# KyleHuang9/YOLO-LP

Measured on AMD Instinct MI355X. Metric: images/sec (640×640) end-to-end detect+NMS, yololps, 1/2/4/8 MI355X, higher is better.
Workload: dtype f16; 1 GPU; yololps 640x640 bs=32/GPU f16, synthetic frames resident in HBM, seeded random-init weights (sigma 0.25), conf 0.40 iou 0.45 max_det 1000; global_batch=32, parallelism=dp1: images sharded, all-gather of detections

## Files before the change

### include/lp_hip.h

```cpp
#ifndef LP_HIP_H
#define LP_HIP_H

#include <stddef.h>
#include <stdint.h>

#ifdef __cplusplus
extern "C" {
#endif

typedef enum { LP_OK = 0, LP_ERR_ARG = -1, LP_ERR_STATE = -2, LP_ERR_HIP = -3, LP_ERR_UNSUPPORTED = -4 } lp_status;
typedef enum { LP_F16 = 0, LP_BF16 = 1, LP_F32 = 2 } lp_dtype;
typedef enum { LP_ACT_NONE = 0, LP_ACT_RELU = 1, LP_ACT_SILU = 2 } lp_act;

#define LP_PRED_COLS 290
#define LP_DET_COLS 28
#define LP_MAX_SRC 4

typedef struct lp_engine lp_engine;

const char* lp_version(void);
const char* lp_last_error(void);

int lp_engine_create(lp_engine** out, int act_dtype );
void lp_engine_destroy(lp_engine* e);

int lp_engine_tensor(lp_engine* e, int channels, int stride_log2);

int lp_engine_set_lane(lp_engine* e, int lane);

int lp_engine_add_input(lp_engine* e, int dst);

typedef struct lp_conv_desc {
    int n_src;
    int src[LP_MAX_SRC];
    int dst;
    int ksize;
    int stride;
    int act;
    int res;
    float res_alpha;
    const float* weight;
    const float* bias;
    int dst2;
} lp_conv_desc;

int lp_engine_add_conv(lp_engine* e, const lp_conv_desc* d);

int lp_engine_add_deconv2x2(lp_engine* e, int src, int dst, const float* weight, const float* bias);

int lp_engine_add_pool5_chain(lp_engine* e, int src, int dst1, int dst2, int dst3);

int lp_engine_add_head_cls(lp_engine* e, int src, int level, int n_cls, const float* weight, const float* bias);

int lp_engine_add_head_box(lp_engine* e, int src, int level, int reg_bins, const float* weight, const float* bias,
                           const float* proj);

int lp_engine_finalize(lp_engine* e, int n_levels);
size_t lp_engine_weight_bytes(const lp_engine* e);
int lp_engine_upload(lp_engine* e, void* dev_weights, void* stream);

size_t lp_engine_arena_bytes(const lp_engine* e, int B, int H, int W);
int lp_engine_bind(lp_engine* e, void* dev_arena, size_t bytes, int B, int H, int W);
int lp_engine_tensor_info(const lp_engine* e, int id, size_t* offset, int* c, int* c_stored, int* h, int* w);
int lp_engine_num_anchors(const lp_engine* e);

int lp_engine_forward(lp_engine* e, const void* x, int x_dtype, float* pred, void* stream);

int lp_engine_forward_det(lp_engine* e, const void* x, int x_dtype, double conf_thres, void* workspace, size_t workspace_bytes,
                          void* stream);

int lp_engine_set_graph(lp_engine* e, int enable);

int lp_engine_set_single_lane(lp_engine* e, int enable);

int lp_engine_set_mfma16(lp_engine* e, int enable);

int lp_engine_num_ops(const lp_engine* e);
int lp_engine_op_info(const lp_engine* e, int op, int* kind, int* ksize, int* cin, int* cout, double* flops,
                      double* bytes);
int lp_engine_profile(lp_engine* e, const void* x, int x_dtype, float* pred, void* stream, float* op_ms, int reps);
int lp_engine_profile_ops(lp_engine* e, const void* x, int x_dtype, float* pred, void* stream, float* op_ms, int reps, int inner);

enum { LP_VARIANT_STREAM64 = 16, LP_VARIANT_STREAM128 = 17, LP_VARIANT_ROWS = 18,
       LP_VARIANT_PIPE_D = 32, LP_VARIANT_PIPE_B = 33, LP_VARIANT_PIPE_F = 34, LP_VARIANT_PIPE_C = 35,
       LP_VARIANT_PIPE_P = 36 ,
       LP_VARIANT_PIPE16_D = 39, LP_VARIANT_PIPE16_F = 41 ,
       LP_VARIANT_PIPE16_V0 = 42, LP_VARIANT_PIPE16_V1 = 43 ,
       LP_VARIANT_FUSED_STEM2 = 37 ,
       LP_VARIANT_FUSED_PW_S2 = 38  };
enum { LP_VARIANT_FUSED_BIFUSION = 45 };
enum { LP_VARIANT_BOX_SPARSE = 46, LP_VARIANT_BOX_DENSE = 47 };
enum { LP_VARIANT_PIPE16_S2A = 48, LP_VARIANT_PIPE16_S2B = 49 };
int lp_engine_op_carrier(const lp_engine* e, int op, int frame_direct);
int lp_engine_op_io(const lp_engine* e, int op, int* src , int* n_src, int* res, int* dst );
int lp_engine_autotune(lp_engine* e, const void* x, int x_dtype, float* pred, void* stream, int reps);
int lp_engine_op_variant(const lp_engine* e, int op, int* cfg, int* nbuf);
int lp_engine_set_op_variant(lp_engine* e, int op, int cfg, int nbuf);
int lp_engine_set_op_tile(lp_engine* e, int op, int choice);
int lp_engine_op_tile(const lp_engine* e, int op, int* choice, int* TH, int* TW);
int lp_engine_copy_tuning(lp_engine* dst, const lp_engine* src);

size_t lp_nms_workspace_bytes(int B, int N);
int lp_nms(float* pred, int B, int N, double conf_thres, double iou_thres, int max_det, float* det, int32_t* count,
           int32_t* keep, void* workspace, size_t workspace_bytes, void* stream);

int lp_nms_candidates(int B, int N, double iou_thres, int max_det, float* det, int32_t* count, int32_t* keep, void* workspace,
                      size_t workspace_bytes, void* stream);

const int32_t* lp_nms_candidate_counts(const void* workspace, int B, int N);

int lp_preprocess_letterbox(const unsigned char* img, int h0, int w0, void* out, int out_dtype, int H, int W, int rh, int rw,
                            int top, int left, void* stream);
int lp_rescale_round(float* det, int n, double ratio, double padx, double pady, int img_w, int img_h, void* stream);

#define LP_FRAMES_PER_LAUNCH 64
typedef struct lp_frame_desc {
    const unsigned char* img;
    int h0, w0, rh, rw, top, left;
} lp_frame_desc;
typedef struct lp_rescale_desc { double ratio, padx, pady; int img_w, img_h; } lp_rescale_desc;
int lp_preprocess_letterbox_batch(const lp_frame_desc* desc, int n_frames, int B, void* out, int out_dtype, int H, int W,
                                  void* stream);
int lp_rescale_round_batch(float* det, const int32_t* count, int B, int max_det, const lp_rescale_desc* desc, void* stream);

typedef struct lp_tile_desc {
    const unsigned char* img;
    int h0, w0;
    int y0, x0, th, tw;
    int rh, rw, top, left;
} lp_tile_desc;
int lp_preprocess_tiles_batch(const lp_tile_desc* desc, int n_tiles, int B, void* out, int out_dtype, int H, int W, void* stream);

#define LP_NV12_PER_LAUNCH 32
typedef struct lp_nv12_desc {
    const unsigned char* y;
    const unsigned char* uv;
    int pitch_y, pitch_uv;
    int h0, w0;
    int y0, x0, th, tw;
    int rh, rw, top, left;
    int matrix;
} lp_nv12_desc;
typedef struct lp_nv12_bgr_desc {
    const unsigned char* y;
    const unsigned char* uv;
    int pitch_y, pitch_uv;
    int h0, w0;
    int matrix;
    unsigned char* out;
} lp_nv12_bgr_desc;
int lp_preprocess_nv12_batch(const lp_nv12_desc* desc, int n, int B, void* out, int out_dtype, int H, int W, void* stream);
int lp_nv12_to_bgr_batch(const lp_nv12_bgr_desc* desc, int n, void* stream);

typedef struct lp_tile_ref { int frame, y0, x0, th, tw; } lp_tile_ref;
size_t lp_merge_tiles_workspace_bytes(int n_frames, int max_det);
int lp_merge_tiles(const float* det_t, const int32_t* count_t, const lp_tile_ref* tiles, int n_tiles, int max_det_t,
                   const int* frame_hw, int n_frames, double thres, int metric , int border, int max_det,
                   float* det, int32_t* count, int32_t* src, void* workspace, size_t workspace_bytes, void* stream);

#define LP_TRACK_MAX_TRACKS 128
#define LP_TRACK_MAX_DETS 128
#define LP_TRACK_MAX_CLS 64
typedef struct lp_track_params { double match_thres, new_thres, expand; int max_age; int ncls[8]; } lp_track_params;
size_t lp_track_state_bytes(int n_streams, int max_tracks);
size_t lp_track_dropped_offset(int max_tracks, int stream_index);
int lp_track_update(void* state, int n_streams, int max_tracks, const lp_track_params* p,
                    const float* det, const int32_t* count, int B, int max_det,
                    const int* stream_of , const unsigned char* flush ,
                    float* det_out, int32_t* tid, int32_t* ended_i, float* ended_f, int32_t* ended_count,
                    int max_ended, void* stream);
int lp_track_update_slots(void* state, int n_streams, int max_tracks, const lp_track_params* p,
                          const float* det, const int32_t* count, int B, int max_det,
                          const int* stream_of , const unsigned char* flush ,
                          float* det_out, int32_t* tid, int32_t* slot, int32_t* ended_i, float* ended_f, int32_t* ended_count,
                          int max_ended, void* stream);
typedef struct lp_track_hold_params { int min_hits, max_misses; } lp_track_hold_params;
int lp_track_update_hold(void* state, int n_streams, int max_tracks, const lp_track_params* p,
                         const float* det, const int32_t* count, int B, int max_det,
                         const int* stream_of , const unsigned char* flush ,
                         float* det_out, int32_t* tid, int32_t* slot, int32_t* ended_i, float* ended_f, int32_t* ended_count,
                         int max_ended, const lp_track_hold_params* hp, float* det_hold, int32_t* count_hold, int32_t* tid_hold,
                         void* stream);

typedef struct lp_crop_desc {
    const unsigned char* img;
    int h0, w0;
    int max_crops;
    int out_slot;
} lp_crop_desc;
int lp_plate_crops_batch(const lp_crop_desc* desc, int n_frames, const float* det, const int32_t* count, int max_det,
                         unsigned char* out, int32_t* status, int n_slots, int crop_h, int crop_w, void* stream);

int lp_crop_sharpness(const unsigned char* crops, const int32_t* status, int n_slots, int crop_h, int crop_w,
                      unsigned long long* sharp, void* stream);

size_t lp_best_shot_state_bytes(int n_streams, int max_tracks, int crop_h, int crop_w);
int lp_best_shot_update(void* state, int n_streams, int max_tracks, int crop_h, int crop_w,
                        const float* det, const int32_t* count, int B, int max_det, const int32_t* tid, const int32_t* slot,
                        const unsigned char* crops, const int32_t* status, const unsigned long long* sharp, int max_crops,
                        const int* stream_of , const int32_t* ended_i, const int32_t* ended_count, int max_ended,
                        double min_score, unsigned char* shot_crops, int32_t* shot_i, unsigned long long* shot_q, float* shot_det,
                        void* stream);

typedef struct lp_stack_params { double min_score, min_width; unsigned long long min_sharp; int search, max_frames; } lp_stack_params;
size_t lp_stack_state_bytes(int n_streams, int max_tracks, int crop_h, int crop_w);
int lp_stack_update(void* state, int n_streams, int max_tracks, int crop_h, int crop_w,
                    const float* det, const int32_t* count, int B, int max_det, const int32_t* tid, const int32_t* slot,
                    const unsigned char* crops, const int32_t* status, const unsigned long long* sharp, int max_crops,
                    const int* stream_of , const int32_t* ended_i, const int32_t* ended_count, int max_ended,
                    const lp_stack_params* p, unsigned char* stack_crops, int32_t* stack_i, void* stream);

#define LP_REDACT_MAX_CELL 64
typedef struct lp_redact_desc {
    unsigned char* p0;
    unsigned char* p1;
    int pitch0, pitch1;
    int h0, w0;
    int format;
} lp_redact_desc;
typedef struct lp_redact_params {
    int mode;
    int cell;
    double margin;
    unsigned char fill[3];
} lp_redact_params;
size_t lp_redact_workspace_bytes(const lp_redact_desc* desc, int n_frames, const lp_redact_params* p);
int lp_redact_plates_batch(const lp_redact_desc* desc, int n_frames, const float* det, const int32_t* count, int max_det,
                           const lp_redact_params* p, int32_t* status ,
                           void* workspace, size_t workspace_bytes, void* stream);

#define LP_REDACT_MAX_RADIUS 48
typedef struct lp_redact_gauss_params {
    double margin;
    int radius, radius_c;
    uint16_t taps[LP_REDACT_MAX_RADIUS + 1];
    uint16_t taps_c[LP_REDACT_MAX_RADIUS + 1];
} lp_redact_gauss_params;
size_t lp_redact_gauss_workspace_bytes(const lp_redact_desc* desc, int n_frames, const lp_redact_gauss_params* p);
int lp_redact_gauss_batch(const lp_redact_desc* desc, int n_frames, const float* det, const int32_t* count, int max_det,
                          const lp_redact_gauss_params* p, int32_t* status ,
                          void* workspace, size_t workspace_bytes, void* stream);

#define LP_JPEG_MAX_RESTART 32
#define LP_JPEG_PER_LAUNCH 32
typedef struct lp_jpeg_desc {
// ... 90 lines not shown
```

### yolo-lp_amd/csrc/lp_conv.hip

```cpp
#include "lp_internal.h"

#include <cstdlib>

namespace lp {

int conv_launch_f16(int cfg, int mode, int ksize, int stride, int nbuf, const ConvArgs& a, hipStream_t st);
int conv_launch_bf16(int cfg, int mode, int ksize, int stride, int nbuf, const ConvArgs& a, hipStream_t st);
int conv_launch_f32(int cfg, int mode, int ksize, int stride, int nbuf, const ConvArgs& a, hipStream_t st);

int conv_stream_launch_f16(int wc, const ConvArgs& a, int cb_pack, int lds, hipStream_t st);
int conv_stream_launch_bf16(int wc, const ConvArgs& a, int cb_pack, int lds, hipStream_t st);
int conv_stream_launch_f32(int wc, const ConvArgs& a, int cb_pack, int lds, hipStream_t st);

int conv_pipe_launch_f16(int pcfg, const ConvArgs& a, int ncu, hipStream_t st);
int conv_pipe_launch_bf16(int pcfg, const ConvArgs& a, int ncu, hipStream_t st);

int head_rows_launch_f16(const ConvArgs& a, int cb_pack, hipStream_t st);
int head_rows_launch_bf16(const ConvArgs& a, int cb_pack, hipStream_t st);
int head_rows_launch_f32(const ConvArgs& a, int cb_pack, hipStream_t st);
int head_box_det_launch_f16(const ConvArgs& a, int cb_pack, hipStream_t st);
int head_box_det_launch_bf16(const ConvArgs& a, int cb_pack, hipStream_t st);
int head_box_det_launch_f32(const ConvArgs& a, int cb_pack, hipStream_t st);

ConvShape conv_shape(int dtype, int cfg, int ksize, int stride) {
    const int sz = (int)dtype_size(dtype);
    ConvShape s;
    int wc = 2, wp = 2, wgc = 1, wgp = 4;
    switch (cfg) {
        case CFG_A: wgc = 2; wgp = 2; break;
        case CFG_B: break;
        case CFG_C: wc = 1; break;
        case CFG_D: wgc = 2; wgp = 4; break;
        case CFG_E: wc = 1; wgc = 2; wgp = 2; break;
        case CFG_F: wc = 1; wgc = 4; wgp = 2; break;
    }
    s.WP = wp;
    s.WGC = wgc;
    s.WGP = wgp;
    s.CB = 32 * wc * wgc;
    s.PB = 32 * wp * wgp;
    s.NT = 64 * wgc * wgp;
    s.KC = ksize == 1 ? 128 / sz : 32 / sz;
    s.HPMAX = ksize == 1 ? s.PB : (stride == 1 ? 2 * s.PB + 128 : 5 * s.PB + 128);
    return s;
}

static inline int swz_host(int row, int g, int gpr) { return gpr == 2 ? (g ^ ((row >> 3) & 1)) : (g ^ ((row >> 1) & 7)); }

int conv_pick_pitch(const ConvShape& s, int dtype, int ksize, int stride, int TH, int TW) {
    const int hw = (TW - 1) * stride + ksize, hh = (TH - 1) * stride + ksize;
    if (ksize == 1) return hw;
    (void)dtype;
    const int rowb = 32, gpr = 2, npix = TH * TW;
    static const int G0[16] = {0, 1, 2, 3, 12, 13, 14, 15, 20, 21, 22, 23, 24, 25, 26, 27};
    static const int G1[16] = {4, 5, 6, 7, 8, 9, 10, 11, 16, 17, 18, 19, 28, 29, 30, 31};
    long best_cost = -1;
    int best = hw;
    for (int pitch = hw; pitch < hw + 16; ++pitch) {
        if (hh * pitch > s.HPMAX) break;
        long cost = 0;
        for (int blk = 0; blk * 32 < s.PB; ++blk)
            for (int t = 0; t < ksize * ksize; ++t)
                for (int half = 0; half < 2; ++half)
                    for (int g = 0; g < 2; ++g) {
                        const int* lanes = g ? G1 : G0;
                        int addr[16], n = 0, slot_cnt[16] = {0};
                        for (int k = 0; k < 16; ++k) {
                            int pl = blk * 32 + lanes[k];
                            if (pl >= npix) pl = 0;
                            const int ty = pl / TW, tx = pl - ty * TW;
                            const int kx = t % ksize, hwe = (hw + 1) >> 1;
                            const int col = stride == 2 ? (kx & 1) * hwe + tx + (kx >> 1) : tx * stride + kx;
                            const int hp = (ty * stride + t / ksize) * pitch + col;
                            const int a = hp * rowb + swz_host(hp, half, gpr) * 16;
                            bool dup = false;
                            for (int m = 0; m < n; ++m) dup |= addr[m] == a;
                            if (!dup) { addr[n++] = a; ++slot_cnt[(a >> 4) & 15]; }
                        }
                        int mx = 1;
                        for (int k = 0; k < 16; ++k) mx = slot_cnt[k] > mx ? slot_cnt[k] : mx;
                        cost += mx;
                    }
        cost = cost * 64 + (pitch - hw);
        if (best_cost < 0 || cost < best_cost) { best_cost = cost; best = pitch; }
    }
    return best;
}

int conv_pick_pitch16(const ConvShape& s, int TH, int TW) {
    const int hw = TW + 2, hh = TH + 2, rowb = 32, npix = TH * TW;
    static const int GRP[4][16] = {{0, 1, 2, 3, 12, 13, 14, 15, 20, 21, 22, 23, 24, 25, 26, 27}, {4, 5, 6, 7, 8, 9, 10, 11, 16, 17, 18, 19, 28, 29, 30, 31},
                                   {32, 33, 34, 35, 44, 45, 46, 47, 52, 53, 54, 55, 56, 57, 58, 59}, {36, 37, 38, 39, 40, 41, 42, 43, 48, 49, 50, 51, 60, 61, 62, 63}};
    auto qo = [](int i) { return ((i >> 2) == 2 ? 12 : (i >> 2) == 3 ? 8 : (i & 12)) + (i & 3); };
    long best_cost = -1;
    int best = hw;
    for (int pitch = hw; pitch < hw + 16; ++pitch) {
        if (hh * pitch > s.HPMAX) break;
        long cost = 0;
        for (int blk = 0; blk * 16 < s.PB; ++blk)
            for (int st = 0; st < 9; ++st) {
                const int ta = st < 4 ? 2 * st : (st == 4 ? 8 : 2 * st - 9), tb = st == 4 ? 0 : ta + 1;
                for (int gq = 0; gq < 4; ++gq) {
                    int addr[16], n = 0, slot_cnt[16] = {0};
                    for (int k = 0; k < 16; ++k) {
                        const int l = GRP[gq][k], i = l & 15, g = l >> 4;
                        int pl = blk * 16 + qo(i);
                        if (pl >= npix) pl = 0;
                        const int ty = pl / TW, tx = pl - ty * TW, t = g < 2 ? ta : tb;
                        const int hp = (ty + t / 3) * pitch + tx + t % 3;
                        const int a = hp * rowb + swz_host(hp, g & 1, 2) * 16 + (g >> 1) * (1 << 20);
                        bool dup = false;
                        for (int m = 0; m < n; ++m) dup |= addr[m] == a;
                        if (!dup) { addr[n++] = a; ++slot_cnt[(a >> 4) & 15]; }
                    }
                    int mx = 1;
                    for (int k = 0; k < 16; ++k) mx = slot_cnt[k] > mx ? slot_cnt[k] : mx;
                    cost += mx;
                }
            }
        cost = cost * 64 + (pitch - hw);
        if (best_cost < 0 || cost < best_cost) { best_cost = cost; best = pitch; }
    }
    return best;
}

void conv_pick_tile16v(const ConvShape& s, int Ho, int Wo, int B, int nct, int choice, int* TH, int* TW, int stride) {
    struct Cand { double cost; int th, tw; };
    Cand best[4];
    int n = 0;
    const int ncu = device_cus();
    for (int th = 1; th <= Ho; ++th)
        for (int tw = 1; tw <= Wo; ++tw) {
            const int hh = (th - 1) * stride + 3, hw = (tw - 1) * stride + 3;
            if (th * tw > s.PB || hh * hw > s.HPMAX) continue;
            const long tiles = (long)B * ceil_div(Ho, th) * ceil_div(Wo, tw) * nct;
            const int nb = ceil_div(th * tw, 16), per_wave = ceil_div(nb, s.WGP);
            const double cost = (double)ceil_div((int)tiles, ncu) * (per_wave + 0.75) + 1e-4 * hh * hw + 1e-7 * tiles;
            int pos = n < 4 ? n : 4;
            for (int k = 0; k < (n < 4 ? n : 4); ++k)
                if (cost < best[k].cost) { pos = k; break; }
            if (pos >= 4) continue;
            for (int k = (n < 4 ? n : 3); k > pos; --k) best[k] = best[k - 1];
            best[pos] = {cost, th, tw};
            if (n < 4) ++n;
        }
    if (n == 0) { *TH = 1; *TW = 1; return; }
    if (choice < 0) choice = 0;
    if (choice >= n) choice = n - 1;
    *TH = best[choice].th;
    *TW = best[choice].tw;
}

void conv_pick_tile(const ConvShape& s, int ksize, int stride, int Ho, int Wo, int choice, int* TH, int* TW) {
    struct Cand { long cost; int th, tw; };
    Cand best[4];
    int n = 0;
    for (int th = 1; th <= s.PB && th <= Ho; ++th) {
        int tw = s.PB / th;
        if (tw > Wo) tw = Wo;
        if (tw < 1) continue;
        const int hh = (th - 1) * stride + ksize, hw = (tw - 1) * stride + ksize;
        if (hh * hw > s.HPMAX) continue;
        const long tiles = (long)ceil_div(Ho, th) * ceil_div(Wo, tw);
        Cand c = {tiles * 100000 + (long)hh * hw, th, tw};
        int pos = n < 4 ? n : 4;
        for (int k = 0; k < (n < 4 ? n : 4); ++k)
            if (c.cost < best[k].cost) { pos = k; break; }
        if (pos >= 4) continue;
        for (int k = (n < 4 ? n : 3); k > pos; --k) best[k] = best[k - 1];
        best[pos] = c;
        if (n < 4) ++n;
    }
    if (n == 0) { *TH = 1; *TW = 1; return; }
    if (choice < 0) choice = 0;
    if (choice >= n) choice = n - 1;
// ... 48 lines not shown
}

ConvShape conv_pipe_shape(int pcfg) {
    ConvShape s;
    s.KC = 16;
    s.NT = 512;
    s.WP = 2;
    switch (pcfg) {
        case PIPE_B: s.CB = 64; s.WGC = 1; s.WGP = 8; s.HPMAX = 704; break;
        case PIPE_F: case PIPE16_F: s.CB = 128; s.WGC = 4; s.WGP = 2; s.HPMAX = 384; break;
        case PIPE_C: s.CB = 32; s.WGC = 1; s.WGP = 8; s.HPMAX = 736; break;
        case PIPE16_V0: s.CB = 128; s.WGC = 2; s.WGP = 4; s.HPMAX = 512; s.PB = 4 * 7 * 16; return s;
        case PIPE16_V1: s.CB = 128; s.WGC = 4; s.WGP = 2; s.HPMAX = 512; s.PB = 2 * 7 * 16; return s;
        case PIPE16_S2A: s.CB = 128; s.WGC = 2; s.WGP = 4; s.HPMAX = 864; s.PB = 4 * 4 * 16; return s;
        case PIPE16_S2B: s.CB = 128; s.WGC = 4; s.WGP = 2; s.HPMAX = 864; s.PB = 2 * 7 * 16; return s;
        default: s.CB = 128; s.WGC = 2; s.WGP = 4; s.HPMAX = 384; break;
    }
    s.PB = 32 * s.WP * s.WGP;
    return s;
}

bool conv_pipe_fits(int dtype, int pcfg, int cb_pack, int ksize, int stride, int mode, int nct, int nphase, int nchunks) {
    if (pcfg == PIPE_P) return false;
    if (pipe_is_16s2(pcfg))
        return dtype != LP_F32 && ksize == 3 && stride == 2 && mode == MODE_ACT && nphase == 1 && cb_pack == 128 && nct * 128 <= 512 && nchunks >= 1 && nchunks <= 64;
    if (pipe_is_16(pcfg) && (nchunks < 4 || nchunks % 4 != 0)) return false;
    if (dtype == LP_F32 || pcfg < 0 || (pcfg >= PIPE_COUNT && !pipe_is_16(pcfg)) || ksize != 3 || stride != 1 || mode != MODE_ACT || nphase != 1) return false;
    const ConvShape s = conv_pipe_shape(pcfg);
    if (pipe_is_16v(pcfg) && (nct * s.CB > 512 || nchunks > 32)) return false;
    return s.CB == cb_pack && nct * s.CB <= 1024 && nchunks <= 64;
}

static int g_ncu[16] = {0};
int device_cus() {
    int dev = 0;
    if (hipGetDevice(&dev) != hipSuccess || dev < 0 || dev >= 16) return 256;
    if (!g_ncu[dev]) {
        int n = 0;
        if (hipDeviceGetAttribute(&n, hipDeviceAttributeMultiprocessorCount, dev) != hipSuccess || n < 8) n = 256;
        g_ncu[dev] = n / 8 * 8;
        if (const char* cap = getenv("LP_PIPE_MAXWG")) { const int c = atoi(cap) / 8 * 8; if (c >= 8 && c < g_ncu[dev]) g_ncu[dev] = c; }
    }
    return g_ncu[dev];
}

bool stem_planar_tile(int Ho, int Wo, int choice, int* TH, int* TW) {
    struct Cand { long long tiles; int th, tw; };
    std::vector<Cand> cands;
    for (int tw = 4; tw <= 512 && tw < Wo + 4; tw += 4) {
        int th = 512 / tw;
        if (th > Ho) th = Ho;
        while (th >= 1 && ((th + 2) * 6 + 2) * (tw / 4 + 2) * 16 > 20 * 1024) --th;
        if (th < 1) continue;
        cands.push_back({(long long)ceil_div(Ho, th) * ceil_div(Wo, tw), th, tw});
    }
    std::sort(cands.begin(), cands.end(), [](const Cand& x, const Cand& y) { return x.tiles != y.tiles ? x.tiles < y.tiles : x.tw > y.tw; });
    if (choice < 0 || choice >= (int)cands.size()) return false;
    *TH = cands[choice].th;
    *TW = cands[choice].tw;
    return true;
}

bool stem2_fused_tile(int Ho, int Wo, int choice, int* TH, int* TW, int* hpitch) {
    struct Cand { long long cost; int th, tw; };
    std::vector<Cand> cands;
    for (int tw = 2; tw <= 128 && tw < Wo + 2; tw += 2)
        for (int th = 1; th <= 128 / tw && th <= Ho; ++th) {
            const int hp4 = tw / 2 + 2, rin = 2 * th + 3, hps = 2 * tw + 1;
            const int ntb = (th * tw + 31) / 32;
            if ((rin * 6 + 2) * hp4 * 16 > 21 * 1024 || (rin * 6 * hp4 + 63) / 64 > 24 || (2 * th + 1) * hps > 640 || ntb * 2 > 16) continue;
            cands.push_back({(long long)ceil_div(Ho, th) * ceil_div(Wo, tw) * (2 * th + 1) * hps, th, tw});
        }
    std::sort(cands.begin(), cands.end(), [](const Cand& x, const Cand& y) { return x.cost != y.cost ? x.cost < y.cost : x.tw > y.tw; });
    if (choice < 0 || choice >= (int)cands.size()) return false;
    *TH = cands[choice].th;
    *TW = cands[choice].tw;
    *hpitch = 2 * cands[choice].tw + 1;
    return true;
}

int conv_pipe_launch(int dtype, int pcfg, const ConvArgs& a, hipStream_t st) {
    if (pcfg == PIPE_P || pcfg == PIPE_FUSED2 || pcfg == PIPE_FUSED_PW || pcfg == PIPE_FUSED_BF) {
        switch (dtype) {
            case LP_F16: return conv_pipe_launch_f16(pcfg, a, device_cus(), st);
            case LP_BF16: return conv_pipe_launch_bf16(pcfg, a, device_cus(), st);
        }
        return fail(LP_ERR_UNSUPPORTED, "planar stem: 16-bit frames only");
    }
    const ConvShape s = conv_pipe_shape(pcfg);
    if (pipe_is_16s2(pcfg)) {
        const int hh2 = 2 * a.TH + 1, hw2 = 2 * a.TW + 1, nchunks = a.chunk_begin[a.nsrc];
        if (a.TH < 1 || a.TW < 1 || a.TH * a.TW > s.PB || a.hpitch != hw2 || hh2 * a.hpitch > s.HPMAX)
            return fail(LP_ERR_ARG, "conv3x3 s2p16: tile does not fit the kernel configuration");
        if (a.tiles_x * a.TW < a.Wo || a.tiles_y * a.TH < a.Ho) return fail(LP_ERR_ARG, "conv3x3 s2p16: tiles do not cover the output");
        if (a.nsrc < 1 || a.nsrc > LP_MAX_SRC || a.nct < 1 || a.nct * s.CB > 512 || nchunks < 1 || nchunks > 64 || a.nphase != 1 || a.out_scale != 1 ||
            a.H != 2 * a.Ho || a.W != 2 * a.Wo || a.out2)
            return fail(LP_ERR_ARG, "conv3x3 s2p16: not a 3x3 stride-2 layer this kernel runs");
        const int stride = a.out_pix_stride > a.res_cs ? a.out_pix_stride : a.res_cs;
        if (((long long)a.TH * a.Wo + a.TW) * stride + 2048 >= (1ll << 31)) return fail(LP_ERR_ARG, "conv3x3 s2p16: a tile's rows span more than 2^31 elements");
        switch (dtype) {
            case LP_F16: return conv_pipe_launch_f16(pcfg, a, device_cus(), st);
            case LP_BF16: return conv_pipe_launch_bf16(pcfg, a, device_cus(), st);
        }
        return fail(LP_ERR_UNSUPPORTED, "conv3x3 s2p16: 16-bit activations only");
    }
    const int hh = a.TH + 2, hw = a.TW + 2;
    if (pcfg < 0 || (pcfg >= PIPE_COUNT && !pipe_is_16(pcfg))) return fail(LP_ERR_ARG, "conv3x3 pipe: configuration");
    if (pipe_is_16(pcfg) && (a.chunk_begin[a.nsrc] < 4 || a.chunk_begin[a.nsrc] % 4 != 0)) return fail(LP_ERR_ARG, "conv3x3 pipe16: K-chunks not a multiple of four");
    if (a.TH < 1 || a.TW < 1 || a.TH * a.TW > s.PB || a.hpitch < hw || hh * a.hpitch > s.HPMAX)
        return fail(LP_ERR_ARG, "conv3x3 pipe: tile does not fit the kernel configuration");
    if (a.tiles_x * a.TW < a.Wo || a.tiles_y * a.TH < a.Ho) return fail(LP_ERR_ARG, "conv3x3 pipe: tiles do not cover the output");
    if (pipe_is_16v(pcfg) && (a.nct * s.CB > 512 || a.chunk_begin[a.nsrc] > 32)) return fail(LP_ERR_ARG, "conv3x3 pipe16v: layer exceeds the kernel's LDS tables");
    if (pipe_is_16v(pcfg)) {
        int stride = a.out_pix_stride > a.res_cs ? a.out_pix_stride : a.res_cs;
        if (a.out2 && a.out2_pix_stride > stride) stride = a.out2_pix_stride;
        if (((long long)a.TH * a.Wo + a.TW) * stride + 2048 >= (1ll << 31)) return fail(LP_ERR_ARG, "conv3x3 pipe16v: a tile's rows span more than 2^31 elements");
    }
    if (a.chunk_begin[a.nsrc] > 64) return fail(LP_ERR_ARG, "conv3x3 pipe: more K-chunks than the kernel's LDS chunk table holds");
    if (a.nsrc < 1 || a.nsrc > LP_MAX_SRC || a.nct < 1 || a.nct * s.CB > 1024 || a.nphase != 1 || a.out_scale != 1 || a.Ho != a.H || a.Wo != a.W)
        return fail(LP_ERR_ARG, "conv3x3 pipe: not a 3x3 stride-1 layer this kernel runs");
    switch (dtype) {
        case LP_F16: return conv_pipe_launch_f16(pcfg, a, device_cus(), st);
        case LP_BF16: return conv_pipe_launch_bf16(pcfg, a, device_cus(), st);
    }
    return fail(LP_ERR_UNSUPPORTED, "conv3x3 pipe: 16-bit activations only");
}

bool head_rows_fits(int dtype, int nchunks, int cb_pack, int out_c) {
    const long lds = (long)nchunks * 9 * 32 * 128 + 9 * 32 * 4 + 32 * 8 + 32 * 1168;
    return nchunks >= 1 && nchunks <= 3 && lds <= 160 * 1024 && (cb_pack == 32 || cb_pack == 64 || cb_pack == 128) && out_c == LP_PRED_COLS - 13;
}
bool head_det_fits(int dtype, int nchunks, int cb_pack, int out_c) {
    const long lds = (long)nchunks * 9 * 32 * 128 + 9 * 32 * 4 + 32 * 8 * 4 + 16 + 6 * 32 * 8 * 4 + 6 * 1168;
    return nchunks >= 1 && nchunks <= (dtype == LP_F32 ? 3 : 4) && lds <= 160 * 1024 && (cb_pack == 32 || cb_pack == 64 || cb_pack == 128) &&
           out_c == LP_PRED_COLS - 13;
}

bool head_box_det_fits(const ConvArgs& a, int cb_pack, int ksize, int stride) {
    const int nchunks = a.chunk_begin[a.nsrc];
    return ksize == 1 && stride == 1 && a.nsrc == 1 && nchunks >= 1 && nchunks <= 4 && a.reg_bins == 1 && a.out_c == 12 && a.nct == 1 &&
           cb_pack >= 32 && a.nphase == 1 && a.out_scale == 1 && a.Ho == a.H && a.Wo == a.W && a.src[0].cs % 8 == 0;
}
int head_box_det_launch(int dtype, const ConvArgs& a, int cb_pack, hipStream_t st) {
    if (!a.det_mode || !a.out || !a.zero || !head_box_det_fits(a, cb_pack, 1, 1)) return fail(LP_ERR_ARG, "head box: op does not fit");
    if (a.out_pix_stride % 4 != 0 || a.out_img_stride % 4 != 0 || ((uintptr_t)a.out & 15)) return fail(LP_ERR_ARG, "head box: candidate rows are not 16-byte aligned");
    switch (dtype) {
        case LP_F16: return head_box_det_launch_f16(a, cb_pack, st);
        case LP_BF16: return head_box_det_launch_bf16(a, cb_pack, st);
        case LP_F32: return head_box_det_launch_f32(a, cb_pack, st);
    }
    return fail(LP_ERR_ARG, "head box: dtype");
}

int head_rows_launch(int dtype, const ConvArgs& a, int cb_pack, hipStream_t st) {
    const int nchunks = a.chunk_begin[a.nsrc];
    if (!(a.det_mode ? head_det_fits(dtype, nchunks, cb_pack, a.out_c) : head_rows_fits(dtype, nchunks, cb_pack, a.out_c)))
        return fail(LP_ERR_ARG, "head rows: op does not fit");
    const int kc = 128 / (int)dtype_size(dtype);
    for (int i = 0; i < a.nsrc; ++i)
        if (a.src[i].cs % (kc / 4) != 0)
            return fail(LP_ERR_ARG, "head rows: source channels are not whole 32-byte K-steps");
    if (a.nphase != 1 || a.out_scale != 1 || a.Ho != a.H || a.Wo != a.W || !a.out) return fail(LP_ERR_ARG, "head rows: bad geometry");
    switch (dtype) {
        case LP_F16: return head_rows_launch_f16(a, cb_pack, st);
        case LP_BF16: return head_rows_launch_bf16(a, cb_pack, st);
        case LP_F32: return head_rows_launch_f32(a, cb_pack, st);
    }
    return fail(LP_ERR_ARG, "head rows: dtype");
}

}

extern "C" int lp_plan_block_tile(int variant, int Ho, int Wo, int B, int nct, int choice, int* TH, int* TW, int* hpitch) {
    const int pcfg = variant - LP_VARIANT_PIPE_D;
    if (!TH || !TW || Ho < 1 || Wo < 1 || B < 1 || nct < 1) return lp::fail(LP_ERR_ARG, "lp_plan_block_tile: bad arguments");
    if (!lp::pipe_is_16v(pcfg) && !lp::pipe_is_16s2(pcfg)) return lp::fail(LP_ERR_UNSUPPORTED, "lp_plan_block_tile: not a block-tiled variant");
    const lp::ConvShape s = lp::conv_pipe_shape(pcfg);
    const int stride = lp::pipe_is_16s2(pcfg) ? 2 : 1;
    lp::conv_pick_tile16v(s, Ho, Wo, B, nct, choice, TH, TW, stride);
    if (hpitch) *hpitch = (*TW - 1) * stride + 3;
    return LP_OK;
}

extern "C" int lp_plan_stem_tile(int fused, int Ho, int Wo, int choice, int* TH, int* TW, int* hpitch) {
    if (!TH || !TW || Ho < 1 || Wo < 1) return lp::fail(LP_ERR_ARG, "lp_plan_stem_tile: bad arguments");
    int hp = 0;
    const bool ok = fused ? lp::stem2_fused_tile(Ho, Wo, choice, TH, TW, &hp) : lp::stem_planar_tile(Ho, Wo, choice, TH, TW);
    if (hpitch) *hpitch = hp;
    return ok ? LP_OK : LP_ERR_UNSUPPORTED;
}
```

### yolo-lp_amd/csrc/lp_conv_bf16.hip

```cpp
#include "lp_conv_kernel.inc"
#include "lp_conv1x1_stream.inc"
#include "lp_head_rows.inc"
#include "lp_head_box.inc"
#include "lp_conv3x3_pipe.inc"
#include "lp_conv3x3_pipe16.inc"
#include "lp_conv3x3_pipe16v.inc"
#include "lp_conv3x3_s2p16.inc"
#include "lp_stem_planar.inc"
#include "lp_stem2_fused.inc"
#include "lp_pw_s2_fused.inc"
#include "lp_bifusion_fused.inc"

namespace lp {
int conv_launch_bf16(int cfg, int mode, int ksize, int stride, int nbuf, const ConvArgs& a, hipStream_t st) {
    return launch_dtype<bf16>(cfg, mode, ksize, stride, nbuf, a, st);
}
int conv_stream_launch_bf16(int wc, const ConvArgs& a, int cb_pack, int lds, hipStream_t st) {
    return stream_launch_dtype<bf16>(wc, a, cb_pack, lds, st);
}
int head_rows_launch_bf16(const ConvArgs& a, int cb_pack, hipStream_t st) { return head_rows_launch_dtype<bf16>(a, cb_pack, st); }
int head_box_det_launch_bf16(const ConvArgs& a, int cb_pack, hipStream_t st) { return head_box_det_launch_dtype<bf16>(a, cb_pack, st); }
int conv_pipe_launch_bf16(int pcfg, const ConvArgs& a, int ncu, hipStream_t st) {
    if (pcfg == PIPE_FUSED2) return stem2_fused_launch<bf16>(a, ncu, st);
    if (pcfg == PIPE_FUSED_PW) return pw_s2_fused_launch<bf16>(a, ncu, st);
    if (pcfg == PIPE_FUSED_BF) return bifusion_launch_dtype<bf16>(a, ncu, st);
    if (pipe_is_16s2(pcfg)) return s2p16_launch_dtype<bf16>(pcfg, a, ncu, st);
    if (pipe_is_16v(pcfg)) return pipe16v_launch_dtype<bf16>(pcfg, a, ncu, st);
    if (pipe_is_16(pcfg)) return pipe16_launch_dtype<bf16>(pcfg, a, ncu, st);
    return pcfg == PIPE_P ? stem_planar_launch<bf16>(a, ncu, st) : pipe_launch_dtype<bf16>(pcfg, a, ncu, st);
}
}
```

### yolo-lp_amd/csrc/lp_conv_f16.hip

```cpp
#include "lp_conv_kernel.inc"
#include "lp_conv1x1_stream.inc"
#include "lp_head_rows.inc"
#include "lp_head_box.inc"
#include "lp_conv3x3_pipe.inc"
#include "lp_conv3x3_pipe16.inc"
#include "lp_conv3x3_pipe16v.inc"
#include "lp_conv3x3_s2p16.inc"
#include "lp_stem_planar.inc"
#include "lp_stem2_fused.inc"
#include "lp_pw_s2_fused.inc"
#include "lp_bifusion_fused.inc"

namespace lp {
int conv_launch_f16(int cfg, int mode, int ksize, int stride, int nbuf, const ConvArgs& a, hipStream_t st) {
    return launch_dtype<f16>(cfg, mode, ksize, stride, nbuf, a, st);
}
int conv_stream_launch_f16(int wc, const ConvArgs& a, int cb_pack, int lds, hipStream_t st) {
    return stream_launch_dtype<f16>(wc, a, cb_pack, lds, st);
}
int head_rows_launch_f16(const ConvArgs& a, int cb_pack, hipStream_t st) { return head_rows_launch_dtype<f16>(a, cb_pack, st); }
int head_box_det_launch_f16(const ConvArgs& a, int cb_pack, hipStream_t st) { return head_box_det_launch_dtype<f16>(a, cb_pack, st); }
int conv_pipe_launch_f16(int pcfg, const ConvArgs& a, int ncu, hipStream_t st) {
    if (pcfg == PIPE_FUSED2) return stem2_fused_launch<f16>(a, ncu, st);
    if (pcfg == PIPE_FUSED_PW) return pw_s2_fused_launch<f16>(a, ncu, st);
    if (pcfg == PIPE_FUSED_BF) return bifusion_launch_dtype<f16>(a, ncu, st);
    if (pipe_is_16s2(pcfg)) return s2p16_launch_dtype<f16>(pcfg, a, ncu, st);
    if (pipe_is_16v(pcfg)) return pipe16v_launch_dtype<f16>(pcfg, a, ncu, st);
    if (pipe_is_16(pcfg)) return pipe16_launch_dtype<f16>(pcfg, a, ncu, st);
    return pcfg == PIPE_P ? stem_planar_launch<f16>(a, ncu, st) : pipe_launch_dtype<f16>(pcfg, a, ncu, st);
}
}
```

### yolo-lp_amd/csrc/lp_engine.hip

```cpp
#include "lp_internal.h"

#include <cmath>
#include <cstdlib>
#include <cstring>
#include <map>
#include <utility>
#include <vector>

namespace lp {

static thread_local std::string g_err;
void set_error(const std::string& msg) { g_err = msg; }
int fail(int code, const std::string& msg) {
    g_err = msg;
    return code;
}

enum OpKind { OP_INPUT = 0, OP_CONV = 1, OP_DECONV = 2, OP_POOL = 3, OP_HEAD_CLS = 4, OP_HEAD_BOX = 5 };

struct Tensor {
    int c, cs, sl;
    bool unused = false;
    size_t offset;
    int h, w;
};

struct Choice {
    int cfg = CFG_A, nbuf = 1, tile = 0;
    int stream_wc = 0, stream_rd = 2;
    int rows = 0;
    int pipe = 0;
    int planar = 0;
    int fused = 0;
    int fused_pw = 0;
    int fused_bf = 0;
    Choice& choice() { return *this; }
};

struct Op : Choice {
    int kind = OP_CONV;
    int nsrc = 0;
    int src[LP_MAX_SRC] = {-1, -1, -1, -1};
    int dst = -1, dst2 = -1, dst3 = -1;
    int ksize = 1, stride = 1, act = 0;
    int res = -1;
    float alpha = 0.f;
    int cout = 0;
    int cin = 0;
    int level = 0, reg_bins = 1;
    bool s2d = false;
    int alg_kk = 0;
    int lane = 0;
    std::vector<int> deps;
    bool signal = false;
    std::vector<float> weight, bias, proj;
    int mode = MODE_ACT, nct = 1, nchunks = 0, nphase = 1;
    size_t det_scratch = (size_t)-1;
    int box_sparse = 1;
    int bf_up = -1, bf_cv1 = -1;
    int bf_carrier = -1;
    int chunk_begin[LP_MAX_SRC + 1] = {0, 0, 0, 0, 0};
    size_t w_off = 0, b_off = 0, proj_off = 0;
    long long w_phase_stride = 0;
};

struct Launch : Choice {
    ConvArgs a;
    long long pred_off = 0;
    int mode = 0, ks = 1, st = 1, cb_pack = 0;
    bool is_conv = false;
};

}

using namespace lp;
struct lp_engine;
static bool bifusion_fused_possible(const lp_engine* e, size_t i, int* up, int* cv1);
static bool op_fam16(const lp_engine* e, const lp::Op& op);
static int fam16_default_pipe(const lp_engine* e, const lp::Op& op);

#ifndef LP_MAX_LANES
#define LP_MAX_LANES 5
#endif
struct lp_engine {
    int dtype = LP_F16;
    bool finalized = false;
    int n_levels = 3;
    std::vector<Tensor> tensors;
    std::vector<Op> ops;
    std::vector<unsigned char> blob;
    char* dev_w = nullptr;
    char* arena = nullptr;
    size_t arena_bytes = 0;
    int B = 0, H = 0, W = 0, n_anchors = 0;
    std::vector<int> level_off;
    std::vector<hipEvent_t> events;
    int cur_lane = 0;
    int n_lanes = 1;
    hipStream_t lane_stream[LP_MAX_LANES] = {};
    std::vector<hipEvent_t> op_event;
    hipEvent_t fork_ev = nullptr, join_ev[LP_MAX_LANES] = {};
    bool single_lane = true;
    bool use_graph = false;
    bool s2p16 = getenv("LP_S2P16") != nullptr;
    bool mfma16 = getenv("LP_NO_MFMA16") == nullptr;
    bool box_sparse_ok = false;
    std::vector<int> box_ord;
    struct CachedGraph {
        hipGraphExec_t exec = nullptr;
        const void* x = nullptr;
        float* pred = nullptr;
        void* ws = nullptr;
        float conf = 0.f;
        int x_dtype = -1;
        unsigned long long epoch = 0, last_use = 0;
        hipStream_t stream = nullptr;
    };
    std::vector<CachedGraph> graphs;
    unsigned long long graph_clock = 0;
    hipEvent_t done_ev = nullptr;
    bool done_valid = false;
    hipStream_t cap_stream = nullptr;
    unsigned long long epoch = 1;
    std::vector<Launch> launches;
    Launch stem_planar;
    Launch stem2_fused;
    std::map<int, Launch> pw_fused;
    std::map<int, Launch> bf_fused;
    std::map<std::vector<int>, std::vector<Choice>> tuned;
};

static int prepare_op(lp_engine* e, size_t idx);
static int* op_tile_slot(lp_engine* e, int op_idx, int* bias, const Launch** L);
static unsigned long long* g_stamps = nullptr;
extern "C" void lpdbg_set_stamps(void* p) { g_stamps = (unsigned long long*)p; }
static bool valid_tensor(const lp_engine* e, int id) { return id >= 0 && id < (int)e->tensors.size(); }

extern "C" const char* lp_version(void) { return "yololp-hip 0.1 (gfx950)"; }
extern "C" const char* lp_last_error(void) { return g_err.c_str(); }

extern "C" int lp_engine_create(lp_engine** out, int act_dtype) {
    if (!out) return fail(LP_ERR_ARG, "lp_engine_create: null out");
    if (act_dtype != LP_F16 && act_dtype != LP_BF16 && act_dtype != LP_F32) return fail(LP_ERR_ARG, "lp_engine_create: dtype");
    lp_engine* e = new lp_engine();
    e->dtype = act_dtype;
    *out = e;
    return LP_OK;
}

extern "C" void lp_engine_destroy(lp_engine* e) {
    if (!e) return;
    for (int l = 1; l < LP_MAX_LANES; ++l)
        if (e->lane_stream[l]) (void)hipStreamSynchronize(e->lane_stream[l]);
    if (e->done_valid) (void)hipEventSynchronize(e->done_ev);
    if (e->done_ev) (void)hipEventDestroy(e->done_ev);
    for (hipEvent_t ev : e->events) (void)hipEventDestroy(ev);
    for (auto& g : e->graphs) {
        if (g.stream) (void)hipStreamSynchronize(g.stream);
        if (g.exec) (void)hipGraphExecDestroy(g.exec);
    }
    if (e->cap_stream) (void)hipStreamDestroy(e->cap_stream);
    for (hipEvent_t ev : e->op_event) if (ev) (void)hipEventDestroy(ev);
    if (e->fork_ev) (void)hipEventDestroy(e->fork_ev);
    for (int l = 1; l < LP_MAX_LANES; ++l) { if (e->join_ev[l]) (void)hipEventDestroy(e->join_ev[l]); if (e->lane_stream[l]) (void)hipStreamDestroy(e->lane_stream[l]); }
    delete e;
}

extern "C" int lp_engine_tensor(lp_engine* e, int channels, int stride_log2) {
    if (!e || e->finalized) return fail(LP_ERR_STATE, "lp_engine_tensor: engine is null or frozen");
    if (channels < 1 || stride_log2 < 0 || stride_log2 > 6) return fail(LP_ERR_ARG, "lp_engine_tensor: bad shape");
    Tensor t;
    t.c = channels;
    t.cs = round_up(channels, 8);
    t.sl = stride_log2;
    t.offset = 0;
    t.h = t.w = 0;
    e->tensors.push_back(t);
    return (int)e->tensors.size() - 1;
}

extern "C" int lp_engine_set_lane(lp_engine* e, int lane) {
    if (!e || e->finalized) return fail(LP_ERR_STATE, "lp_engine_set_lane: engine is null or frozen");
    if (lane < 0 || lane >= LP_MAX_LANES) return fail(LP_ERR_ARG, "lp_engine_set_lane: lane must be 0..4");
    e->cur_lane = lane;
    return LP_OK;
}

extern "C" int lp_engine_add_input(lp_engine* e, int dst) {
    if (!e || e->finalized) return fail(LP_ERR_STATE, "lp_engine_add_input: engine is null or frozen");
    if (!e->ops.empty()) return fail(LP_ERR_STATE, "lp_engine_add_input: must be the first op");
    if (!valid_tensor(e, dst) || e->tensors[dst].c != 3 || e->tensors[dst].sl != 0)
        return fail(LP_ERR_ARG, "lp_engine_add_input: dst must be a 3-channel full-resolution tensor");
    Op op;
    op.kind = OP_INPUT;
    op.dst = dst;
    op.cout = 3;
    op.cin = 3;
    op.lane = e->cur_lane;
    e->ops.push_back(op);
    return LP_OK;
}

extern "C" int lp_engine_add_conv(lp_engine* e, const lp_conv_desc* d) {
    if (!e || e->finalized) return fail(LP_ERR_STATE, "lp_engine_add_conv: engine is null or frozen");
    if (!d || !d->weight || !d->bias) return fail(LP_ERR_ARG, "lp_engine_add_conv: null descriptor / weights");
    if (d->n_src < 1 || d->n_src > LP_MAX_SRC) return fail(LP_ERR_ARG, "lp_engine_add_conv: n_src");
    if (!((d->ksize == 1 && d->stride == 1) || (d->ksize == 3 && (d->stride == 1 || d->stride == 2))))
        return fail(LP_ERR_UNSUPPORTED, "lp_engine_add_conv: only 1x1/s1, 3x3/s1 and 3x3/s2");
    if (d->act < LP_ACT_NONE || d->act > LP_ACT_SILU) return fail(LP_ERR_ARG, "lp_engine_add_conv: act");
    if (!valid_tensor(e, d->dst)) return fail(LP_ERR_ARG, "lp_engine_add_conv: dst");
    Op op;
    op.kind = OP_CONV;
    op.nsrc = d->n_src;
    int cin = 0;
    if (!valid_tensor(e, d->src[0])) return fail(LP_ERR_ARG, "lp_engine_add_conv: src");
    const int sl = e->tensors[d->src[0]].sl;
    for (int i = 0; i < d->n_src; ++i) {
        if (!valid_tensor(e, d->src[i])) return fail(LP_ERR_ARG, "lp_engine_add_conv: src");
        if (e->tensors[d->src[i]].sl != sl) return fail(LP_ERR_ARG, "lp_engine_add_conv: sources differ in resolution");
        if (d->src[i] == d->dst) return fail(LP_ERR_ARG, "lp_engine_add_conv: in-place conv");
        op.src[i] = d->src[i];
        cin += e->tensors[d->src[i]].c;
    }
    const Tensor& td = e->tensors[d->dst];
    if (td.sl != sl + (d->stride == 2 ? 1 : 0)) return fail(LP_ERR_ARG, "lp_engine_add_conv: dst resolution");
    if (d->res >= 0) {
        if (!valid_tensor(e, d->res) || e->tensors[d->res].c != td.c || e->tensors[d->res].sl != td.sl || d->res == d->dst)
            return fail(LP_ERR_ARG, "lp_engine_add_conv: residual shape");
    }
    int cout2 = 0;
    if (d->dst2 > 0) {
        if (!valid_tensor(e, d->dst2) || d->dst2 == d->dst || e->tensors[d->dst2].sl != td.sl) return fail(LP_ERR_ARG, "lp_engine_add_conv: dst2");
        for (int i = 0; i < d->n_src; ++i) if (d->src[i] == d->dst2) return fail(LP_ERR_ARG, "lp_engine_add_conv: in-place conv");
        if (d->res >= 0) return fail(LP_ERR_UNSUPPORTED, "lp_engine_add_conv: no residual with two destinations");
        if (td.c % 8 != 0) return fail(LP_ERR_UNSUPPORTED, "lp_engine_add_conv: the first destination of two needs a multiple of 8 channels");
        cout2 = e->tensors[d->dst2].c;
    }
    op.dst = d->dst;
    op.dst2 = d->dst2 > 0 ? d->dst2 : -1;
    op.ksize = d->ksize;
    op.stride = d->stride;
    op.act = d->act;
    op.res = d->res >= 0 ? d->res : -1;
    op.alpha = d->res_alpha;
    op.cout = td.c + cout2;
    op.cin = cin;
    op.weight.assign(d->weight, d->weight + (size_t)op.cout * cin * d->ksize * d->ksize);
    op.bias.assign(d->bias, d->bias + op.cout);
    op.lane = e->cur_lane;
    e->ops.push_back(op);
    return LP_OK;
}

extern "C" int lp_engine_add_deconv2x2(lp_engine* e, int src, int dst, const float* weight, const float* bias) {
    if (!e || e->finalized) return fail(LP_ERR_STATE, "lp_engine_add_deconv2x2: engine is null or frozen");
    if (!weight || !bias || !valid_tensor(e, src) || !valid_tensor(e, dst) || src == dst)
        return fail(LP_ERR_ARG, "lp_engine_add_deconv2x2: bad argument");
    if (e->tensors[dst].sl != e->tensors[src].sl - 1) return fail(LP_ERR_ARG, "lp_engine_add_deconv2x2: dst must be 2x the source");
    Op op;
    op.kind = OP_DECONV;
    op.nsrc = 1;
    op.src[0] = src;
    op.dst = dst;
    op.cin = e->tensors[src].c;
    op.cout = e->tensors[dst].c;
    op.weight.assign(weight, weight + (size_t)op.cin * op.cout * 4);
    op.bias.assign(bias, bias + op.cout);
    op.lane = e->cur_lane;
    e->ops.push_back(op);
    return LP_OK;
}

extern "C" int lp_engine_add_pool5_chain(lp_engine* e, int src, int dst1, int dst2, int dst3) {
    if (!e || e->finalized) return fail(LP_ERR_STATE, "lp_engine_add_pool5_chain: engine is null or frozen");
    const int ids[4] = {src, dst1, dst2, dst3};
    for (int i = 0; i < 4; ++i) {
        if (!valid_tensor(e, ids[i])) return fail(LP_ERR_ARG, "lp_engine_add_pool5_chain: tensor id");
        if (e->tensors[ids[i]].c != e->tensors[src].c || e->tensors[ids[i]].sl != e->tensors[src].sl)
            return fail(LP_ERR_ARG, "lp_engine_add_pool5_chain: shapes differ");
        for (int k = 0; k < i; ++k)
            if (ids[k] == ids[i]) return fail(LP_ERR_ARG, "lp_engine_add_pool5_chain: tensors must be distinct");
    }
    Op op;
    op.kind = OP_POOL;
    op.nsrc = 1;
    op.src[0] = src;
    op.dst = dst1;
    op.dst2 = dst2;
    op.dst3 = dst3;
    op.cin = op.cout = e->tensors[src].c;
    op.lane = e->cur_lane;
    e->ops.push_back(op);
    return LP_OK;
}

static int add_head(lp_engine* e, int kind, int src, int level, int cout, int reg_bins, const float* weight, const float* bias,
                    const float* proj) {
    if (!e || e->finalized) return fail(LP_ERR_STATE, "lp_engine_add_head: engine is null or frozen");
    if (!weight || !bias || !valid_tensor(e, src) || level < 0 || level > 3 || cout < 1)
        return fail(LP_ERR_ARG, "lp_engine_add_head: bad argument");
    if (e->tensors[src].sl != 3 + level) return fail(LP_ERR_ARG, "lp_engine_add_head: level / resolution mismatch (strides 8,16,32,64)");
    Op op;
    op.kind = kind;
    op.nsrc = 1;
    op.src[0] = src;
    op.level = level;
    op.reg_bins = reg_bins;
    op.cin = e->tensors[src].c;
    op.cout = cout;
    op.weight.assign(weight, weight + (size_t)cout * op.cin);
    op.bias.assign(bias, bias + cout);
    if (proj) op.proj.assign(proj, proj + reg_bins);
    op.lane = e->cur_lane;
    e->ops.push_back(op);
// ... 55 lines not shown
            const Op& o = e->ops[i];
            for (int k = 0; k < o.nsrc; ++k) only_reader &= o.src[k] != in_id;
            only_reader &= o.res != in_id;
        }
        if (only_reader) {
            Tensor t;
            t.c = 12; t.cs = 16; t.sl = 1; t.offset = 0; t.h = t.w = 0;
            e->tensors.push_back(t);
            const int s2d_id = (int)e->tensors.size() - 1;
            e->tensors[in_id].unused = true;
            e->ops[0].s2d = true;
            e->ops[0].dst = s2d_id;
            std::vector<float> w2((size_t)c.cout * 12 * 9, 0.f);
            for (int co = 0; co < c.cout; ++co)
                for (int ch = 0; ch < 3; ++ch)
                    for (int ky = 0; ky < 3; ++ky)
                        for (int kx = 0; kx < 3; ++kx) {
                            const int dy = ky == 0 ? 0 : 1, py = ky == 1 ? 0 : 1;
                            const int dx = kx == 0 ? 0 : 1, px = kx == 1 ? 0 : 1;
                            w2[(((size_t)co * 12 + ch * 4 + py * 2 + px) * 3 + dy) * 3 + dx] = c.weight[(((size_t)co * 3 + ch) * 3 + ky) * 3 + kx];
                        }
            c.weight.swap(w2);
            c.src[0] = s2d_id;
            c.stride = 1;
            c.cin = 12;
            c.alg_kk = 27;
        }
    }
    if (getenv("LP_SINGLE_LANE")) for (Op& op : e->ops) op.lane = 0;
    e->n_lanes = 1;
    for (size_t i = 0; i < e->ops.size(); ++i) {
        Op& op = e->ops[i];
        if (op.lane + 1 > e->n_lanes) e->n_lanes = op.lane + 1;
        auto reads = [](const Op& o, int t) { for (int k = 0; k < o.nsrc; ++k) if (o.src[k] == t) return true; return o.res == t; };
        auto writes = [](const Op& o, int t) { return o.dst == t || o.dst2 == t || o.dst3 == t; };
        std::vector<int> mine_r, mine_w;
        for (int k = 0; k < op.nsrc; ++k) mine_r.push_back(op.src[k]);
        if (op.res >= 0) mine_r.push_back(op.res);
        for (int t : {op.dst, op.dst2, op.dst3}) if (t >= 0) mine_w.push_back(t);
        for (int lane = 0; lane < LP_MAX_LANES; ++lane) {
            if (lane == op.lane) continue;
            for (size_t j = i; j-- > 0;) {
                const Op& o = e->ops[j];
                if (o.lane != lane) continue;
                bool hit = false;
                for (int t : mine_r) hit |= writes(o, t);
                for (int t : mine_w) hit |= writes(o, t) || reads(o, t);
                if (hit) { op.deps.push_back((int)j); e->ops[j].signal = true; break; }
            }
        }
    }
    for (Op& op : e->ops) {
        if (op.kind == OP_INPUT || op.kind == OP_POOL) continue;
        const int ks = op.kind == OP_CONV ? op.ksize : 1;
        const int st = op.kind == OP_CONV ? op.stride : 1;
        int cout_store;
        if (op.kind == OP_HEAD_CLS) { op.mode = MODE_PRED; op.cfg = getenv("LP_PRED_CFG") ? atoi(getenv("LP_PRED_CFG")) : CFG_C; cout_store = op.cout; }
        else if (op.kind == OP_HEAD_BOX) {
            op.mode = MODE_DECODE; op.cfg = op.cout <= 32 ? CFG_C : CFG_A; cout_store = op.cout;
        }
        else {
            op.mode = MODE_ACT;
            cout_store = e->tensors[op.dst].cs + (op.kind == OP_CONV && op.dst2 >= 0 ? e->tensors[op.dst2].cs : 0);
            op.cfg = pick_cfg(dt, ks, st, cout_store);
            if (op.cfg == CFG_A) op.cfg = CFG_D;
            const char* tc = getenv("LP_TUNE_CFG128");
            const char* tb = getenv("LP_TUNE_NBUF");
            if (tc && op.cfg == CFG_D) op.cfg = atoi(tc);
            if (tb && op.cfg != CFG_C) op.nbuf = atoi(tb) == 2 ? 2 : 1;
        }
        const ConvShape s = conv_shape(dt, op.cfg, ks, st);
        op.nct = ceil_div(cout_store, s.CB);
        op.nphase = op.kind == OP_DECONV ? 4 : 1;
        int cin_off[LP_MAX_SRC + 1] = {0};
        op.chunk_begin[0] = 0;
        for (int i = 0; i < op.nsrc; ++i) {
            const Tensor& t = e->tensors[op.src[i]];
            op.chunk_begin[i + 1] = op.chunk_begin[i] + ceil_div(t.cs, s.KC);
            cin_off[i + 1] = cin_off[i] + t.c;
        }
        for (int i = op.nsrc; i < LP_MAX_SRC; ++i) op.chunk_begin[i + 1] = op.chunk_begin[op.nsrc];
        op.nchunks = op.chunk_begin[op.nsrc];
        if (op_fam16(e, op)) op.pipe = fam16_default_pipe(e, op);
        const int taps = ks * ks;
        const size_t per_phase = (size_t)op.nct * op.nchunks * taps * s.CB * s.KC;
        op.w_phase_stride = (long long)per_phase;
        align();
        op.w_off = blob.size();
        blob.resize(blob.size() + per_phase * op.nphase * esz, 0);
        unsigned char* wp = blob.data() + op.w_off;
        for (int ph = 0; ph < op.nphase; ++ph)
            for (int ct = 0; ct < op.nct; ++ct)
                for (int i = 0; i < op.nsrc; ++i) {
                    const Tensor& t = e->tensors[op.src[i]];
                    for (int q = op.chunk_begin[i]; q < op.chunk_begin[i + 1]; ++q) {
                        const int c0 = (q - op.chunk_begin[i]) * s.KC;
                        for (int tp = 0; tp < taps; ++tp)
                            for (int cl = 0; cl < s.CB; ++cl) {
                                const int co = ct * s.CB + cl;
                                if (co >= op.cout) continue;
                                const size_t row = ((((size_t)ph * op.nct + ct) * op.nchunks + q) * taps + tp) * s.CB + cl;
                                const int srow = tp * s.CB + cl;
                                for (int kc = 0; kc < s.KC; ++kc) {
                                    const int c = c0 + kc;
                                    if (c >= t.c) break;
                                    const int ci = cin_off[i] + c;
                                    float v;
                                    if (op.kind == OP_DECONV)
                                        v = op.weight[((size_t)ci * op.cout + co) * 4 + ph];
                                    else
                                        v = op.weight[((size_t)co * op.cin + ci) * taps + tp];
                                    const int epg = 16 / (int)esz, gpr = s.KC / epg;
                                    const int pos = gpr == 2 ? ((kc / epg) ^ ((srow >> 3) & 1)) : ((kc / epg) ^ ((srow >> 1) & 7));
                                    put_elem(wp, row * s.KC + (size_t)pos * epg + kc % epg, v, dt);
                                }
                            }
                    }
                }
        align();
        op.b_off = blob.size();
        blob.resize(blob.size() + (size_t)op.nct * s.CB * 4, 0);
        memcpy(blob.data() + op.b_off, op.bias.data(), (size_t)op.cout * 4);
        if (!op.proj.empty()) {
            align();
            op.proj_off = blob.size();
            blob.resize(blob.size() + op.proj.size() * 4, 0);
            memcpy(blob.data() + op.proj_off, op.proj.data(), op.proj.size() * 4);
        }
        std::vector<float>().swap(op.weight);
    }
    align();
    for (size_t i = 0; i < e->ops.size(); ++i) {
        int up = -1, c1 = -1;
        if (!bifusion_fused_possible(e, i, &up, &c1)) continue;
        e->ops[i].bf_up = up;
        e->ops[i].bf_cv1 = c1;
        e->ops[(size_t)up].bf_carrier = e->ops[(size_t)c1].bf_carrier = (int)i;
    }
    {
        e->box_ord.assign(e->ops.size(), -1);
        bool ok = true;
        int nbox = 0, cls_seen = 0, cls_level = -1;
        for (size_t i = 0; i < e->ops.size(); ++i) {
            const Op& o = e->ops[i];
            if (o.kind == OP_HEAD_CLS) { ++cls_seen; cls_level = o.level; }
            if (o.kind == OP_HEAD_BOX) {
                ok = ok && cls_seen == 1 && cls_level == o.level;
                e->box_ord[i] = nbox++;
                cls_seen = 0;
            }
        }
        e->box_sparse_ok = ok && nbox >= 1 && nbox <= 4 && cls_seen == 0;
    }
    e->finalized = true;
    return LP_OK;
}

extern "C" size_t lp_engine_weight_bytes(const lp_engine* e) { return e && e->finalized ? e->blob.size() : 0; }

extern "C" int lp_engine_upload(lp_engine* e, void* dev_weights, void* stream) {
    if (!e || !e->finalized) return fail(LP_ERR_STATE, "lp_engine_upload: finalize first");
    if (!dev_weights || ((uintptr_t)dev_weights & 255)) return fail(LP_ERR_ARG, "lp_engine_upload: need a 256-byte aligned device pointer");
    LP_HIP_CHECK(hipMemcpyAsync(dev_weights, e->blob.data(), e->blob.size(), hipMemcpyHostToDevice, (hipStream_t)stream));
    LP_HIP_CHECK(hipStreamSynchronize((hipStream_t)stream));
    e->dev_w = (char*)dev_weights;
    return LP_OK;
}

static bool rows_fits(const lp_engine* e, const Op& op);
static bool det_fits(const lp_engine* e, const Op& op);

static size_t place(const lp_engine* e, int B, int H, int W, std::vector<Tensor>* out, std::vector<size_t>* scratch = nullptr) {
    size_t off = 0;
    const size_t esz = dtype_size(e->dtype);
    for (size_t i = 0; i < e->tensors.size(); ++i) {
        Tensor t = e->tensors[i];
        t.h = H >> t.sl;
        t.w = W >> t.sl;
        t.offset = off;
        if (!t.unused) off += ((size_t)B * t.h * t.w * t.cs * esz + 255) / 256 * 256;
        if (out) (*out)[i] = t;
    }
    if (scratch) scratch->assign(e->ops.size(), (size_t)-1);
    for (size_t i = 0; i < e->ops.size(); ++i) {
        const Op& op = e->ops[i];
        if (op.kind != OP_HEAD_CLS || det_fits(e, op)) continue;
        if (scratch) (*scratch)[i] = off;
        off += ((size_t)B * (H >> (3 + op.level)) * (W >> (3 + op.level)) * LP_PRED_COLS * 4 + 255) / 256 * 256;
    }
    return off + 256;
}

static bool pool_fits(const lp_engine* e, int H, int W) {
    for (const Op& op : e->ops) {
        if (op.kind != OP_POOL) continue;
        const Tensor& t = e->tensors[op.src[0]];
        const int h = H >> t.sl, w = W >> t.sl;
        if (pool_min_lds_bytes(e->dtype, h, w) > POOL_MAX_LDS || h * w >= 65536) return false;
    }
    return true;
}

static int size_granule(const lp_engine* e) {
    int sl = 5;
    for (const Tensor& t : e->tensors) sl = t.sl > sl ? t.sl : sl;
    return 1 << sl;
}

extern "C" size_t lp_engine_arena_bytes(const lp_engine* e, int B, int H, int W) {
    if (!e || B < 1) return 0;
    const int g = size_granule(e);
    if (H < g || W < g || H % g || W % g || !pool_fits(e, H, W)) return 0;
    return place(e, B, H, W, nullptr);
}

static bool apply_tuned(lp_engine* e) {
    const auto it = e->tuned.find({e->B, e->H, e->W});
    if (it == e->tuned.end()) return false;
    for (size_t i = 0; i < e->ops.size(); ++i) e->ops[i].choice() = it->second[i];
    return true;
}

extern "C" int lp_engine_bind(lp_engine* e, void* dev_arena, size_t bytes, int B, int H, int W) {
    if (!e || !e->finalized) return fail(LP_ERR_STATE, "lp_engine_bind: finalize first");
    const int gran = size_granule(e);
    if (B < 1 || H < gran || W < gran || H % gran || W % gran)
        return fail(LP_ERR_ARG, "lp_engine_bind: H and W must be positive multiples of " + std::to_string(gran) + " (the coarsest stride of the graph)");
    if (!dev_arena || ((uintptr_t)dev_arena & 255)) return fail(LP_ERR_ARG, "lp_engine_bind: need a 256-byte aligned device pointer");
    if (!pool_fits(e, H, W))
        return fail(LP_ERR_UNSUPPORTED, "lp_engine_bind: the SPPF pool chain keeps a whole stride-32 map in LDS: input too large (limit ~2048x2048 px in "
                                        "f16 / bf16, ~1440x1440 in f32)");
    const size_t need = place(e, B, H, W, nullptr);
    if (bytes < need) return fail(LP_ERR_ARG, "lp_engine_bind: arena too small");
    if ((long long)B * H * W >= (1LL << 31)) return fail(LP_ERR_UNSUPPORTED, "lp_engine_bind: batch too large for 32-bit pixel indices");
    std::vector<size_t> scratch;
    place(e, B, H, W, &e->tensors, &scratch);
    for (size_t i = 0; i < e->ops.size(); ++i) e->ops[i].det_scratch = scratch[i];
    e->arena = (char*)dev_arena;
    e->arena_bytes = bytes;
    e->B = B;
    e->H = H;
    e->W = W;
    e->level_off.assign(e->n_levels + 1, 0);
    for (int l = 0; l < e->n_levels; ++l) e->level_off[l + 1] = e->level_off[l] + (H >> (3 + l)) * (W >> (3 + l));
    e->n_anchors = e->level_off[e->n_levels];
    if (!e->dev_w) return fail(LP_ERR_STATE, "lp_engine_bind: upload the weights first");
    apply_tuned(e);
    e->launches.assign(e->ops.size(), Launch());
    for (size_t i = 0; i < e->ops.size(); ++i) {
        int rc = prepare_op(e, i);
        if (rc) return rc;
    }
    return LP_OK;
}

extern "C" int lp_engine_tensor_info(const lp_engine* e, int id, size_t* offset, int* c, int* c_stored, int* h, int* w) {
    if (!e || !valid_tensor(e, id)) return fail(LP_ERR_ARG, "lp_engine_tensor_info: tensor id");
    const Tensor& t = e->tensors[id];
    if (offset) *offset = t.offset;
    if (c) *c = t.c;
    if (c_stored) *c_stored = t.cs;
    if (h) *h = t.h;
    if (w) *w = t.w;
    return LP_OK;
}

extern "C" int lp_engine_num_anchors(const lp_engine* e) { return e ? e->n_anchors : 0; }
extern "C" int lp_engine_num_ops(const lp_engine* e) { return e ? (int)e->ops.size() : 0; }

extern "C" int lp_engine_op_info(const lp_engine* e, int i, int* kind, int* ksize, int* cin, int* cout, double* flops, double* bytes) {
    if (!e || i < 0 || i >= (int)e->ops.size()) return fail(LP_ERR_ARG, "lp_engine_op_info: op index");
    if (!e->arena) return fail(LP_ERR_STATE, "lp_engine_op_info: bind first");
    const Op& op = e->ops[i];
    const double esz = (double)dtype_size(e->dtype);
    double fl = 0, by = 0;
    auto tbytes = [&](int id) { const Tensor& t = e->tensors[id]; return (double)e->B * t.h * t.w * t.c * esz; };
    const Tensor& s0 = e->tensors[op.kind == OP_INPUT ? op.dst : op.src[0]];
    const double in_px = (double)e->B * s0.h * s0.w;
    switch (op.kind) {
        case OP_INPUT: by = (double)e->B * e->H * e->W * 3 * esz + tbytes(op.dst); break;
        case OP_CONV: {
            const Tensor& d = e->tensors[op.dst];
            fl = 2.0 * e->B * d.h * d.w * op.cout * (op.alg_kk ? op.alg_kk : op.cin * op.ksize * op.ksize);
            for (int k = 0; k < op.nsrc; ++k) by += tbytes(op.src[k]);
            by += tbytes(op.dst) + (op.dst2 >= 0 ? tbytes(op.dst2) : 0) + (op.res >= 0 ? tbytes(op.res) : 0) + (double)op.cout * op.cin * op.ksize * op.ksize * esz;
            break;
        }
        case OP_DECONV: fl = 2.0 * in_px * op.cin * op.cout * 4; by = tbytes(op.src[0]) + tbytes(op.dst) + 4.0 * op.cin * op.cout * esz; break;
        case OP_POOL: by = 4 * tbytes(op.src[0]); break;
        case OP_HEAD_CLS:
        case OP_HEAD_BOX:
            fl = 2.0 * in_px * op.cin * op.cout;
            by = tbytes(op.src[0]) + in_px * (op.kind == OP_HEAD_CLS ? op.cout : 13) * 4 + (double)op.cin * op.cout * esz;
            break;
    }
    if (kind) *kind = op.kind;
    if (ksize) *ksize = op.ksize;
    if (cin) *cin = op.cin;
    if (cout) *cout = op.cout;
    if (flops) *flops = fl;
    if (bytes) *bytes = by;
    return LP_OK;
}

static bool stream_fits(const lp_engine* e, const Op& op, int wc) {
    if (op.kind != OP_CONV || op.ksize != 1 || op.stride != 1 || op.mode != MODE_ACT) return false;
    if (op.dst2 >= 0 && e->tensors[op.dst].cs % (32 * wc) != 0) return false;
    const int kc = 128 / (int)dtype_size(e->dtype);
    for (int i = 0; i < op.nsrc; ++i)
        if (e->tensors[op.src[i]].cs % (kc / 4) != 0) return false;
    return conv_stream_lds(e->dtype, wc, op.nchunks, conv_shape(e->dtype, op.cfg, 1, 1).CB) >= 0;
}

static bool rows_fits(const lp_engine* e, const Op& op) {
    if (op.kind != OP_HEAD_CLS) return false;
    const int kc = 128 / (int)dtype_size(e->dtype);
    for (int i = 0; i < op.nsrc; ++i) {
        const int cs = e->tensors[op.src[i]].cs;
        if (cs % (kc / 4) != 0) return false;
    }
    return head_rows_fits(e->dtype, op.nchunks, conv_shape(e->dtype, op.cfg, 1, 1).CB, op.cout);
}

static bool det_fits(const lp_engine* e, const Op& op) {
    if (op.kind != OP_HEAD_CLS || getenv("LP_NO_HEAD_DET")) return false;
    const int kc = 128 / (int)dtype_size(e->dtype);
    for (int i = 0; i < op.nsrc; ++i) {
        const int cs = e->tensors[op.src[i]].cs;
        if (cs % (kc / 4) != 0) return false;
    }
    return head_det_fits(e->dtype, op.nchunks, conv_shape(e->dtype, op.cfg, 1, 1).CB, op.cout);
}

static bool op_fam16(const lp_engine* e, const Op& op) {
    if (!e->mfma16 || e->dtype == LP_F32 || op.kind != OP_CONV || op.ksize != 3 || op.mode != MODE_ACT) return false;
    if (op.stride == 2)
        return e->s2p16 && op.dst2 < 0 && conv_pipe_fits(e->dtype, PIPE16_S2A, conv_shape(e->dtype, op.cfg, 3, 2).CB, 3, 2, op.mode, op.nct, op.nphase, op.nchunks);
    if (op.stride != 1) return false;
    return conv_pipe_fits(e->dtype, PIPE16_D, conv_shape(e->dtype, op.cfg, 1, 1).CB, 3, 1, op.mode, op.nct, op.nphase, op.nchunks);
}
static int fam16_default_pipe(const lp_engine*, const Op& op) { return (op.stride == 2 ? PIPE16_S2A : PIPE16_D) + 1; }

static int prepare_op(lp_engine* e, size_t idx) {
    ++e->epoch;
    const Op& op = e->ops[idx];
    Launch& L = e->launches[idx];
    L.is_conv = !(op.kind == OP_INPUT || op.kind == OP_POOL);
    if (!L.is_conv) return LP_OK;
    const int dt = e->dtype;
    auto tptr = [&](int id) { return (void*)(e->arena + e->tensors[id].offset); };
    const int ks = op.kind == OP_CONV ? op.ksize : 1, stv = op.kind == OP_CONV ? op.stride : 1;
    const int cb_pack = conv_shape(dt, op.cfg, ks, stv).CB;
    const ConvShape s = op.pipe ? conv_pipe_shape(op.pipe - 1) : conv_shape(dt, op.cfg, ks, stv);
    ConvArgs& a = L.a;
    memset(&a, 0, sizeof(a));
    a.nsrc = op.nsrc;
    for (int i = 0; i < op.nsrc; ++i) { a.src[i].ptr = tptr(op.src[i]); a.src[i].cs = e->tensors[op.src[i]].cs; }
    for (int i = 0; i <= LP_MAX_SRC; ++i) a.chunk_begin[i] = op.chunk_begin[i];
    a.zero = e->dev_w;
    a.trash = e->dev_w + 128;
    a.w = e->dev_w + op.w_off;
    a.bias = (const float*)(e->dev_w + op.b_off);
    const Tensor& s0 = e->tensors[op.src[0]];
    a.B = e->B;
    a.H = s0.h;
    a.W = s0.w;
    a.Ho = stv == 2 ? s0.h / 2 : s0.h;
    a.Wo = stv == 2 ? s0.w / 2 : s0.w;
    if (op.pipe && pipe_is_16s2(op.pipe - 1)) {
        conv_pick_tile16v(s, a.Ho, a.Wo, e->B, op.nct, op.tile, &a.TH, &a.TW, 2);
        a.hpitch = 2 * a.TW + 1;
    } else if (op.pipe && pipe_is_16v(op.pipe - 1)) {
        conv_pick_tile16v(s, a.Ho, a.Wo, e->B, op.nct, op.tile, &a.TH, &a.TW);
        a.hpitch = a.TW + 2;
    } else {
        conv_pick_tile(s, ks, stv, a.Ho, a.Wo, op.tile, &a.TH, &a.TW);
        a.hpitch = (op.pipe && pipe_is_16(op.pipe - 1)) ? conv_pick_pitch16(s, a.TH, a.TW) : conv_pick_pitch(s, dt, ks, stv, a.TH, a.TW);
    }
    a.tw_magic = (unsigned)(((1u << 22) + a.TW - 1) / a.TW);
    a.hp_magic = (unsigned)(((1u << 22) + a.hpitch - 1) / a.hpitch);
    a.tiles_x = ceil_div(a.Wo, a.TW);
    a.tiles_y = ceil_div(a.Ho, a.TH);
    a.nct = op.nct;
    a.nphase = op.nphase;
    a.w_phase_stride = op.w_phase_stride;
    a.out_scale = op.kind == OP_DECONV ? 2 : 1;
    a.act = op.act;
    a.alpha = op.alpha;
    if (op.mode == MODE_ACT) {
        const Tensor& d = e->tensors[op.dst];
        a.out = tptr(op.dst);
        a.out_c = d.cs;
        a.out_pix_stride = d.cs;
        a.out_img_stride = (long long)d.h * d.w * d.cs;
        if (op.kind == OP_CONV && op.dst2 >= 0) {
            const Tensor& d2 = e->tensors[op.dst2];
            a.out2 = tptr(op.dst2);
            a.out_split = d.cs;
            a.out_c = d.cs + d2.cs;
            a.out2_pix_stride = d2.cs;
            a.out2_img_stride = (long long)d2.h * d2.w * d2.cs;
        }
        if (op.res >= 0) { a.res = tptr(op.res); a.res_cs = e->tensors[op.res].cs; }
    } else {
        a.out = nullptr;
        L.pred_off = (long long)e->level_off[op.level] * LP_PRED_COLS + (op.mode == MODE_PRED ? 13 : 0);
        a.out_pix_stride = LP_PRED_COLS;
        a.out_img_stride = (long long)e->n_anchors * LP_PRED_COLS;
        a.out_c = op.cout;
        if (op.mode == MODE_DECODE) {
            a.reg_bins = op.reg_bins;
            a.proj = op.proj.empty() ? nullptr : (const float*)(e->dev_w + op.proj_off);
            a.stride_px = (float)(8 << op.level);
        }
    }
    a.stamps = g_stamps;
    L.choice() = op;
    L.mode = op.mode;
    L.ks = ks;
    L.st = stv;
    L.cb_pack = cb_pack;
    if (op.planar) {
        Launch& P = e->stem_planar;
        P = L;
        ConvArgs& pa = P.a;
        if (pa.W % 4 != 0 || !stem_planar_tile(pa.Ho, pa.Wo, op.planar - 1, &pa.TH, &pa.TW))
            return fail(LP_ERR_UNSUPPORTED, "planar stem: no tile for this frame size");
        pa.tw_magic = (unsigned)(((1u << 22) + pa.TW - 1) / pa.TW);
        pa.tiles_x = ceil_div(pa.Wo, pa.TW);
        pa.tiles_y = ceil_div(pa.Ho, pa.TH);
        pa.src[0].ptr = nullptr;
        P.pipe = PIPE_P + 1;
    }
    if (op.fused) {
        const Op& stem = e->ops[1];
        Launch& F = e->stem2_fused;
        F = L;
        ConvArgs& fa = F.a;
        if (!stem2_fused_tile(fa.Ho, fa.Wo, op.fused - 1, &fa.TH, &fa.TW, &fa.hpitch))
            return fail(LP_ERR_UNSUPPORTED, "fused stem: no tile for this frame size");
        fa.tw_magic = (unsigned)(((1u << 22) + fa.TW - 1) / fa.TW);
        fa.hp_magic = (unsigned)(((1u << 22) + fa.hpitch - 1) / fa.hpitch);
        fa.tiles_x = ceil_div(fa.Wo, fa.TW);
        fa.tiles_y = ceil_div(fa.Ho, fa.TH);
        fa.src[0].ptr = nullptr;
        fa.fz_w1 = e->dev_w + stem.w_off;
        fa.fz_b1 = (const float*)(e->dev_w + stem.b_off);
        fa.fz_act1 = stem.act;
        fa.fz_c1 = e->tensors[stem.dst].cs;
        F.pipe = PIPE_FUSED2 + 1;
    }
    if (op.fused_bf) {
        const Op& up = e->ops[op.bf_up];
        const Op& c1 = e->ops[op.bf_cv1];
        Launch& F = e->bf_fused[(int)idx];
        F = L;
        ConvArgs& fa = F.a;
        fa.src[0].ptr = tptr(up.src[0]); fa.src[0].cs = e->tensors[up.src[0]].cs;
        fa.src[1].ptr = tptr(c1.src[0]); fa.src[1].cs = e->tensors[c1.src[0]].cs;
        fa.fz_w1 = e->dev_w + c1.w_off;
        fa.fz_b1 = (const float*)(e->dev_w + c1.b_off);
        fa.fz_act1 = c1.act;
        fa.bf_wd = e->dev_w + up.w_off;
        fa.bf_bd = (const float*)(e->dev_w + up.b_off);
        fa.bf_wd_phase_stride = up.w_phase_stride;
        F.pipe = PIPE_FUSED_BF + 1;
    }
    if (op.fused_pw) {
        const Op& pw = e->ops[idx - 1];
        Launch& F = e->pw_fused[(int)idx];
        F = L;
        ConvArgs& fa = F.a;
        int hp = 0;
        if (!stem2_fused_tile(fa.Ho, fa.Wo, op.fused_pw - 1, &fa.TH, &fa.TW, &hp))
            return fail(LP_ERR_UNSUPPORTED, "fused 1x1 + 3x3 s2: no tile for this map size");
        fa.hpitch = hp;
        fa.tw_magic = (unsigned)(((1u << 22) + fa.TW - 1) / fa.TW);
        fa.hp_magic = (unsigned)(((1u << 22) + fa.hpitch - 1) / fa.hpitch);
        fa.tiles_x = ceil_div(fa.Wo, fa.TW);
        fa.tiles_y = ceil_div(fa.Ho, fa.TH);
        fa.src[0].ptr = tptr(pw.src[0]);
        fa.src[0].cs = e->tensors[pw.src[0]].cs;
        fa.fz_w1 = e->dev_w + pw.w_off;
        fa.fz_b1 = (const float*)(e->dev_w + pw.b_off);
        fa.fz_act1 = pw.act;
        fa.fz_c1 = e->tensors[pw.dst].cs;
        F.pipe = PIPE_FUSED_PW + 1;
    }
    return LP_OK;
}

static bool stem_planar_possible(const lp_engine* e) {
    return e->dtype != LP_F32 && e->ops.size() > 1 && e->ops[0].kind == OP_INPUT && e->ops[0].s2d && e->ops[1].kind == OP_CONV &&
           e->ops[1].ksize == 3 && e->ops[1].stride == 1 && e->ops[1].mode == MODE_ACT && e->ops[1].nct == 1 && e->ops[1].nchunks == 1 &&
           (conv_shape(e->dtype, e->ops[1].cfg, 3, 1).CB == 32 || conv_shape(e->dtype, e->ops[1].cfg, 3, 1).CB == 64) && e->ops[1].res < 0 &&
           e->ops[1].dst2 < 0;
}
static bool frame_direct(const lp_engine* e, const void* x, int x_dtype) { return x_dtype == e->dtype && ((uintptr_t)x & 15) == 0; }
static bool stem_planar_now(const lp_engine* e, const void* x, int x_dtype) { return e->ops.size() > 1 && e->ops[1].planar && frame_direct(e, x, x_dtype); }
static bool stem2_fused_possible(const lp_engine* e) {
    if (!stem_planar_possible(e) || e->ops.size() < 3) return false;
    const Op& s = e->ops[1];
    const Op& c = e->ops[2];
    if (c.kind != OP_CONV || c.ksize != 3 || c.stride != 2 || c.nsrc != 1 || c.src[0] != s.dst || c.res >= 0 || c.dst2 >= 0 || c.mode != MODE_ACT ||
        c.nct != 1 || c.nphase != 1 || c.nchunks < 1 || c.nchunks > 2 || s.act != LP_ACT_RELU || c.act != LP_ACT_RELU) return false;
    const int cb = conv_shape(e->dtype, c.cfg, 3, 2).CB, cs2 = e->tensors[c.dst].cs;
    if ((cb != 32 && cb != 64) || cb != 32 * ((cs2 + 31) / 32) || e->tensors[s.dst].cs > 16 * c.nchunks) return false;
    for (size_t i = 3; i < e->ops.size(); ++i) {
        const Op& o = e->ops[i];
        for (int k = 0; k < o.nsrc; ++k) if (o.src[k] == s.dst) return false;
        if (o.res == s.dst) return false;
    }
    return true;
}
static bool pw_fused_possible(const lp_engine* e, size_t i) {
    if (e->dtype == LP_F32 || i < 2 || i >= e->ops.size()) return false;
    const Op& p = e->ops[i - 1];
    const Op& c = e->ops[i];
    if (c.kind != OP_CONV || c.ksize != 3 || c.stride != 2 || c.nsrc != 1 || c.res >= 0 || c.dst2 >= 0 || c.mode != MODE_ACT || c.nct != 1 || c.nphase != 1) return false;
    if (p.kind != OP_CONV || p.ksize != 1 || p.stride != 1 || p.nsrc != 1 || p.res >= 0 || p.dst2 >= 0 || p.mode != MODE_ACT || p.nct != 1 || p.nphase != 1 ||
        p.nchunks != 1 || p.dst != c.src[0] || p.lane != c.lane || p.signal) return false;
    const int cs0 = e->tensors[p.src[0]].cs, cs1 = e->tensors[p.dst].cs, cs2 = e->tensors[c.dst].cs;
    if (cs0 != 64 || (cs1 != 32 && cs1 != 64) || (cs2 != 32 && cs2 != 64)) return false;
    if (conv_shape(e->dtype, p.cfg, 1, 1).CB != cs1 || conv_shape(e->dtype, c.cfg, 3, 2).CB != cs2 || c.nchunks != cs1 / 16) return false;
    for (size_t k = 0; k < e->ops.size(); ++k) {
        if (k == i) continue;
        const Op& o = e->ops[k];
        for (int q = 0; q < o.nsrc; ++q) if (o.src[q] == p.dst) return false;
        if (o.res == p.dst) return false;
    }
    return true;
}
static bool bifusion_fused_possible(const lp_engine* e, size_t i, int* up, int* cv1) {
    if (e->dtype == LP_F32 || i >= e->ops.size()) return false;
    const Op& c = e->ops[i];
    if (c.kind != OP_CONV || c.ksize != 1 || c.stride != 1 || c.nsrc != 3 || c.res >= 0 || c.dst2 >= 0 || c.mode != MODE_ACT || c.nct != 1 || c.nphase != 1 ||
        c.nchunks != 3 || c.act != LP_ACT_RELU || conv_shape(e->dtype, c.cfg, 1, 1).CB != 64 || e->tensors[c.dst].cs != 64) return false;
    int ju = -1, ja = -1;
    for (size_t k = 0; k < i; ++k) {
        if (e->ops[k].kind == OP_DECONV && e->ops[k].dst == c.src[0]) ju = (int)k;
        if (e->ops[k].kind == OP_CONV && e->ops[k].dst == c.src[1]) ja = (int)k;
    }
    if (ju < 0 || ja < 0) return false;
    const Op& u = e->ops[ju];
    const Op& p = e->ops[ja];
    if (u.nsrc != 1 || u.nct != 1 || u.nphase != 4 || u.nchunks != 1 || u.act != LP_ACT_NONE ||
        conv_shape(e->dtype, u.cfg, 1, 1).CB != 64 || e->tensors[u.src[0]].cs != 64 || e->tensors[u.dst].cs != 64) return false;
    if (p.ksize != 1 || p.stride != 1 || p.nsrc != 1 || p.res >= 0 || p.dst2 >= 0 || p.mode != MODE_ACT || p.nct != 1 || p.nphase != 1 || p.nchunks != 2 ||
        p.act != LP_ACT_RELU || conv_shape(e->dtype, p.cfg, 1, 1).CB != 64 || e->tensors[p.src[0]].cs != 128 ||
        e->tensors[p.dst].cs != 64 || e->tensors[c.src[2]].cs != 64) return false;
    const Tensor& tf = e->tensors[c.dst];
    const Tensor& tc = e->tensors[u.src[0]];
    if (tf.h != 2 * tc.h || tf.w != 2 * tc.w) return false;
    for (size_t k = 0; k < e->ops.size(); ++k) {
        if (k == i) continue;
        const Op& o = e->ops[k];
        for (int q = 0; q < o.nsrc; ++q) if (o.src[q] == u.dst || o.src[q] == p.dst) return false;
        if (o.res == u.dst || o.res == p.dst) return false;
    }
    if (up) *up = ju;
    if (cv1) *cv1 = ja;
    return true;
}
static bool stem2_fused_now(const lp_engine* e, const void* x, int x_dtype) { return e->ops.size() > 2 && e->ops[2].fused && frame_direct(e, x, x_dtype); }

struct DetCtx {
    NmsWs w;
    float conf;
};

static int run_head_det(lp_engine* e, size_t idx, const DetCtx& dc, hipStream_t st) {
    const Op& op = e->ops[idx];
    const Launch& L = e->launches[idx];
    const int dt = e->dtype;
    ConvArgs a = L.a;
    const int anchor0 = e->level_off[op.level], N = e->n_anchors;
    if (L.mode == MODE_DECODE) {
        a.det_mode = 1;
        a.out = dc.w.rows + (long long)anchor0 * LP_DET_COLS;
        a.out_pix_stride = LP_DET_COLS;
        a.out_img_stride = (long long)N * LP_DET_COLS;
        static const bool no_box_stream = getenv("LP_NO_BOX_STREAM") != nullptr;
        static const bool no_box_sparse = getenv("LP_NO_BOX_SPARSE") != nullptr;
        const bool snap_ok = !no_box_sparse && e->box_sparse_ok && (e->n_lanes <= 1 || e->single_lane) && e->box_ord[idx] >= 0 && N >= 8;
        auto streams = [&](size_t j) { const Launch& Lj = e->launches[j]; return !no_box_stream && head_box_det_fits(Lj.a, Lj.cb_pack, Lj.ks, Lj.st); };
        if (streams(idx)) {
            if (snap_ok) {
                const int k = e->box_ord[idx];
                int* const snaps = dc.w.kept;
                a.det_cnt = dc.w.cnt;
                a.det_np = dc.w.NP;
                a.det_snap = snaps + (size_t)k * e->B;
                bool prev_snap = k == 0;
                for (size_t j = 0; j < idx && !prev_snap; ++j) prev_snap = e->box_ord[j] == k - 1 && streams(j);
                if (op.box_sparse && prev_snap) {
                    a.det_keys = dc.w.keys;
                    a.det_n = N;
                    a.det_anchor0 = anchor0;
                    a.det_prev = k > 0 ? snaps + (size_t)(k - 1) * e->B : nullptr;
                }
            }
            return head_box_det_launch(dt, a, L.cb_pack, st);
        }
        return conv_launch(dt, L.cfg, L.mode, L.ks, L.st, L.nbuf, a, st);
    }
    if (op.det_scratch == (size_t)-1) {
        a.det_mode = 1;
        a.out = dc.w.rows;
        a.det_keys = dc.w.keys;
        a.det_cnt = dc.w.cnt;
        a.det_np = dc.w.NP;
        a.det_n = N;
        a.det_anchor0 = anchor0;
        a.det_conf = dc.conf;
        return head_rows_launch(dt, a, L.cb_pack, st);
    }
    float* const scratch = (float*)(e->arena + op.det_scratch);
    const int rpi = a.Ho * a.Wo;
    a.out = scratch + 13;
    a.out_img_stride = (long long)rpi * LP_PRED_COLS;
    int rc = conv_launch(dt, L.cfg, L.mode, L.ks, L.st, L.nbuf, a, st);
    if (rc) return rc;
    return nms_score_launch(scratch, e->B, rpi, anchor0, N, dc.conf, dc.w, false, st);
}

static int run_op(lp_engine* e, size_t idx, const void* x, int x_dtype, float* pred, hipStream_t st, const DetCtx* det = nullptr) {
    const Op& op = e->ops[idx];
    const int dt = e->dtype;
    auto tptr = [&](int id) { return (void*)(e->arena + e->tensors[id].offset); };
    if (op.kind == OP_INPUT) {
        if (op.s2d && (stem_planar_now(e, x, x_dtype) || stem2_fused_now(e, x, x_dtype))) return LP_OK;
        return op.s2d ? input_s2d_launch(x, x_dtype, tptr(op.dst), dt, e->B, e->H, e->W, st)
                      : input_launch(x, x_dtype, tptr(op.dst), dt, e->B, e->H, e->W, st);
    }
    if (op.kind == OP_POOL) {
        const Tensor& t = e->tensors[op.src[0]];
        return pool_launch(tptr(op.src[0]), tptr(op.dst), tptr(op.dst2), tptr(op.dst3), dt, e->B, t.h, t.w, t.cs, st);
    }
    const Launch& L = e->launches[idx];
    if (idx + 1 < e->ops.size() && e->ops[idx + 1].fused_pw) return LP_OK;
    if (op.bf_carrier >= 0 && e->ops[op.bf_carrier].fused_bf) return LP_OK;
    if (op.fused_bf) return conv_pipe_launch(dt, PIPE_FUSED_BF, e->bf_fused[(int)idx].a, st);
    if (op.fused_pw) return conv_pipe_launch(dt, PIPE_FUSED_PW, e->pw_fused[(int)idx].a, st);
    if (idx == 1 && stem2_fused_now(e, x, x_dtype)) return LP_OK;
    if (idx == 2 && stem2_fused_now(e, x, x_dtype)) {
        ConvArgs a = e->stem2_fused.a;
        a.src[0].ptr = x;
        return conv_pipe_launch(dt, PIPE_FUSED2, a, st);
    }
    if (idx == 1 && op.planar && stem_planar_now(e, x, x_dtype)) {
        ConvArgs a = e->stem_planar.a;
        a.src[0].ptr = x;
        return conv_pipe_launch(dt, PIPE_P, a, st);
    }
    if (L.mode == MODE_ACT && L.pipe) return conv_pipe_launch(dt, L.pipe - 1, L.a, st);
    if (L.mode == MODE_ACT && L.stream_wc) return conv_stream_launch(dt, L.stream_wc, L.a, L.cb_pack, st);
    if (L.mode == MODE_ACT) return conv_launch(dt, L.cfg, L.mode, L.ks, L.st, L.nbuf, L.a, st);
    if (det) return run_head_det(e, idx, *det, st);
    if (!pred) return fail(LP_ERR_ARG, "forward: pred is null");
    ConvArgs a = L.a;
    a.out = pred + L.pred_off;
    if (L.mode == MODE_PRED && L.rows) return head_rows_launch(dt, a, L.cb_pack, st);
    return conv_launch(dt, L.cfg, L.mode, L.ks, L.st, L.nbuf, a, st);
}

static int check_ready(const lp_engine* e, const void* x, int x_dtype) {
    if (!e || !e->finalized) return fail(LP_ERR_STATE, "forward: engine not finalized");
    if (!e->dev_w) return fail(LP_ERR_STATE, "forward: weights not uploaded");
    if (!e->arena) return fail(LP_ERR_STATE, "forward: arena not bound");
    if (!x) return fail(LP_ERR_ARG, "forward: x is null");
    if (x_dtype != LP_F16 && x_dtype != LP_BF16 && x_dtype != LP_F32) return fail(LP_ERR_ARG, "forward: x dtype");
    return LP_OK;
}

static int ensure_lanes(lp_engine* e) {
    for (int l = 1; l < e->n_lanes; ++l)
        if (!e->lane_stream[l]) LP_HIP_CHECK(hipStreamCreateWithFlags(&e->lane_stream[l], hipStreamNonBlocking));
    if (!e->fork_ev) LP_HIP_CHECK(hipEventCreateWithFlags(&e->fork_ev, hipEventDisableTiming));
    for (int l = 1; l < e->n_lanes; ++l)
        if (!e->join_ev[l]) LP_HIP_CHECK(hipEventCreateWithFlags(&e->join_ev[l], hipEventDisableTiming));
    if (e->op_event.size() != e->ops.size()) e->op_event.assign(e->ops.size(), nullptr);
    for (size_t i = 0; i < e->ops.size(); ++i)
        if (e->ops[i].signal && !e->op_event[i]) LP_HIP_CHECK(hipEventCreateWithFlags(&e->op_event[i], hipEventDisableTiming));
    return LP_OK;
}

static int issue_forward(lp_engine* e, const void* x, int x_dtype, float* pred, hipStream_t main_st, const DetCtx* det = nullptr) {
    int rc;
    if (e->n_lanes <= 1 || e->single_lane) {
        for (size_t i = 0; i < e->ops.size(); ++i) {
            rc = run_op(e, i, x, x_dtype, pred, main_st, det);
            if (rc) return rc;
        }
        return LP_OK;
    }
    rc = ensure_lanes(e);
    if (rc) return rc;
    e->lane_stream[0] = main_st;
    LP_HIP_CHECK(hipEventRecord(e->fork_ev, main_st));
    for (int l = 1; l < e->n_lanes; ++l) LP_HIP_CHECK(hipStreamWaitEvent(e->lane_stream[l], e->fork_ev, 0));
    for (size_t i = 0; i < e->ops.size(); ++i) {
        const Op& op = e->ops[i];
        hipStream_t st = e->lane_stream[op.lane];
        for (int d : op.deps) LP_HIP_CHECK(hipStreamWaitEvent(st, e->op_event[d], 0));
        rc = run_op(e, i, x, x_dtype, pred, st, det);
        if (rc) return rc;
        if (op.signal) LP_HIP_CHECK(hipEventRecord(e->op_event[i], st));
    }
    for (int l = 1; l < e->n_lanes; ++l) {
        LP_HIP_CHECK(hipEventRecord(e->join_ev[l], e->lane_stream[l]));
        LP_HIP_CHECK(hipStreamWaitEvent(main_st, e->join_ev[l], 0));
    }
    return LP_OK;
}

extern "C" int lp_engine_set_single_lane(lp_engine* e, int enable) {
    if (!e) return fail(LP_ERR_ARG, "lp_engine_set_single_lane: null engine");
    if (e->single_lane != (enable != 0)) ++e->epoch;
    e->single_lane = enable != 0;
    return LP_OK;
}

extern "C" int lp_engine_set_mfma16(lp_engine* e, int enable) {
    if (!e) return fail(LP_ERR_ARG, "lp_engine_set_mfma16: null engine");
    if (e->finalized) return fail(LP_ERR_STATE, "lp_engine_set_mfma16: the families are fixed by lp_engine_finalize");
    e->mfma16 = enable != 0;
    return LP_OK;
}

extern "C" int lp_engine_set_graph(lp_engine* e, int enable) {
    if (!e) return fail(LP_ERR_ARG, "lp_engine_set_graph: null engine");
    e->use_graph = enable != 0;
    return LP_OK;
}

static int mark_done(lp_engine* e, hipStream_t st) {
    if (!e->done_ev) LP_HIP_CHECK(hipEventCreateWithFlags(&e->done_ev, hipEventDisableTiming | hipEventDisableSystemFence));
    LP_HIP_CHECK(hipEventRecord(e->done_ev, st));
    e->done_valid = true;
    return LP_OK;
}

static int run_forward(lp_engine* e, const void* x, int x_dtype, float* pred, const DetCtx* det, void* ws, hipStream_t main_st) {
    int rc;
    auto issue = [&](hipStream_t st) -> int {
        if (det) { if (int zr = zero_counts_launch(det->w.cnt, e->B, st)) return zr; }
        return issue_forward(e, x, x_dtype, pred, st, det);
    };
    if (!e->use_graph) {
        rc = issue(main_st);
        return rc ? rc : mark_done(e, main_st);
    }
    constexpr size_t kMaxGraphs = 8;
    const float conf = det ? det->conf : 0.f;
    lp_engine::CachedGraph* hit = nullptr;
    for (auto& g : e->graphs)
        if (g.exec && g.x == x && g.pred == pred && g.ws == ws && g.conf == conf && g.x_dtype == x_dtype && g.epoch == e->epoch) hit = &g;
    if (!hit) {
        for (size_t i = 0; i < e->graphs.size();) {
            auto& g = e->graphs[i];
            bool drop = g.epoch != e->epoch;
            if (!drop && e->graphs.size() >= kMaxGraphs) {
                drop = true;
                for (const auto& o : e->graphs) drop = drop && o.last_use >= g.last_use;
            }
            if (!drop) { ++i; continue; }
            if (g.stream) (void)hipStreamSynchronize(g.stream);
            if (g.exec) (void)hipGraphExecDestroy(g.exec);
            e->graphs.erase(e->graphs.begin() + (long)i);
        }
        rc = ensure_lanes(e);
        if (rc) return rc;
        hipGraph_t g = nullptr;
        if (!e->cap_stream) LP_HIP_CHECK(hipStreamCreateWithFlags(&e->cap_stream, hipStreamNonBlocking));
        LP_HIP_CHECK(hipStreamBeginCapture(e->cap_stream, hipStreamCaptureModeThreadLocal));
        rc = issue(e->cap_stream);
        hipError_t ce = hipStreamEndCapture(e->cap_stream, &g);
        if (rc) { if (g) (void)hipGraphDestroy(g); return rc; }
        if (ce != hipSuccess) return fail(LP_ERR_HIP, std::string("hipStreamEndCapture: ") + hipGetErrorString(ce));
        lp_engine::CachedGraph cg;
        ce = hipGraphInstantiate(&cg.exec, g, nullptr, nullptr, 0);
        (void)hipGraphDestroy(g);
        if (ce != hipSuccess) return fail(LP_ERR_HIP, std::string("hipGraphInstantiate: ") + hipGetErrorString(ce));
        cg.x = x;
        cg.pred = pred;
        cg.ws = ws;
        cg.conf = conf;
        cg.x_dtype = x_dtype;
        cg.epoch = e->epoch;
        e->graphs.push_back(cg);
        hit = &e->graphs.back();
    }
    LP_HIP_CHECK(hipGraphLaunch(hit->exec, main_st));
    hit->stream = main_st;
    hit->last_use = ++e->graph_clock;
    return mark_done(e, main_st);
}

extern "C" int lp_engine_forward(lp_engine* e, const void* x, int x_dtype, float* pred, void* stream) {
    int rc = check_ready(e, x, x_dtype);
    if (rc) return rc;
    if (!pred) return fail(LP_ERR_ARG, "forward: pred is null");
    return run_forward(e, x, x_dtype, pred, nullptr, nullptr, (hipStream_t)stream);
}

extern "C" int lp_engine_forward_det(lp_engine* e, const void* x, int x_dtype, double conf_thres, void* workspace, size_t workspace_bytes,
                                     void* stream) {
    int rc = check_ready(e, x, x_dtype);
    if (rc) return rc;
    if (!workspace || ((uintptr_t)workspace & 255)) return fail(LP_ERR_ARG, "lp_engine_forward_det: need a 256-byte aligned workspace");
    if (!(conf_thres >= 0.0 && conf_thres <= 1.0)) return fail(LP_ERR_ARG, "lp_engine_forward_det: conf_thres must be in [0, 1]");
    DetCtx dc;
    dc.w = nms_carve(workspace, e->B, e->n_anchors);
    dc.conf = (float)conf_thres;
    if (workspace_bytes < dc.w.bytes) return fail(LP_ERR_ARG, "lp_engine_forward_det: workspace too small (lp_nms_workspace_bytes)");
    return run_forward(e, x, x_dtype, nullptr, &dc, workspace, (hipStream_t)stream);
}

static int forward_single_lane(lp_engine* e, const void* x, int x_dtype, float* pred, hipStream_t st) {
    for (size_t i = 0; i < e->ops.size(); ++i) {
        int rc = run_op(e, i, x, x_dtype, pred, st);
        if (rc) return rc;
    }
    return LP_OK;
}

extern "C" int lp_engine_profile_ops(lp_engine* e, const void* x, int x_dtype, float* pred, void* stream, float* op_ms, int reps,
                                     int inner) {
    int rc = check_ready(e, x, x_dtype);
    if (rc) return rc;
    if (!op_ms || reps < 1 || inner < 1) return fail(LP_ERR_ARG, "profile: op_ms / reps / inner");
    hipStream_t st = (hipStream_t)stream;
    const size_t n = e->ops.size();
    while (e->events.size() < n + 1) {
        hipEvent_t ev;
        LP_HIP_CHECK(hipEventCreate(&ev));
        e->events.push_back(ev);
    }
    rc = forward_single_lane(e, x, x_dtype, pred, (hipStream_t)stream);
    if (rc) return rc;
    for (size_t i = 0; i < n; ++i) op_ms[i] = 0.f;
    for (int r = 0; r < reps; ++r) {
        LP_HIP_CHECK(hipEventRecord(e->events[0], st));
        for (size_t i = 0; i < n; ++i) {
            for (int k = 0; k < inner; ++k) {
                rc = run_op(e, i, x, x_dtype, pred, st);
                if (rc) return rc;
            }
            LP_HIP_CHECK(hipEventRecord(e->events[i + 1], st));
        }
        LP_HIP_CHECK(hipEventSynchronize(e->events[n]));
        for (size_t i = 0; i < n; ++i) {
            float ms = 0.f;
            LP_HIP_CHECK(hipEventElapsedTime(&ms, e->events[i], e->events[i + 1]));
            op_ms[i] += ms / reps / inner;
        }
    }
    return LP_OK;
}

extern "C" int lp_engine_profile(lp_engine* e, const void* x, int x_dtype, float* pred, void* stream, float* op_ms, int reps) {
    return lp_engine_profile_ops(e, x, x_dtype, pred, stream, op_ms, reps, 1);
}

extern "C" int lp_engine_autotune(lp_engine* e, const void* x, int x_dtype, float* pred, void* stream, int reps) {
    int rc = check_ready(e, x, x_dtype);
    if (rc) return rc;
    if (reps < 1) reps = 3;
    hipStream_t st = (hipStream_t)stream;
    for (Op& op : e->ops) { op.planar = 0; op.fused = 0; op.fused_pw = 0; op.fused_bf = 0; }
    rc = forward_single_lane(e, x, x_dtype, pred, st);
    if (rc) return rc;
    struct EventPair {
        hipEvent_t a = nullptr, b = nullptr;
        ~EventPair() { if (a) (void)hipEventDestroy(a); if (b) (void)hipEventDestroy(b); }
    } evp;
    LP_HIP_CHECK(hipEventCreate(&evp.a));
    LP_HIP_CHECK(hipEventCreate(&evp.b));
    const hipEvent_t e0 = evp.a, e1 = evp.b;
    int trc = LP_OK;
    auto time_best = [&](std::initializer_list<size_t> seq) -> float {
        float ms_min = -1.f;
        for (int round = 0; round < 3 && trc == LP_OK; ++round) {
            float ms = 0.f;
            if (hipEventRecord(e0, st) != hipSuccess) { trc = LP_ERR_HIP; break; }
            for (int r = 0; r < reps; ++r)
                for (size_t k : seq) run_op(e, k, x, x_dtype, pred, st);
            if (hipEventRecord(e1, st) != hipSuccess || hipEventSynchronize(e1) != hipSuccess || hipEventElapsedTime(&ms, e0, e1) != hipSuccess) { trc = LP_ERR_HIP; break; }
            if (ms_min < 0.f || ms < ms_min) ms_min = ms;
        }
        return trc ? -1.f : ms_min;
    };
    auto time_current = [&](size_t i) -> float { return run_op(e, i, x, x_dtype, pred, st) == LP_OK ? time_best({i}) : -1.f; };
    auto walk_tiles = [&](size_t i, float* best) -> int {
        int bias = 0, won = -1, last_th = -1, last_tw = -1;
        const Launch* L = nullptr;
        int* const slot = op_tile_slot(e, (int)i, &bias, &L);
        for (int tile = 0; tile < 3 && slot && trc == LP_OK; ++tile) {
            *slot = tile + bias;
            if (prepare_op(e, i) != LP_OK) continue;
            if (L->a.TH == last_th && L->a.TW == last_tw) break;
            last_th = L->a.TH;
            last_tw = L->a.TW;
            const float ms = time_current(i);
            if (ms >= 0.f && (*best < 0.f || ms < *best)) { *best = ms; won = tile; }
        }
        return won;
    };
    auto try_form = [&](size_t i, int& form, float t_sep, bool tiled) -> int {
        float t_form = -1.f;
        int won = -1;
        if (trc == LP_OK) {
            form = 1;
            if (tiled) won = walk_tiles(i, &t_form);
            else if (prepare_op(e, i) == LP_OK && (t_form = time_current(i)) >= 0.f) won = 0;
        }
        if (trc) return fail(trc, "autotune: event timing failed");
        form = (won >= 0 && t_form < t_sep) ? won + 1 : 0;
        return prepare_op(e, i);
    };
    for (size_t i = 0; i < e->ops.size(); ++i) {
        Op& op = e->ops[i];
        if (e->launches[i].is_conv && op.kind == OP_HEAD_CLS && rows_fits(e, op) && !getenv("LP_NO_HEAD_ROWS")) {
            float best = -1.f;
            int best_rows = 0;
            for (int rows = 0; rows <= 1; ++rows) {
                op.rows = rows;
                if (prepare_op(e, i) != LP_OK) continue;
                const float ms = time_current(i);
                if (ms >= 0.f && (best < 0.f || ms < best)) { best = ms; best_rows = rows; }
            }
            if (trc) return fail(trc, "autotune: event timing failed");
            op.rows = best_rows;
            rc = prepare_op(e, i);
            if (rc) return rc;
            continue;
        }
        if (!e->launches[i].is_conv || op.mode != MODE_ACT) continue;
        const int cb = conv_shape(e->dtype, op.cfg, 1, 1).CB;
        int best_cfg = op.cfg, best_nb = op.nbuf, best_tile = op.tile, best_wc = 0, best_rd = 2, best_pipe = 0;
        float best_ms = -1.f;
        op.stream_wc = 0;
        op.pipe = 0;
        const bool fam16 = op_fam16(e, op);
        for (int cfg = 0; cfg < CFG_COUNT && !fam16; ++cfg) {
            if (conv_shape(e->dtype, cfg, 1, 1).CB != cb) continue;
            for (int nb = 1; nb <= (cfg == CFG_C ? 1 : 2); ++nb) {
                op.cfg = cfg;
                op.nbuf = nb;
                const int tile = walk_tiles(i, &best_ms);
                if (tile >= 0) { best_cfg = cfg; best_nb = nb; best_tile = tile; }
            }
        }
        if (!getenv("LP_NO_STREAM") && !fam16) {
            op.cfg = best_cfg; op.nbuf = best_nb; op.tile = best_tile;
            for (int wc = 2; wc <= 4; wc += 2) {
                if (!stream_fits(e, op, wc)) continue;
                for (int rd = 2; rd <= 2; ++rd) {
                    op.stream_wc = wc;
                    op.stream_rd = rd;
                    if (prepare_op(e, i) != LP_OK) continue;
                    const float ms = time_current(i);
                    if (ms >= 0.f && (best_ms < 0.f || ms < best_ms)) { best_ms = ms; best_wc = wc; best_rd = rd; }
                }
            }
        }
        int pipe_tile = 0;
        if ((!getenv("LP_NO_PIPE") || fam16) && op.kind == OP_CONV) {
            op.cfg = best_cfg; op.nbuf = best_nb; op.stream_wc = 0;
            for (int pc = fam16 ? PIPE16_D : 0; pc < (fam16 ? PIPE_S2_END : PIPE_COUNT); ++pc) {
                if (fam16 && !pipe_is_16(pc)) continue;
                if (!conv_pipe_fits(e->dtype, pc, cb, op.ksize, op.stride, op.mode, op.nct, op.nphase, op.nchunks)) continue;
                op.pipe = pc + 1;
                const int tile = walk_tiles(i, &best_ms);
                if (tile >= 0) { best_pipe = pc + 1; pipe_tile = tile; }
            }
            op.pipe = 0;
            if (fam16 && !best_pipe) best_pipe = fam16_default_pipe(e, op);
        }
        if (trc) return fail(trc, "autotune: event timing failed");
        op.cfg = best_cfg;
        op.nbuf = best_nb;
        op.tile = best_pipe ? pipe_tile : best_tile;
        op.stream_wc = best_pipe ? 0 : best_wc;
        op.stream_rd = best_rd;
        op.pipe = best_pipe;
        op.planar = 0;
        op.fused = 0;
        op.fused_pw = 0;
        rc = prepare_op(e, i);
        if (rc) return rc;
        if (i == 1 && stem_planar_possible(e) && frame_direct(e, x, x_dtype) && !getenv("LP_NO_PLANAR")) {
            const float t_in = time_best({0});
            rc = try_form(i, op.planar, best_ms + t_in, true);
            if (rc) return rc;
        }
        if (i == 2 && stem2_fused_possible(e) && frame_direct(e, x, x_dtype) && !getenv("LP_NO_PLANAR") && !getenv("LP_NO_FUSED_STEM")) {
            rc = try_form(i, op.fused, time_best({0, 1, 2}), true);
            if (rc) return rc;
        }
        if (pw_fused_possible(e, i) && !getenv("LP_NO_FUSED_PW")) {
            rc = try_form(i, op.fused_pw, time_best({i - 1, i}), true);
            if (rc) return rc;
        }
        if (op.bf_up >= 0 && !getenv("LP_NO_FUSED_BF")) {
            rc = try_form(i, op.fused_bf, time_best({(size_t)op.bf_up, (size_t)op.bf_cv1, i}), false);
            if (rc) return rc;
        }
    }
    e->tuned[{e->B, e->H, e->W}].assign(e->ops.begin(), e->ops.end());
    return LP_OK;
}

extern "C" int lp_engine_copy_tuning(lp_engine* dst, const lp_engine* src) {
    if (!dst || !src || !dst->finalized || !src->finalized) return fail(LP_ERR_STATE, "lp_engine_copy_tuning: finalize both engines first");
    if (dst->dtype != src->dtype || dst->ops.size() != src->ops.size()) return fail(LP_ERR_ARG, "lp_engine_copy_tuning: engines differ");
    for (size_t i = 0; i < src->ops.size(); ++i) {
        const Op &a = src->ops[i], &b = dst->ops[i];
        if (a.kind != b.kind || a.ksize != b.ksize || a.stride != b.stride || a.cout != b.cout || a.nchunks != b.nchunks || a.nct != b.nct)
            return fail(LP_ERR_ARG, "lp_engine_copy_tuning: engines were built from different graphs");
    }
    dst->tuned = src->tuned;
    if (dst->arena && apply_tuned(dst))
        for (size_t i = 0; i < dst->ops.size(); ++i) {
            int rc = prepare_op(dst, i);
            if (rc) return rc;
        }
    return LP_OK;
}

extern "C" int lp_engine_set_op_variant(lp_engine* e, int op_idx, int cfg, int nbuf) {
    if (!e || !e->finalized || op_idx < 0 || op_idx >= (int)e->ops.size()) return fail(LP_ERR_ARG, "lp_engine_set_op_variant: op index");
    Op& op = e->ops[op_idx];
    if (op.kind == OP_HEAD_CLS) {
        if (cfg == LP_VARIANT_ROWS && !rows_fits(e, op)) return fail(LP_ERR_UNSUPPORTED, "lp_engine_set_op_variant: the row-writer kernel does not fit this op");
        if (cfg != LP_VARIANT_ROWS && cfg != op.cfg) return fail(LP_ERR_UNSUPPORTED, "lp_engine_set_op_variant: head_cls takes LP_VARIANT_ROWS or its packing tile");
        op.rows = cfg == LP_VARIANT_ROWS;
        e->tuned.erase({e->B, e->H, e->W});
        if (e->arena && op_idx < (int)e->launches.size()) return prepare_op(e, (size_t)op_idx);
        return LP_OK;
    }
    if (op.kind == OP_HEAD_BOX && (cfg == LP_VARIANT_BOX_SPARSE || cfg == LP_VARIANT_BOX_DENSE)) {
        op.box_sparse = cfg == LP_VARIANT_BOX_SPARSE;
        ++e->epoch;
        return LP_OK;
    }
    if (op.kind == OP_INPUT || op.kind == OP_POOL || op.mode != MODE_ACT) return fail(LP_ERR_UNSUPPORTED, "lp_engine_set_op_variant: op has no variants");
    const int ks = op.kind == OP_CONV ? op.ksize : 1, stv = op.kind == OP_CONV ? op.stride : 1;
    const int cb = conv_shape(e->dtype, op.cfg, ks, stv).CB;
    const Choice before = op;
    auto commit = [&]() -> int {
        if (e->arena && op_idx < (int)e->launches.size()) {
            const int rc = prepare_op(e, (size_t)op_idx);
            if (rc) {
                op.choice() = before;
                const std::string why = g_err;
                prepare_op(e, (size_t)op_idx);
                return fail(rc, why);
            }
        }
        e->tuned.erase({e->B, e->H, e->W});
        return LP_OK;
    };
    if (cfg == LP_VARIANT_FUSED_BIFUSION) {
        if (op.bf_up < 0 || nbuf != 3) return fail(LP_ERR_UNSUPPORTED, "lp_engine_set_op_variant: not the cv3 of a 64-channel BiFusion level");
        op.fused_bf = 1;
        return commit();
    }
    if (cfg == LP_VARIANT_FUSED_PW_S2) {
        if (!pw_fused_possible(e, (size_t)op_idx) || nbuf != 3)
            return fail(LP_ERR_UNSUPPORTED, "lp_engine_set_op_variant: no 1x1 layer of at most 64 channels feeds this 3x3 stride-2 layer alone");
        op.fused_bf = 0;
        op.fused_pw = 1;
        return commit();
    }
    if (cfg == LP_VARIANT_FUSED_STEM2) {
        if (op_idx != 2 || !stem2_fused_possible(e) || nbuf != 3)
            return fail(LP_ERR_UNSUPPORTED, "lp_engine_set_op_variant: only the layer behind the stem (3x3 stride 2, <= 64 channels) has the fused form");
        op.fused_bf = op.fused_pw = 0;
        op.fused = 1;
        return commit();
    }
    if (cfg == LP_VARIANT_PIPE_D + PIPE_P) {
        if (op_idx != 1 || !stem_planar_possible(e) || nbuf != 3)
            return fail(LP_ERR_UNSUPPORTED, "lp_engine_set_op_variant: only the stem over the space-to-depth image has the planar form");
        op.fused_bf = op.fused_pw = op.fused = 0;
        op.planar = 1;
        return commit();
    }
    if ((cfg >= LP_VARIANT_PIPE_D && cfg < LP_VARIANT_PIPE_D + PIPE_COUNT) || pipe_is_16(cfg - LP_VARIANT_PIPE_D)) {
        const int pc = cfg - LP_VARIANT_PIPE_D;
        if (!conv_pipe_fits(e->dtype, pc, cb, ks, stv, op.mode, op.nct, op.nphase, op.nchunks) || op.kind != OP_CONV || nbuf != 3)
            return fail(LP_ERR_UNSUPPORTED, "lp_engine_set_op_variant: the pipelined 3x3 kernel does not fit this op");
        op.stream_wc = 0;
        op.pipe = pc + 1;
    } else if (cfg == LP_VARIANT_STREAM64 || cfg == LP_VARIANT_STREAM128) {
        const int wc = cfg == LP_VARIANT_STREAM64 ? 2 : 4;
        if (!stream_fits(e, op, wc) || nbuf != 2)
            return fail(LP_ERR_UNSUPPORTED, "lp_engine_set_op_variant: the streaming 1x1 kernel does not fit this op");
        op.stream_wc = wc;
        op.stream_rd = nbuf;
        op.pipe = 0;
    } else {
        if (cfg < 0 || cfg >= CFG_COUNT || conv_shape(e->dtype, cfg, ks, stv).CB != cb || nbuf < 1 || nbuf > (cfg == CFG_C ? 1 : 2))
            return fail(LP_ERR_UNSUPPORTED, "lp_engine_set_op_variant: variant does not share the op's weight packing");
        op.stream_wc = 0;
        op.pipe = 0;
        op.cfg = cfg;
        op.nbuf = nbuf;
    }
    op.fused_bf = op.fused_pw = op.fused = op.planar = 0;
    return commit();
}

static int* op_tile_slot(lp_engine* e, int op_idx, int* bias, const Launch** L) {
    Op& op = e->ops[(size_t)op_idx];
    if (op.kind == OP_INPUT || op.kind == OP_POOL || op.mode != MODE_ACT || op.fused_bf) return nullptr;
    const bool bound = e->arena && op_idx < (int)e->launches.size();
    *bias = 1;
    if (op.fused_pw) { *L = bound ? &e->pw_fused[op_idx] : nullptr; return &op.fused_pw; }
    if (op.fused) { *L = bound ? &e->stem2_fused : nullptr; return &op.fused; }
    if (op.planar) { *L = bound ? &e->stem_planar : nullptr; return &op.planar; }
    if (op.stream_wc && !op.pipe) return nullptr;
    *bias = 0;
    *L = bound ? &e->launches[(size_t)op_idx] : nullptr;
    return &op.tile;
}

extern "C" int lp_engine_set_op_tile(lp_engine* e, int op_idx, int choice) {
    if (!e || !e->finalized || op_idx < 0 || op_idx >= (int)e->ops.size() || choice < 0) return fail(LP_ERR_ARG, "lp_engine_set_op_tile: op index or choice");
    int bias = 0;
    const Launch* L = nullptr;
    int* slot = op_tile_slot(e, op_idx, &bias, &L);
    if (!slot) return fail(LP_ERR_UNSUPPORTED, "lp_engine_set_op_tile: the op's kernel has no output tiles");
    const Choice before = e->ops[op_idx];
    *slot = choice + bias;
    e->tuned.erase({e->B, e->H, e->W});
    if (e->arena && op_idx < (int)e->launches.size()) {
        const int rc = prepare_op(e, (size_t)op_idx);
        if (rc) { e->ops[op_idx].choice() = before; prepare_op(e, (size_t)op_idx); }
        return rc;
    }
    return LP_OK;
}

extern "C" int lp_engine_op_tile(const lp_engine* e, int op_idx, int* choice, int* TH, int* TW) {
    if (!e || !e->finalized || op_idx < 0 || op_idx >= (int)e->ops.size()) return fail(LP_ERR_ARG, "lp_engine_op_tile: op index");
    int bias = 0;
    const Launch* L = nullptr;
    const int* slot = op_tile_slot(const_cast<lp_engine*>(e), op_idx, &bias, &L);
    if (!slot) return fail(LP_ERR_UNSUPPORTED, "lp_engine_op_tile: the op's kernel has no output tiles");
    if (!L) return fail(LP_ERR_STATE, "lp_engine_op_tile: no shape bound");
    if (choice) *choice = *slot - bias;
    if (TH) *TH = L->a.TH;
    if (TW) *TW = L->a.TW;
    return LP_OK;
}

extern "C" int lp_engine_op_carrier(const lp_engine* e, int op, int frame_direct_) {
    if (!e || op < 0 || op >= (int)e->ops.size()) return -1;
    const Op& o = e->ops[(size_t)op];
    if (o.bf_carrier >= 0 && e->ops[(size_t)o.bf_carrier].fused_bf) return o.bf_carrier;
    if ((size_t)op + 1 < e->ops.size() && e->ops[(size_t)op + 1].fused_pw) return op + 1;
    if (frame_direct_ && e->ops.size() > 2 && e->ops[0].kind == OP_INPUT && e->ops[0].s2d) {
        if (e->ops[2].fused && op <= 1) return 2;
        if (e->ops[1].planar && op == 0) return 1;
    }
    return -1;
}

extern "C" int lp_engine_op_io(const lp_engine* e, int op, int* src, int* n_src, int* res, int* dst) {
    if (!e || !e->finalized || op < 0 || op >= (int)e->ops.size()) return fail(LP_ERR_ARG, "lp_engine_op_io: engine not finalized, or op index");
    const Op& o = e->ops[(size_t)op];
    if (src) for (int k = 0; k < LP_MAX_SRC; ++k) src[k] = k < o.nsrc ? o.src[k] : -1;
    if (n_src) *n_src = o.nsrc;
    if (res) *res = o.res;
    if (dst) { dst[0] = o.dst; dst[1] = o.dst2; dst[2] = o.dst3; }
    return LP_OK;
}

extern "C" int lp_engine_op_variant(const lp_engine* e, int op, int* cfg, int* nbuf) {
    if (!e || op < 0 || op >= (int)e->ops.size()) return fail(LP_ERR_ARG, "lp_engine_op_variant: op index");
    const bool stream = e->ops[op].stream_wc != 0;
    if (e->ops[op].fused_bf) {
        if (cfg) *cfg = LP_VARIANT_FUSED_BIFUSION;
        if (nbuf) *nbuf = 3;
        return LP_OK;
    }
    if (e->ops[op].fused_pw) {
        if (cfg) *cfg = LP_VARIANT_FUSED_PW_S2;
        if (nbuf) *nbuf = 3;
        return LP_OK;
    }
    if (e->ops[op].fused) {
        if (cfg) *cfg = LP_VARIANT_FUSED_STEM2;
        if (nbuf) *nbuf = 3;
        return LP_OK;
    }
    if (e->ops[op].planar) {
        if (cfg) *cfg = LP_VARIANT_PIPE_D + PIPE_P;
        if (nbuf) *nbuf = 3;
        return LP_OK;
    }
    if (e->ops[op].pipe) {
        if (cfg) *cfg = LP_VARIANT_PIPE_D + e->ops[op].pipe - 1;
        if (nbuf) *nbuf = 3;
        return LP_OK;
    }
    if (cfg) *cfg = e->ops[op].rows ? LP_VARIANT_ROWS : stream ? (e->ops[op].stream_wc == 2 ? LP_VARIANT_STREAM64 : LP_VARIANT_STREAM128) : e->ops[op].cfg;
    if (nbuf) *nbuf = stream ? e->ops[op].stream_rd : e->ops[op].nbuf;
    return LP_OK;
}
```

### yolo-lp_amd/csrc/lp_head_box.inc

```
#pragma once
#include "lp_conv_kernel.inc"

namespace lp {

template <typename T, int NCH, bool SPARSE>
__global__ __launch_bounds__(256) void head_box_det_kernel(const ConvArgs a, const int cb_pack, const int gpi) {
    typedef typename Mma<T>::V V;
    constexpr int SZ = sizeof(T), EPG = 16 / SZ, ROWB = 128, NKB = 4, GPR = 8, NK = NCH * NKB;
    const int lane = threadIdx.x & 63, wave = threadIdx.x >> 6;
    const int r = lane & 31, h = lane >> 5;
    const int HW = a.Ho * a.Wo;
    const long long M = (long long)a.B * HW;
    long long ntiles = (M + 31) / 32;
    long long t0 = (long long)blockIdx.x * 4 + wave, tstride = (long long)gridDim.x * 4;
    [[maybe_unused]] int sb = 0, slo = 0, sn = 0;
    if constexpr (SPARSE) {
        sb = blockIdx.x / gpi;
        const int gi = blockIdx.x - sb * gpi;
        int hi = a.det_cnt[sb];
        hi = hi > a.det_np ? a.det_np : hi;
        slo = a.det_prev ? a.det_prev[sb] : 0;
        slo = slo < 0 ? 0 : (slo > hi ? hi : slo);
        sn = hi - slo;
        if (gi == 0 && threadIdx.x == 0) a.det_snap[sb] = hi;
        ntiles = (sn + 31) / 32;
        t0 = (long long)gi * 4 + wave;
        tstride = (long long)gpi * 4;
    } else if (a.det_snap) {
        const int b = blockIdx.x * 256 + threadIdx.x;
        if (b < a.B) { const int c = a.det_cnt[b]; a.det_snap[b] = c > a.det_np ? a.det_np : c; }
    }
    if (t0 >= ntiles) return;

    V wa[NK];
#pragma unroll
    for (int k = 0; k < NK; ++k)
        wa[k] = *(const V*)((const char*)a.w + ((long long)(k / NKB) * cb_pack + r) * ROWB + swz(r, 2 * (k % NKB) + h, GPR) * 16);
    f32x16 bias;
#pragma unroll
    for (int rg = 0; rg < 4; ++rg)
#pragma unroll
        for (int j = 0; j < 4; ++j) bias[4 * rg + j] = a.bias[8 * rg + 4 * h + j];
    const char* const src = (const char*)a.src[0].ptr;
    const int cs = a.src[0].cs;
    const int ngran = cs / EPG;
    const float sp = a.stride_px;

    for (long long t = t0; t < ntiles; t += tstride) {
        long long m = t * 32 + r;
        bool live = m < M;
        if constexpr (SPARSE) {
            live = m < sn;
            const unsigned long long key = a.det_keys[(long long)sb * a.det_np + slo + (live ? m : 0)];
            const int n_ = (int)(unsigned)key - a.det_anchor0;
            live = live && n_ >= 0 && n_ < HW;
            m = (long long)sb * HW + (live ? n_ : 0);
        }
        const char* const row = src + (live ? m : M - 1) * (long long)cs * SZ + h * 16;
        V vb[NK];
#pragma unroll
        for (int k = 0; k < NK; ++k) vb[k] = *(const V*)(2 * k + h < ngran ? row + k * 32 : (const char*)a.zero);
        __builtin_amdgcn_sched_barrier(0);
        f32x16 acc = bias;
#pragma unroll
        for (int k = 0; k < NK; ++k) acc = Mma<T>::mma(wa[k], vb[k], acc);
        if (!live) continue;
        const int b = (int)(m / HW), n = (int)(m - (long long)b * HW);
        const int oy = n / a.Wo, ox = n - oy * a.Wo;
        const float ax = (float)ox + 0.5f, ay = (float)oy + 0.5f;
        float* const o = (float*)a.out + (long long)b * a.out_img_stride + (long long)n * a.out_pix_stride;
        if (h == 0) {
            const float x1 = ax - acc[0], y1 = ay - acc[1], x2 = ax + acc[2], y2 = ay + acc[3];
            const float cx = ((x1 + x2) / 2.f) * sp, cy = ((y1 + y2) / 2.f) * sp, bw = (x2 - x1) * sp, bh = (y2 - y1) * sp;
            const f32x4 v0 = {cx - bw / 2, cy - bh / 2, cx + bw / 2, cy + bh / 2};
            const f32x4 v2 = {(ax + acc[4]) * sp, (ay + acc[5]) * sp, (ax + acc[6]) * sp, (ay - acc[7]) * sp};
            *(f32x4*)o = v0;
            *(f32x4*)(o + 8) = v2;
        } else {
            const f32x4 v1 = {(ax - acc[0]) * sp, (ay - acc[1]) * sp, (ax - acc[2]) * sp, (ay + acc[3]) * sp};
            *(f32x4*)(o + 4) = v1;
        }
    }
}

template <typename T, int NCH>
static inline int head_box_det_launch_one(const ConvArgs& a, int cb_pack, hipStream_t st) {
    const long long ntiles = ((long long)a.B * a.Ho * a.Wo + 31) / 32;
    long long grid = (ntiles + 3) / 4;
    if (grid > 2048) grid = 2048;
    if (a.det_keys) {
        long long gpi = (ntiles / a.B + 3) / 4;
        const long long cap = 2048 / a.B;
        if (gpi > cap) gpi = cap;
        if (gpi < 1) gpi = 1;
        hipLaunchKernelGGL((head_box_det_kernel<T, NCH, true>), dim3((unsigned)(gpi * a.B)), dim3(256), 0, st, a, cb_pack, (int)gpi);
    } else
    hipLaunchKernelGGL((head_box_det_kernel<T, NCH, false>), dim3((unsigned)grid), dim3(256), 0, st, a, cb_pack, 1);
    hipError_t e = hipGetLastError();
    if (e != hipSuccess) return fail(LP_ERR_HIP, std::string("head box launch: ") + hipGetErrorString(e));
    return LP_OK;
}

template <typename T>
static inline int head_box_det_launch_dtype(const ConvArgs& a, int cb_pack, hipStream_t st) {
    switch (a.chunk_begin[a.nsrc]) {
        case 1: return head_box_det_launch_one<T, 1>(a, cb_pack, st);
        case 2: return head_box_det_launch_one<T, 2>(a, cb_pack, st);
        case 3: return head_box_det_launch_one<T, 3>(a, cb_pack, st);
        case 4: return head_box_det_launch_one<T, 4>(a, cb_pack, st);
    }
    return fail(LP_ERR_UNSUPPORTED, "head box: more than four K-chunks");
}

}
```

### yolo-lp_amd/csrc/lp_internal.h

```cpp
#pragma once
#include <hip/hip_runtime.h>
#include <stdint.h>
#include <stddef.h>
#include <atomic>
#include <string>

#include "../../include/lp_hip.h"

#ifndef LP_PRO_ORDER
#define LP_PRO_ORDER 0
#endif

namespace lp {

typedef _Float16 f16;
typedef __bf16 bf16;

void set_error(const std::string& msg);
int fail(int code, const std::string& msg);
#define LP_HIP_CHECK(expr)                                                                       \
    do {                                                                                         \
        hipError_t _e = (expr);                                                                  \
        if (_e != hipSuccess)                                                                    \
            return ::lp::fail(LP_ERR_HIP, std::string(#expr) + ": " + hipGetErrorString(_e));    \
    } while (0)

template <typename K> inline int set_max_lds_once(K kernel, int bytes, std::atomic<unsigned long long>& done, const char* what) {
    int dev = 0;
    if (hipGetDevice(&dev) != hipSuccess || dev < 0 || dev >= 64) dev = -1;
    if (dev >= 0 && ((done.load(std::memory_order_acquire) >> dev) & 1ull)) return LP_OK;
    hipError_t e = hipFuncSetAttribute((const void*)kernel, hipFuncAttributeMaxDynamicSharedMemorySize, bytes);
    if (e != hipSuccess) return fail(LP_ERR_HIP, std::string(what) + ": LDS attribute: " + hipGetErrorString(e));
    if (dev >= 0) done.fetch_or(1ull << dev, std::memory_order_release);
    return LP_OK;
}

__device__ __forceinline__ void resize_coef(int d, double scale, int src, int* s0, int* a0, int* a1) {
    float f = (float)((d + 0.5) * scale - 0.5);
    int s = (int)floorf(f);
    f -= (float)s;
    if (s < 0) { f = 0.f; s = 0; }
    if (s >= src - 1) { f = 0.f; s = src - 1; }
    *s0 = s;
    const float c0 = (1.f - f) * 2048.f, c1 = f * 2048.f;
    *a0 = (int)rintf(c0);
    *a1 = (int)rintf(c1);
}
__device__ __forceinline__ int resize_blend(int t00, int t01, int t10, int t11, int a0, int a1, int b0, int b1) {
    const int h0v = t00 * a0 + t01 * a1;
    const int h1v = t10 * a0 + t11 * a1;
    return (((b0 * (h0v >> 4)) >> 16) + ((b1 * (h1v >> 4)) >> 16) + 2) >> 2;
}
constexpr int LETTERBOX_PAD = 114;

std::string plane_fault(const unsigned char* y, const unsigned char* uv, int pitch_y, int pitch_uv, int h0, int w0, int matrix);

inline size_t dtype_size(int dt) { return dt == LP_F32 ? 4 : 2; }
inline int round_up(int x, int m) { return (x + m - 1) / m * m; }
inline int ceil_div(int a, int b) { return (a + b - 1) / b; }

enum ConvMode { MODE_ACT = 0, MODE_PRED = 1, MODE_DECODE = 2 };
enum ConvCfg { CFG_A = 0 , CFG_B = 1 , CFG_C = 2 , CFG_D = 3 , CFG_E = 4 , CFG_F = 5 , CFG_COUNT = 6 };

enum PipeCfgId { PIPE_D = 0 , PIPE_B = 1 , PIPE_F = 2 , PIPE_C = 3 , PIPE_P = 4 , PIPE_COUNT = 5,
                 PIPE_FUSED2 = 5 ,
                 PIPE_FUSED_PW = 6 ,
                 PIPE_FUSED_BF = 13 ,
                 PIPE16_D = 7, PIPE16_F = 9 ,
                 PIPE16_V0 = 10, PIPE16_V1 = 11 , PIPE_END = 12,
                 PIPE16_S2A = 16, PIPE16_S2B = 17 , PIPE_S2_END = 18 };
inline bool pipe_is_16s2(int pcfg) { return pcfg == PIPE16_S2A || pcfg == PIPE16_S2B; }
inline bool pipe_is_16(int pcfg) { return pcfg == PIPE16_D || pcfg == PIPE16_F || pcfg == PIPE16_V0 || pcfg == PIPE16_V1 || pipe_is_16s2(pcfg); }
inline bool pipe_is_16v(int pcfg) { return pcfg == PIPE16_V0 || pcfg == PIPE16_V1; }

struct ConvSrc {
    const void* ptr;
    int cs;
};

struct ConvArgs {
    ConvSrc src[LP_MAX_SRC];
    int chunk_begin[LP_MAX_SRC + 1];
    int nsrc;
    const void* w;
    const float* bias;
    unsigned long long* stamps;
    const void* zero;
    void* trash;
    void* out;
    void* out2;
    int out_split;
    int out2_pix_stride;
    long long out2_img_stride;
    const void* res;
    int res_cs;
    float alpha;
    int B, H, W;
    int Ho, Wo;
    int TH, TW, tiles_x, tiles_y;
    unsigned tw_magic, hp_magic;
    int hpitch;
    int nct;
    int out_c;
    long long out_img_stride;
    int out_pix_stride;
    int out_scale;
    int nphase;
    long long w_phase_stride;
    int act;
    int det_mode;
    unsigned long long* det_keys;
    int* det_cnt;
    int det_np, det_n, det_anchor0;
    float det_conf;
    const int* det_prev;
    int* det_snap;
    const void* fz_w1;
    const float* fz_b1;
    int fz_act1, fz_c1;
    const void* bf_wd;
    const float* bf_bd;
    long long bf_wd_phase_stride;
    int reg_bins;
    const float* proj;
    float stride_px;
};

struct ConvShape {
    int CB, PB, KC, HPMAX, NT, WP, WGC, WGP;
};
ConvShape conv_shape(int dtype, int cfg, int ksize, int stride);
void conv_pick_tile(const ConvShape& s, int ksize, int stride, int Ho, int Wo, int choice, int* TH, int* TW);
int conv_pick_pitch(const ConvShape& s, int dtype, int ksize, int stride, int TH, int TW);
int conv_pick_pitch16(const ConvShape& s, int TH, int TW);
void conv_pick_tile16v(const ConvShape& s, int Ho, int Wo, int B, int nct, int choice, int* TH, int* TW, int stride = 1);
int device_cus();
int conv_launch(int dtype, int cfg, int mode, int ksize, int stride, int nbuf, const ConvArgs& a, hipStream_t st);
bool stem_planar_tile(int Ho, int Wo, int choice, int* TH, int* TW);
bool stem2_fused_tile(int Ho, int Wo, int choice, int* TH, int* TW, int* hpitch);

int conv_stream_lds(int dtype, int wc, int nchunks, int cb_pack);
int conv_stream_launch(int dtype, int wc, const ConvArgs& a, int cb_pack, hipStream_t st);

ConvShape conv_pipe_shape(int pcfg);
bool conv_pipe_fits(int dtype, int pcfg, int cb_pack, int ksize, int stride, int mode, int nct, int nphase, int nchunks);
int conv_pipe_launch(int dtype, int pcfg, const ConvArgs& a, hipStream_t st);

bool head_rows_fits(int dtype, int nchunks, int cb_pack, int out_c);
bool head_det_fits(int dtype, int nchunks, int cb_pack, int out_c);
bool head_box_det_fits(const ConvArgs& a, int cb_pack, int ksize, int stride);
int head_box_det_launch(int dtype, const ConvArgs& a, int cb_pack, hipStream_t st);
int head_rows_launch(int dtype, const ConvArgs& a, int cb_pack, hipStream_t st);

struct NmsWs {
    int32_t* cnt;
    unsigned long long* keys;
    float* rows;
    float4* sbox;
    int32_t* kept;
    int NP;
    size_t bytes;
};
NmsWs nms_carve(void* base, int B, int N);
int nms_score_launch(float* pred, int B, int rows_per_img, int anchor0, int N, float conf_f, const NmsWs& w, bool write_box, hipStream_t st);
int zero_counts_launch(int* p, int n, hipStream_t st);

int input_launch(const void* x, int x_dtype, void* dst, int dtype, int B, int H, int W, hipStream_t st);
int input_s2d_launch(const void* x, int x_dtype, void* dst, int dtype, int B, int H, int W, hipStream_t st);
size_t pool_min_lds_bytes(int dtype, int h, int w);
constexpr size_t POOL_MAX_LDS = 128 * 1024;
int pool_launch(const void* src, void* d1, void* d2, void* d3, int dtype, int B, int h, int w, int cs, hipStream_t st);

}
```

### yolo-lp_amd/yolov6/hip/abi.py

```python
import ctypes
import os
from ctypes import POINTER, c_char_p, c_double, c_float, c_int, c_int32, c_size_t, c_void_p

LP_F16, LP_BF16, LP_F32 = 0, 1, 2
LP_ACT_NONE, LP_ACT_RELU, LP_ACT_SILU = 0, 1, 2
LP_PRED_COLS, LP_DET_COLS, LP_MAX_SRC = 290, 28, 4
LP_VARIANT_STREAM64, LP_VARIANT_STREAM128, LP_VARIANT_ROWS = 16, 17, 18
LP_VARIANT_PIPE_D, LP_VARIANT_PIPE_B, LP_VARIANT_PIPE_F, LP_VARIANT_PIPE_C = 32, 33, 34, 35
LP_VARIANT_PIPE16_D, LP_VARIANT_PIPE16_F = 39, 41
LP_VARIANT_PIPE16_V0, LP_VARIANT_PIPE16_V1 = 42, 43
LP_VARIANT_PIPE16_S2A, LP_VARIANT_PIPE16_S2B = 48, 49
LP_VARIANT_FUSED_BIFUSION = 45
LP_VARIANT_BOX_SPARSE, LP_VARIANT_BOX_DENSE = 46, 47
LP_VARIANT_FUSED_PW_S2 = 38
LP_VARIANT_FUSED_STEM2 = 37
LP_VARIANT_PIPE_P = 36
VARIANT_SHORT = {
    LP_VARIANT_STREAM64: 'S', LP_VARIANT_STREAM128: 'W', LP_VARIANT_ROWS: 'R',
    LP_VARIANT_PIPE_D: 'Pd', LP_VARIANT_PIPE_B: 'Pb', LP_VARIANT_PIPE_F: 'Pf', LP_VARIANT_PIPE_C: 'Pc', LP_VARIANT_PIPE_P: 'Pp',
    LP_VARIANT_FUSED_STEM2: 'Fz', LP_VARIANT_FUSED_PW_S2: 'Fp', LP_VARIANT_FUSED_BIFUSION: 'Fb',
    LP_VARIANT_PIPE16_D: 'Md', LP_VARIANT_PIPE16_F: 'Mf', LP_VARIANT_PIPE16_V0: 'V0', LP_VARIANT_PIPE16_V1: 'V1',
    LP_VARIANT_PIPE16_S2A: 'Xa', LP_VARIANT_PIPE16_S2B: 'Xb',
}
LP_FRAMES_PER_LAUNCH = 64
LP_NV12_PER_LAUNCH = 32
LP_MERGE_MAX_TILES, LP_MERGE_MAX_CANDIDATES = 64, 16384
LP_TRACK_MAX_TRACKS, LP_TRACK_MAX_DETS, LP_TRACK_MAX_CLS = 128, 128, 64
LP_REDACT_MAX_CELL = 64
LP_REDACT_MAX_RADIUS = 48
LP_JPEG_MAX_RESTART, LP_JPEG_PER_LAUNCH = 32, 32
LP_LOOKBACK_MAX_DEPTH = 32
LP_WATCH_MAX_ENTRIES, LP_WATCH_MAX_COST = 1 << 24, 32768
LP_WATCH_BLOCK_ENTRIES, LP_WATCH_QUERY_BLOCK = 2048, 16
LP_SIGHT_MAX_CAPACITY = 1 << 24
LP_SIGHT_BLOCK_ENTRIES, LP_SIGHT_QUERY_BLOCK = 1024, 16
LP_TILE_GATE_TILE_WORDS = 8
LP_EVAL_NCOUNTS = 43

_PKG_ROOT = os.path.dirname(os.path.dirname(os.path.dirname(os.path.abspath(__file__))))
LIB_PATH = os.environ.get('LP_HIP_LIB') or os.path.join(_PKG_ROOT, 'libyololp_hip.so')
CSRC_DIR = os.path.join(_PKG_ROOT, 'csrc')


class FrameDesc(ctypes.Structure):
    _fields_ = [('img', c_void_p), ('h0', c_int), ('w0', c_int), ('rh', c_int), ('rw', c_int), ('top', c_int), ('left', c_int)]


class RescaleDesc(ctypes.Structure):
    _fields_ = [('ratio', c_double), ('padx', c_double), ('pady', c_double), ('img_w', c_int), ('img_h', c_int)]


class CropDesc(ctypes.Structure):
    _fields_ = [('img', c_void_p), ('h0', c_int), ('w0', c_int), ('max_crops', c_int), ('out_slot', c_int)]


class TileDesc(ctypes.Structure):
    _fields_ = [('img', c_void_p), ('h0', c_int), ('w0', c_int), ('y0', c_int), ('x0', c_int), ('th', c_int), ('tw', c_int),
                ('rh', c_int), ('rw', c_int), ('top', c_int), ('left', c_int)]


class Nv12Desc(ctypes.Structure):
    _fields_ = [('y', c_void_p), ('uv', c_void_p), ('pitch_y', c_int), ('pitch_uv', c_int), ('h0', c_int), ('w0', c_int),
                ('y0', c_int), ('x0', c_int), ('th', c_int), ('tw', c_int), ('rh', c_int), ('rw', c_int), ('top', c_int),
                ('left', c_int), ('matrix', c_int)]


class Nv12BgrDesc(ctypes.Structure):
    _fields_ = [('y', c_void_p), ('uv', c_void_p), ('pitch_y', c_int), ('pitch_uv', c_int), ('h0', c_int), ('w0', c_int),
                ('matrix', c_int), ('out', c_void_p)]


class RedactDesc(ctypes.Structure):
    _fields_ = [('p0', c_void_p), ('p1', c_void_p), ('pitch0', c_int), ('pitch1', c_int), ('h0', c_int), ('w0', c_int),
                ('format', c_int)]


class RedactParams(ctypes.Structure):
    _fields_ = [('mode', c_int), ('cell', c_int), ('margin', c_double), ('fill', ctypes.c_ubyte * 3)]


class RedactGaussParams(ctypes.Structure):
    _fields_ = [('margin', c_double), ('radius', c_int), ('radius_c', c_int), ('taps', ctypes.c_uint16 * (LP_REDACT_MAX_RADIUS + 1)),
                ('taps_c', ctypes.c_uint16 * (LP_REDACT_MAX_RADIUS + 1))]


class JpegDesc(ctypes.Structure):
    _fields_ = [('p0', c_void_p), ('p1', c_void_p), ('pitch0', c_int), ('pitch1', c_int), ('h0', c_int), ('w0', c_int),
                ('format', c_int), ('matrix', c_int)]


class JpegParams(ctypes.Structure):
    _fields_ = [('quality', c_int), ('restart', c_int)]


class TileGateDesc(ctypes.Structure):
    _fields_ = [('p0', c_void_p), ('pitch0', c_int), ('h0', c_int), ('w0', c_int), ('format', c_int), ('blocks', c_void_p)]


class TileRef(ctypes.Structure):
    _fields_ = [('frame', c_int), ('y0', c_int), ('x0', c_int), ('th', c_int), ('tw', c_int)]


class TrackParams(ctypes.Structure):
    _fields_ = [('match_thres', c_double), ('new_thres', c_double), ('expand', c_double), ('max_age', c_int), ('ncls', c_int * 8)]


class TrackHoldParams(ctypes.Structure):
    _fields_ = [('min_hits', c_int), ('max_misses', c_int)]


class StackParams(ctypes.Structure):
    _fields_ = [('min_score', c_double), ('min_width', c_double), ('min_sharp', ctypes.c_ulonglong), ('search', c_int),
                ('max_frames', c_int)]


class ConvDesc(ctypes.Structure):
    _fields_ = [('n_src', c_int), ('src', c_int * LP_MAX_SRC), ('dst', c_int), ('ksize', c_int), ('stride', c_int),
                ('act', c_int), ('res', c_int), ('res_alpha', c_float), ('weight', c_void_p), ('bias', c_void_p), ('dst2', c_int)]


SYMBOLS = {
    'lp_version': (c_char_p, []),
    'lp_last_error': (c_char_p, []),
    'lp_engine_create': (c_int, [POINTER(c_void_p), c_int]),
    'lp_engine_destroy': (None, [c_void_p]),
    'lp_engine_tensor': (c_int, [c_void_p, c_int, c_int]),
    'lp_engine_set_lane': (c_int, [c_void_p, c_int]),
    'lp_engine_add_input': (c_int, [c_void_p, c_int]),
    'lp_engine_add_conv': (c_int, [c_void_p, POINTER(ConvDesc)]),
    'lp_engine_add_deconv2x2': (c_int, [c_void_p, c_int, c_int, c_void_p, c_void_p]),
    'lp_engine_add_pool5_chain': (c_int, [c_void_p, c_int, c_int, c_int, c_int]),
    'lp_engine_add_head_cls': (c_int, [c_void_p, c_int, c_int, c_int, c_void_p, c_void_p]),
    'lp_engine_add_head_box': (c_int, [c_void_p, c_int, c_int, c_int, c_void_p, c_void_p, c_void_p]),
    'lp_engine_finalize': (c_int, [c_void_p, c_int]),
    'lp_engine_weight_bytes': (c_size_t, [c_void_p]),
    'lp_engine_upload': (c_int, [c_void_p, c_void_p, c_void_p]),
    'lp_engine_arena_bytes': (c_size_t, [c_void_p, c_int, c_int, c_int]),
    'lp_engine_bind': (c_int, [c_void_p, c_void_p, c_size_t, c_int, c_int, c_int]),
    'lp_engine_tensor_info': (c_int, [c_void_p, c_int, POINTER(c_size_t), POINTER(c_int), POINTER(c_int),
                                      POINTER(c_int), POINTER(c_int)]),
    'lp_engine_num_anchors': (c_int, [c_void_p]),
    'lp_engine_forward': (c_int, [c_void_p, c_void_p, c_int, c_void_p, c_void_p]),
    'lp_engine_set_graph': (c_int, [c_void_p, c_int]),
    'lp_engine_set_single_lane': (c_int, [c_void_p, c_int]),
    'lp_engine_set_mfma16': (c_int, [c_void_p, c_int]),
    'lp_engine_op_carrier': (c_int, [c_void_p, c_int, c_int]),
    'lp_engine_op_io': (c_int, [c_void_p, c_int, POINTER(c_int), POINTER(c_int), POINTER(c_int), POINTER(c_int)]),
    'lp_engine_num_ops': (c_int, [c_void_p]),
    'lp_engine_op_info': (c_int, [c_void_p, c_int, POINTER(c_int), POINTER(c_int), POINTER(c_int), POINTER(c_int),
                                  POINTER(c_double), POINTER(c_double)]),
    'lp_engine_forward_det': (c_int, [c_void_p, c_void_p, c_int, ctypes.c_double, c_void_p, c_size_t, c_void_p]),
    'lp_nms_candidates': (c_int, [c_int, c_int, ctypes.c_double, c_int, c_void_p, c_void_p, c_void_p, c_void_p, c_size_t, c_void_p]),
    'lp_engine_profile': (c_int, [c_void_p, c_void_p, c_int, c_void_p, c_void_p, POINTER(c_float), c_int]),
    'lp_engine_profile_ops': (c_int, [c_void_p, c_void_p, c_int, c_void_p, c_void_p, POINTER(c_float), c_int, c_int]),
    'lp_engine_autotune': (c_int, [c_void_p, c_void_p, c_int, c_void_p, c_void_p, c_int]),
    'lp_engine_op_variant': (c_int, [c_void_p, c_int, POINTER(c_int), POINTER(c_int)]),
    'lp_engine_set_op_variant': (c_int, [c_void_p, c_int, c_int, c_int]),
    'lp_engine_set_op_tile': (c_int, [c_void_p, c_int, c_int]),
    'lp_engine_op_tile': (c_int, [c_void_p, c_int, POINTER(c_int), POINTER(c_int), POINTER(c_int)]),
    'lp_engine_copy_tuning': (c_int, [c_void_p, c_void_p]),
    'lp_nms_workspace_bytes': (c_size_t, [c_int, c_int]),
    'lp_nms_candidate_counts': (c_void_p, [c_void_p, c_int, c_int]),
    'lp_preprocess_letterbox': (c_int, [c_void_p, c_int, c_int, c_void_p, c_int, c_int, c_int, c_int, c_int, c_int, c_int,
                                        c_void_p]),
    'lp_rescale_round': (c_int, [c_void_p, c_int, c_double, c_double, c_double, c_int, c_int, c_void_p]),
    'lp_preprocess_letterbox_batch': (c_int, [POINTER(FrameDesc), c_int, c_int, c_void_p, c_int, c_int, c_int, c_void_p]),
    'lp_rescale_round_batch': (c_int, [c_void_p, c_void_p, c_int, c_int, POINTER(RescaleDesc), c_void_p]),
    'lp_preprocess_tiles_batch': (c_int, [POINTER(TileDesc), c_int, c_int, c_void_p, c_int, c_int, c_int, c_void_p]),
    'lp_preprocess_nv12_batch': (c_int, [POINTER(Nv12Desc), c_int, c_int, c_void_p, c_int, c_int, c_int, c_void_p]),
    'lp_nv12_to_bgr_batch': (c_int, [POINTER(Nv12BgrDesc), c_int, c_void_p]),
    'lp_merge_tiles_workspace_bytes': (c_size_t, [c_int, c_int]),
    'lp_merge_tiles': (c_int, [c_void_p, c_void_p, POINTER(TileRef), c_int, c_int, POINTER(c_int), c_int, c_double, c_int, c_int, c_int,
                               c_void_p, c_void_p, c_void_p, c_void_p, c_size_t, c_void_p]),
    'lp_track_state_bytes': (c_size_t, [c_int, c_int]),
    'lp_track_dropped_offset': (c_size_t, [c_int, c_int]),
    'lp_track_update': (c_int, [c_void_p, c_int, c_int, POINTER(TrackParams), c_void_p, c_void_p, c_int, c_int, POINTER(c_int),
                                c_void_p, c_void_p, c_void_p, c_void_p, c_void_p, c_void_p, c_int, c_void_p]),
    'lp_track_update_slots': (c_int, [c_void_p, c_int, c_int, POINTER(TrackParams), c_void_p, c_void_p, c_int, c_int, POINTER(c_int),
                                      c_void_p, c_void_p, c_void_p, c_void_p, c_void_p, c_void_p, c_void_p, c_int, c_void_p]),
    'lp_track_update_hold': (c_int, [c_void_p, c_int, c_int, POINTER(TrackParams), c_void_p, c_void_p, c_int, c_int, POINTER(c_int),
                                     c_void_p, c_void_p, c_void_p, c_void_p, c_void_p, c_void_p, c_void_p, c_int,
                                     POINTER(TrackHoldParams), c_void_p, c_void_p, c_void_p, c_void_p]),
    'lp_plate_crops_batch': (c_int, [POINTER(CropDesc), c_int, c_void_p, c_void_p, c_int, c_void_p, c_void_p, c_int, c_int, c_int,
                                     c_void_p]),
    'lp_crop_sharpness': (c_int, [c_void_p, c_void_p, c_int, c_int, c_int, c_void_p, c_void_p]),
    'lp_best_shot_state_bytes': (c_size_t, [c_int, c_int, c_int, c_int]),
    'lp_best_shot_update': (c_int, [c_void_p, c_int, c_int, c_int, c_int, c_void_p, c_void_p, c_int, c_int, c_void_p, c_void_p, c_void_p,
                                    c_void_p, c_void_p, c_int, POINTER(c_int), c_void_p, c_void_p, c_int, c_double, c_void_p, c_void_p,
                                    c_void_p, c_void_p, c_void_p]),
    'lp_stack_state_bytes': (c_size_t, [c_int, c_int, c_int, c_int]),
    'lp_stack_update': (c_int, [c_void_p, c_int, c_int, c_int, c_int, c_void_p, c_void_p, c_int, c_int, c_void_p, c_void_p, c_void_p,
                                c_void_p, c_void_p, c_int, POINTER(c_int), c_void_p, c_void_p, c_int, POINTER(StackParams), c_void_p,
                                c_void_p, c_void_p]),
    'lp_redact_workspace_bytes': (c_size_t, [POINTER(RedactDesc), c_int, POINTER(RedactParams)]),
    'lp_redact_plates_batch': (c_int, [POINTER(RedactDesc), c_int, c_void_p, c_void_p, c_int, POINTER(RedactParams), c_void_p, c_void_p,
                                       c_size_t, c_void_p]),
    'lp_redact_gauss_workspace_bytes': (c_size_t, [POINTER(RedactDesc), c_int, POINTER(RedactGaussParams)]),
    'lp_redact_gauss_batch': (c_int, [POINTER(RedactDesc), c_int, c_void_p, c_void_p, c_int, POINTER(RedactGaussParams), c_void_p, c_void_p,
                                      c_size_t, c_void_p]),
    'lp_jpeg_workspace_bytes': (c_size_t, [POINTER(JpegDesc), c_int, c_int]),
    'lp_jpeg_encode_batch': (c_int, [POINTER(JpegDesc), c_int, POINTER(JpegParams), c_void_p, c_int, c_void_p, c_size_t, c_void_p,
                                     c_void_p, c_size_t, c_void_p]),
    'lp_lookback_state_bytes': (c_size_t, [c_int, c_int, c_int, c_int]),
    'lp_lookback_update': (c_int, [c_void_p, c_int, c_int, c_int, c_int, c_int, c_void_p, c_void_p, c_void_p, c_void_p, c_int, c_int, c_int,
                                   POINTER(c_int), c_void_p, c_void_p, c_void_p, c_void_p, c_void_p, c_void_p, c_void_p, c_void_p]),
    'lp_watch_workspace_bytes': (c_size_t, [c_int, c_int]),
    'lp_watch_match': (c_int, [c_void_p, c_int, c_void_p, c_void_p, c_void_p, c_void_p, c_int, c_int, c_int, c_int, c_void_p, c_void_p,
                               c_size_t, c_void_p]),
    'lp_watch_live_state_bytes': (c_size_t, [c_int, c_int]),
    'lp_watch_live_workspace_bytes': (c_size_t, [c_int, c_int]),
    'lp_watch_live': (c_int, [c_void_p, c_int, c_int, POINTER(c_int), c_int, c_void_p, c_void_p, c_int, c_void_p, c_int, c_int, c_void_p,
                              c_void_p, c_void_p, c_void_p, c_void_p, c_void_p, c_size_t, c_void_p]),
    'lp_sight_state_bytes': (c_size_t, [c_int]),
    'lp_sight_workspace_bytes': (c_size_t, [c_int, c_int]),
    'lp_sight_update': (c_int, [c_void_p, c_int, c_void_p, c_void_p, c_void_p, c_void_p, c_void_p, c_int, c_int, c_void_p, c_int, c_int,
                                c_int, c_int, c_void_p, c_void_p, c_size_t, c_void_p]),
    'lp_tile_gate_luma_batch': (c_int, [POINTER(TileGateDesc), c_int, c_void_p]),
    'lp_tile_gate_update': (c_int, [POINTER(TileGateDesc), c_int, POINTER(c_int), c_int, c_void_p, POINTER(c_int), c_int, c_void_p,
                                    ctypes.c_longlong, c_void_p, c_int, c_int, c_int, c_void_p, c_void_p, c_void_p]),
    'lp_tile_gate_update_gain': (c_int, [POINTER(TileGateDesc), c_int, POINTER(c_int), c_int, c_void_p, POINTER(c_int), c_int, c_void_p,
                                         ctypes.c_longlong, c_void_p, c_int, c_int, c_int, c_int, c_int, c_void_p, c_void_p, c_void_p,
                                         c_void_p]),
    'lp_eval_counts': (c_int, [c_void_p, c_void_p, c_int, c_void_p, c_void_p, c_int, c_int, c_void_p, c_void_p]),
    'lp_check_sigmoid_monotone': (c_int, [c_void_p, c_void_p]),
    'lp_debug_poison_lds': (c_int, [c_void_p]),
    'lp_check_iou_predicate': (c_int, [c_void_p, ctypes.c_longlong, c_double, c_void_p, c_void_p]),
    'lp_plan_stem_tile': (c_int, [c_int, c_int, c_int, c_int, c_void_p, c_void_p, c_void_p]),
    'lp_plan_block_tile': (c_int, [c_int, c_int, c_int, c_int, c_int, c_int, c_void_p, c_void_p, c_void_p]),
    'lp_nms': (c_int, [c_void_p, c_int, c_int, c_double, c_double, c_int, c_void_p, c_void_p, c_void_p, c_void_p,
                       c_size_t, c_void_p]),
}

_lib = None


def load():
    global _lib
    if _lib is None:
        import torch
        if not os.path.exists(LIB_PATH):
            raise RuntimeError('HIP extension %s is missing: build it with `make -C %s` (or '
                               '`python -c "import __graft_entry__ as g; g.build()"`). The GPU path has no '
                               'eager fallback.' % (LIB_PATH, CSRC_DIR))
        lib = ctypes.CDLL(LIB_PATH)
        for name, (restype, argtypes) in SYMBOLS.items():
            fn = getattr(lib, name)
            fn.restype = restype
            fn.argtypes = argtypes
        _lib = lib
    return _lib


def check(rc, what=''):
    if rc < 0:
        msg = load().lp_last_error()
        raise RuntimeError('%s failed (%d): %s' % (what or 'libyololp_hip', rc, msg.decode() if msg else '?'))
    return rc
```

### yolo-lp_amd/yolov6/hip/runtime.py

```python
import copy
import ctypes
import os
import weakref

import numpy as np
import torch
import torch.nn as nn

from yolov6.core.frames import letterbox_placement
from yolov6.core.tiles import hw_pair, plan_frames, tiles_per_frame
from yolov6.hip import abi
from yolov6.layers import common as L
from yolov6.utils.lookback import LookbackHost
from yolov6.utils.nv12 import Nv12Frame, is_nv12_list

DET_CROSSOVER = 0.5
_DT = {torch.float16: abi.LP_F16, torch.bfloat16: abi.LP_BF16, torch.float32: abi.LP_F32}
_TORCH_DT = {v: k for k, v in _DT.items()}
CLS_HEADS = ('pro', 'alp', 'ad0', 'ad1', 'ad2', 'ad3', 'ad4', 'ad5')
OP_KINDS = ('input', 'conv', 'deconv', 'pool', 'head_cls', 'head_box', 'stem')


def _dptr(t):
    return None if t is None else ctypes.c_void_p(t.data_ptr())
# ... 213 lines not shown
            c1, y0 = self.cba_pair(m.cv1, m.cv2, [x], sl)
            x1 = self.cba(m.cv4, [self.cba(m.cv3, [c1], sl)], sl)
            y3 = self.cba(m.cv6, [self.cba(m.cv5, [x1] + self.pools(x1, sl, m.cv4.conv.out_channels), sl)], sl)
            return self.cba(m.cv7, [y0, y3], sl)
        if isinstance(m, L._SPPFBase):
            x1 = self.cba(m.cv1, [x], sl)
            return self.cba(m.cv2, [x1] + self.pools(x1, sl, m.cv1.conv.out_channels), sl)
        raise NotImplementedError('%s has no HIP lowering' % type(m).__name__)

    def bifusion(self, m, x0, sl0, x1, x2):
        t = m.upsample.upsample_transpose
        up = self.tensor(t.out_channels, sl0 - 1)
        abi.check(self.lib.lp_engine_add_deconv2x2(self.h, x0, up, self._ptr(_f32(t.weight)), self._ptr(_f32(t.bias))),
                  'lp_engine_add_deconv2x2')
        self.lane(1)
        a = self.cba(m.cv1, [x1], sl0 - 1)
        self.lane(2)
        d = self.cba(m.downsample, [self.cba(m.cv2, [x2], sl0 - 2)], sl0 - 2)
        self.lane(0)
        return self.cba(m.cv3, [up, a, d], sl0 - 1)

    def upsample(self, m, x, sl):
        t = m.upsample_transpose
        up = self.tensor(t.out_channels, sl - 1)
        abi.check(self.lib.lp_engine_add_deconv2x2(self.h, x, up, self._ptr(_f32(t.weight)), self._ptr(_f32(t.bias))),
                  'lp_engine_add_deconv2x2')
        return up

    def _build(self, model):
        bb, nk, det = model.backbone, model.neck, model.detect
        p6 = hasattr(bb, 'ERBlock_6')
        last = 6 if p6 else 5
        x = self.basic(bb.stem, [self.input_id], 0)
        feats = []
        for i in range(2, last + 1):
            st = getattr(bb, 'ERBlock_%d' % i)
            x = self.basic(st[0], [x], i - 1)
            x = self.stage(st[1], [x], i)
            if len(st) > 2:
                x = self.merge_layer(st[2], x, i)
            feats.append(x)
        self.backbone_ops = self.lib.lp_engine_num_ops(self.h)
        bifusion = hasattr(nk, 'Bifusion0')
        has_p2 = bool(getattr(bb, 'fuse_P2', False)) or type(bb).__name__ == 'CSPBepBackbone_P6'
        if bifusion and not has_p2:
            raise NotImplementedError('the BiFusion necks need the P2 output of the backbone (fuse_P2=True)')
        if not bifusion and has_p2:
            raise ValueError('the plain PAN necks take (P3, P4, P5[, P6]): build the backbone with fuse_P2=False')
        nlev = 4 if p6 else 3
        if det.nl != nlev:
            raise ValueError('head with %d levels on a neck with %d outputs' % (det.nl, nlev))
        names_p = ['Rep_p5', 'Rep_p4', 'Rep_p3'] if p6 else ['Rep_p4', 'Rep_p3']
        names_n = ['Rep_n4', 'Rep_n5', 'Rep_n6'] if p6 else ['Rep_n3', 'Rep_n4']
        downs = ['downsample2', 'downsample1', 'downsample0'] if p6 else ['downsample2', 'downsample1']
        x, sl = feats[-1], last
        fpn = []
        for k in range(nlev - 1):
            f = self.cba(getattr(nk, 'reduce_layer%d' % k), [x], sl)
            fpn.append(f)
            if bifusion:
                t = [self.bifusion(getattr(nk, 'Bifusion%d' % k), f, sl, feats[-2 - k], feats[-3 - k])]
            else:
                t = [self.upsample(getattr(nk, 'upsample%d' % k), f, sl), feats[-2 - k]]
            sl -= 1
            x = self.stage(getattr(nk, names_p[k]), t, sl)
        self.neck_ids = [x]
        for k in range(nlev - 1):
            d = self.cba(getattr(nk, downs[k]), [x], sl)
            sl += 1
            x = self.stage(getattr(nk, names_n[k]), [d, fpn[-1 - k]], sl)
            self.neck_ids.append(x)
        for i, f in enumerate(self.neck_ids):
            self._head(det, i, f, (i % 3, (i + 1) % 3))
        self.lane(0)

    def _head(self, det, i, f, lanes):
        sl = 3 + i
        self.lane(lanes[0])
        s = self.cba(det.stems[i], [f], sl)
        c, r = self.cba_pair(det.cls_convs[i], det.reg_convs[i], [s], sl)
        preds = [getattr(det, '%s_preds' % h)[i] for h in CLS_HEADS]
        wc = np.concatenate([_f32(p.weight).reshape(p.out_channels, -1) for p in preds], 0)
        bc = np.concatenate([_f32(p.bias) for p in preds], 0)
        abi.check(self.lib.lp_engine_add_head_cls(self.h, c, i, wc.shape[0], self._ptr(wc), self._ptr(bc)),
                  'lp_engine_add_head_cls')
        self.lane(lanes[1])
        rp, cp = det.reg_preds[i], det.cor_preds[i]
        bins = det.reg_max + 1 if det.use_dfl else 1
        if rp.out_channels != 4 * bins:
            raise NotImplementedError('reg_preds width %d does not match use_dfl/reg_max' % rp.out_channels)
        wb = np.concatenate([_f32(rp.weight).reshape(rp.out_channels, -1), _f32(cp.weight).reshape(8, -1)], 0)
        bbias = np.concatenate([_f32(rp.bias), _f32(cp.bias)], 0)
        proj = self._ptr(_f32(det.proj_conv.weight).reshape(-1)) if bins > 1 else None
        abi.check(self.lib.lp_engine_add_head_box(self.h, r, i, bins, self._ptr(wb), self._ptr(bbias), proj),
                  'lp_engine_add_head_box')
        self.lane(0)

    def bind(self, B, H, W):
        if self.bound == (B, H, W):
            return
        if H % 32 or W % 32:
            raise ValueError('input height/width must be multiples of 32, got %dx%d' % (H, W))
        need = self.lib.lp_engine_arena_bytes(self.h, B, H, W)
        if need == 0:
            raise ValueError('bad input shape %s: H and W must be positive multiples of the coarsest stride of the model '
                             '(32; 64 with a P6 level), and small enough for the SPPF pool chain, which keeps a whole stride-32 '
                             'map in LDS (up to ~2048x2048 px in f16 / bf16, ~1440x1440 in f32)' % ((B, H, W),))
        if self.arena is None or self.arena.numel() < need + 256:
            self.arena = None
            self.arena = torch.zeros(need + 256, dtype=torch.uint8, device=self.device)
        abi.check(self.lib.lp_engine_bind(self.h, _aligned(self.arena), need, B, H, W), 'lp_engine_bind')
        self.bound = (B, H, W)
        self.n_anchors = self.lib.lp_engine_num_anchors(self.h)

    def set_graph(self, enable=True):
        self.graph = bool(enable)
        abi.check(self.lib.lp_engine_set_graph(self.h, 1 if enable else 0), 'lp_engine_set_graph')

    def _stream_enter(self):
        cur = torch.cuda.current_stream(self.device)
        if self._last_stream is not None and self._last_stream.cuda_stream != cur.cuda_stream:
            cur.wait_stream(self._last_stream)
        return cur

    def _stream_leave(self, cur):
        self._last_stream = cur

    def set_single_lane(self, enable=True):
        if bool(enable) != self.single_lane:
            self.single_lane = bool(enable)
            abi.check(self.lib.lp_engine_set_single_lane(self.h, 1 if enable else 0), 'lp_engine_set_single_lane')

    def copy_tuning(self, other):
        abi.check(self.lib.lp_engine_copy_tuning(self.h, other.h), 'lp_engine_copy_tuning')
        self.tuned = set(other.tuned)

    def set_variant(self, op, cfg, nbuf):
        self.autotune = False
        abi.check(self.lib.lp_engine_set_op_variant(self.h, op, cfg, nbuf), 'lp_engine_set_op_variant')

    def set_tile(self, op, choice):
        self.autotune = False
        abi.check(self.lib.lp_engine_set_op_tile(self.h, op, choice), 'lp_engine_set_op_tile')

    def tile(self, op):
        c, th, tw = ctypes.c_int(), ctypes.c_int(), ctypes.c_int()
        abi.check(self.lib.lp_engine_op_tile(self.h, op, ctypes.byref(c), ctypes.byref(th), ctypes.byref(tw)), 'lp_engine_op_tile')
        return c.value, th.value, tw.value

    def variant(self, op):
        cfg, nb = ctypes.c_int(), ctypes.c_int()
        abi.check(self.lib.lp_engine_op_variant(self.h, op, ctypes.byref(cfg), ctypes.byref(nb)), 'lp_engine_op_variant')
        return cfg.value, nb.value

    def op_io(self, op):
        src, dst = (ctypes.c_int * abi.LP_MAX_SRC)(), (ctypes.c_int * 3)()
        n, res = ctypes.c_int(), ctypes.c_int()
        abi.check(self.lib.lp_engine_op_io(self.h, op, src, ctypes.byref(n), ctypes.byref(res), dst), 'lp_engine_op_io')
        return list(src[:n.value]), res.value, [t for t in dst if t >= 0]

    def tensor_view(self, tid):
        off, c, cs, h, w = ctypes.c_size_t(), ctypes.c_int(), ctypes.c_int(), ctypes.c_int(), ctypes.c_int()
        abi.check(self.lib.lp_engine_tensor_info(self.h, tid, ctypes.byref(off), ctypes.byref(c), ctypes.byref(cs),
                                                 ctypes.byref(h), ctypes.byref(w)), 'lp_engine_tensor_info')
        B = self.bound[0]
        esz = torch.empty(0, dtype=self.dtype).element_size()
        base = _aligned(self.arena) - self.arena.data_ptr() + off.value
        n = B * h.value * w.value * cs.value
        flat = self.arena[base:base + n * esz].view(self.dtype)
        return flat.view(B, h.value, w.value, cs.value)[..., :c.value].permute(0, 3, 1, 2)

    def prepare(self, B, H, W, x_dtype=None):
        if not self._untuned((B, H, W)):
            return
        x = torch.zeros(B, 3, H, W, dtype=x_dtype or self.dtype, device=self.device)
        graph = self.graph
        if graph:
            self.set_graph(False)
        try:
            self.forward(x)
            torch.cuda.current_stream(self.device).synchronize()
        finally:
            if graph:
                self.set_graph(True)

    @staticmethod
    def _check_input(x):
        if x.dim() != 4 or x.shape[1] != 3:
            raise ValueError('expected [B,3,H,W], got %s' % (tuple(x.shape),))
        if x.dtype not in _DT:
            raise TypeError('unsupported input dtype %s' % x.dtype)
        return x.contiguous(), (x.shape[0], x.shape[2], x.shape[3])

    def _new_pred(self, B):
        return torch.empty(B, self.n_anchors, abi.LP_PRED_COLS, dtype=torch.float32, device=self.device)

    def _untuned(self, shape):
        return self.autotune and shape not in self.tuned and len(self.tuned) < self.max_tuned_shapes

    def forward(self, x):
        x, shape = self._check_input(x)
        with torch.cuda.device(self.device):
            cur = self._stream_enter()
            self.bind(*shape)
            if self.graph:
                if self._graph_pred is None or self._graph_pred.shape != (shape[0], self.n_anchors, abi.LP_PRED_COLS):
                    self._graph_pred = self._new_pred(shape[0])
                pred = self._graph_pred
                x = self._stage_for_graph(x)
            else:
                pred = self._new_pred(shape[0])
            if self._untuned(shape):
                abi.check(self.lib.lp_engine_autotune(self.h, _dptr(x), _DT[x.dtype], _dptr(pred), _stream_ptr(self.device), 5),
                          'lp_engine_autotune')
                self.tuned.add(shape)
            abi.check(self.lib.lp_engine_forward(self.h, _dptr(x), _DT[x.dtype], _dptr(pred), _stream_ptr(self.device)),
                      'lp_engine_forward')
            self._stream_leave(cur)
        return pred

    def _stage_for_graph(self, x):
        gx = self._graph_x
        if gx is None or gx.shape != x.shape or gx.dtype != x.dtype:
            gx = self._graph_x = torch.empty_like(x)
        if gx.data_ptr() != x.data_ptr():
            gx.copy_(x)
        return gx

    def forward_det(self, x, conf_thres, ws=None):
        x, shape = self._check_input(x)
        if not 0.0 <= conf_thres <= 1.0:
            raise ValueError('conf_thres must be in [0, 1]')
        with torch.cuda.device(self.device):
            if self._untuned(shape):
                self.forward(x)
            cur = self._stream_enter()
            self.bind(*shape)
            B, N = shape[0], self.n_anchors
            need = self.lib.lp_nms_workspace_bytes(B, N)
            if ws is None:
                ws = _nms_workspace(self.device, need)
            elif ws.numel() < need + 256:
                raise ValueError('workspace too small: %d bytes needed' % (need + 256))
            if self.graph:
                x = self._stage_for_graph(x)
            abi.check(self.lib.lp_engine_forward_det(self.h, _dptr(x), _DT[x.dtype], float(conf_thres), _aligned(ws), need,
                                                     _stream_ptr(self.device)), 'lp_engine_forward_det')
            self._stream_leave(cur)
        return ws, B, N

    def det_workspace(self, B, H, W):
        with torch.cuda.device(self.device):
            self.bind(B, H, W)
            return torch.empty(self.lib.lp_nms_workspace_bytes(B, self.n_anchors) + 256, dtype=torch.uint8, device=self.device)

    def detect(self, x, conf_thres, iou_thres, max_det, want_keep=False, route=None):
        if route is None:
            self._poll_pass_rate()
            route = 'pred' if (self.pass_rate is not None and self.pass_rate > self.det_crossover) else 'det'
        self.det_routes[route] += 1
        if route == 'pred':
            pred = self.forward(x)
            out = nms_padded(pred, conf_thres, iou_thres, max_det, want_keep)
            self._probe_pass_rate(_nms_workspace(self.device, 0), pred.shape[0], pred.shape[1])
            return out
        handle = self.forward_det(x, conf_thres)
        out = nms_candidates(handle, iou_thres, max_det, want_keep)
        self._probe_pass_rate(*handle)
        return out

    def _probe_pass_rate(self, ws, B, N):
        with torch.cuda.device(self.device):
            ptr = self.lib.lp_nms_candidate_counts(_aligned(ws), B, N)
            off = ptr - ws.data_ptr()
            pr = self._pass_probe
            if pr is None or pr[0].numel() != B:
                pr = (torch.empty(B, dtype=torch.int32).pin_memory(), torch.cuda.Event(), N)
            pr[0].copy_(ws[off:off + 4 * B].view(torch.int32), non_blocking=True)
            pr[1].record(torch.cuda.current_stream(self.device))
            self._pass_probe = (pr[0], pr[1], N)

    def _poll_pass_rate(self):
        pr = self._pass_probe
        if pr is not None and pr[1].query():
            self.pass_rate = float(pr[0].float().mean()) / max(1, pr[2])

    def op_kinds(self):
        return [self._op_info(i)['kind'] for i in range(self.lib.lp_engine_num_ops(self.h))]

    def _op_info(self, i):
        kind, ks, cin, cout = ctypes.c_int(), ctypes.c_int(), ctypes.c_int(), ctypes.c_int()
        fl, by = ctypes.c_double(), ctypes.c_double()
        abi.check(self.lib.lp_engine_op_info(self.h, i, ctypes.byref(kind), ctypes.byref(ks), ctypes.byref(cin),
                                             ctypes.byref(cout), ctypes.byref(fl), ctypes.byref(by)), 'lp_engine_op_info')
        return dict(kind=OP_KINDS[kind.value], ksize=ks.value, cin=cin.value, cout=cout.value, flops=fl.value, bytes=by.value)

    def profile(self, x, reps=3, inner=1):
        x = x.contiguous()
        B, _, H, W = x.shape
        with torch.cuda.device(self.device):
            self.bind(B, H, W)
            pred = self._new_pred(B)
            n = self.lib.lp_engine_num_ops(self.h)
            ms = (ctypes.c_float * n)()
            abi.check(self.lib.lp_engine_profile_ops(self.h, _dptr(x), _DT[x.dtype], _dptr(pred), _stream_ptr(self.device), ms, reps,
                                                     inner), 'lp_engine_profile_ops')
# ... 1366 lines not shown
```

Before: 18390 images/s.

## Compute head regression tower only at candidate anchors when few survive confidence

Adds a sparse regression-tower path. The shared 3x3 head conv computes only the classification channels densely. The regression channels are then computed by a new kernel only at anchors whose class score passed the confidence threshold, using the candidate keys from the NMS workspace. A gate reads per-level candidate counts from pinned host memory (written by the previous run) and enables the path when candidates are under 1/32 of the pixels. In exchange it adds extra launches, gather-style loads, graph-mask bookkeeping, and a dependency on counts from earlier frames.

```diff
diff --git a/include/lp_hip.h b/include/lp_hip.h
--- a/include/lp_hip.h
+++ b/include/lp_hip.h
@@ -91,6 +91,11 @@
 enum { LP_VARIANT_FUSED_BIFUSION = 45 };
 enum { LP_VARIANT_BOX_SPARSE = 46, LP_VARIANT_BOX_DENSE = 47 };
 enum { LP_VARIANT_PIPE16_S2A = 48, LP_VARIANT_PIPE16_S2B = 49 };
+enum { LP_VARIANT_REG_SPARSE = 50, LP_VARIANT_REG_DENSE = 51, LP_VARIANT_REG_AUTO = 52 };
+int lp_engine_op_reg_tower(const lp_engine* e, int op, int* sparse, int* now, int* cls_variant, int* cls_tile);
+int lp_engine_set_op_cls_only(lp_engine* e, int op, int variant, int tile);
+int lp_engine_remember_tuning(lp_engine* e, int B, int H, int W);
+int lp_engine_tuned_cls_only(const lp_engine* e, int B, int H, int W, int op, int* cls_variant, int* cls_tile);
 int lp_engine_op_carrier(const lp_engine* e, int op, int frame_direct);
 int lp_engine_op_io(const lp_engine* e, int op, int* src , int* n_src, int* res, int* dst );
 int lp_engine_autotune(lp_engine* e, const void* x, int x_dtype, float* pred, void* stream, int reps);
diff --git a/yolo-lp_amd/csrc/lp_conv.hip b/yolo-lp_amd/csrc/lp_conv.hip
--- a/yolo-lp_amd/csrc/lp_conv.hip
+++ b/yolo-lp_amd/csrc/lp_conv.hip
@@ -21,6 +21,9 @@
 int head_box_det_launch_f16(const ConvArgs& a, int cb_pack, hipStream_t st);
 int head_box_det_launch_bf16(const ConvArgs& a, int cb_pack, hipStream_t st);
 int head_box_det_launch_f32(const ConvArgs& a, int cb_pack, hipStream_t st);
+
+int head_regtower_launch_f16(const ConvArgs& a, hipStream_t st);
+int head_regtower_launch_bf16(const ConvArgs& a, hipStream_t st);
 
 ConvShape conv_shape(int dtype, int cfg, int ksize, int stride) {
     const int sz = (int)dtype_size(dtype);
@@ -375,6 +378,23 @@
     return fail(LP_ERR_ARG, "head box: dtype");
 }
 
+bool head_regtower_fits(int dtype, int cb_pack, int ksize, int stride, int nsrc, int nchunks, int out_split, int out2_c) {
+    return dtype != LP_F32 && cb_pack == 128 && ksize == 3 && stride == 1 && nsrc == 1 && nchunks >= 4 && nchunks % 4 == 0 && nchunks <= 16 &&
+           out_split >= 128 && out_split % 128 == 0 && out2_c >= 8 && out2_c % 8 == 0;
+}
+int head_regtower_launch(int dtype, const ConvArgs& a, hipStream_t st) {
+    if (!a.out2 || !a.zero || !a.det_keys || !a.det_cnt || a.B < 1 ||
+        !head_regtower_fits(dtype, 128, 3, 1, a.nsrc, a.chunk_begin[a.nsrc], a.out_split, a.out2_pix_stride) ||
+        a.nct * 128 < a.out_split + a.out2_pix_stride || a.Ho != a.H || a.Wo != a.W || a.nphase != 1 || a.out_scale != 1 || a.res ||
+        a.out2_img_stride != (long long)a.H * a.W * a.out2_pix_stride || a.src[0].cs % 8 != 0)
+        return fail(LP_ERR_ARG, "head regtower: op does not fit");
+    switch (dtype) {
+        case LP_F16: return head_regtower_launch_f16(a, st);
+        case LP_BF16: return head_regtower_launch_bf16(a, st);
+    }
+    return fail(LP_ERR_UNSUPPORTED, "head regtower: 16-bit activations only");
+}
+
 int head_rows_launch(int dtype, const ConvArgs& a, int cb_pack, hipStream_t st) {
     const int nchunks = a.chunk_begin[a.nsrc];
     if (!(a.det_mode ? head_det_fits(dtype, nchunks, cb_pack, a.out_c) : head_rows_fits(dtype, nchunks, cb_pack, a.out_c)))
diff --git a/yolo-lp_amd/csrc/lp_conv_bf16.hip b/yolo-lp_amd/csrc/lp_conv_bf16.hip
--- a/yolo-lp_amd/csrc/lp_conv_bf16.hip
+++ b/yolo-lp_amd/csrc/lp_conv_bf16.hip
@@ -2,6 +2,7 @@
 #include "lp_conv1x1_stream.inc"
 #include "lp_head_rows.inc"
 #include "lp_head_box.inc"
+#include "lp_head_regtower.inc"
 #include "lp_conv3x3_pipe.inc"
 #include "lp_conv3x3_pipe16.inc"
 #include "lp_conv3x3_pipe16v.inc"
@@ -20,6 +21,7 @@
 }
 int head_rows_launch_bf16(const ConvArgs& a, int cb_pack, hipStream_t st) { return head_rows_launch_dtype<bf16>(a, cb_pack, st); }
 int head_box_det_launch_bf16(const ConvArgs& a, int cb_pack, hipStream_t st) { return head_box_det_launch_dtype<bf16>(a, cb_pack, st); }
+int head_regtower_launch_bf16(const ConvArgs& a, hipStream_t st) { return head_regtower_launch_dtype<bf16>(a, st); }
 int conv_pipe_launch_bf16(int pcfg, const ConvArgs& a, int ncu, hipStream_t st) {
     if (pcfg == PIPE_FUSED2) return stem2_fused_launch<bf16>(a, ncu, st);
     if (pcfg == PIPE_FUSED_PW) return pw_s2_fused_launch<bf16>(a, ncu, st);
diff --git a/yolo-lp_amd/csrc/lp_conv_f16.hip b/yolo-lp_amd/csrc/lp_conv_f16.hip
--- a/yolo-lp_amd/csrc/lp_conv_f16.hip
+++ b/yolo-lp_amd/csrc/lp_conv_f16.hip
@@ -2,6 +2,7 @@
 #include "lp_conv1x1_stream.inc"
 #include "lp_head_rows.inc"
 #include "lp_head_box.inc"
+#include "lp_head_regtower.inc"
 #include "lp_conv3x3_pipe.inc"
 #include "lp_conv3x3_pipe16.inc"
 #include "lp_conv3x3_pipe16v.inc"
@@ -20,6 +21,7 @@
 }
 int head_rows_launch_f16(const ConvArgs& a, int cb_pack, hipStream_t st) { return head_rows_launch_dtype<f16>(a, cb_pack, st); }
 int head_box_det_launch_f16(const ConvArgs& a, int cb_pack, hipStream_t st) { return head_box_det_launch_dtype<f16>(a, cb_pack, st); }
+int head_regtower_launch_f16(const ConvArgs& a, hipStream_t st) { return head_regtower_launch_dtype<f16>(a, st); }
 int conv_pipe_launch_f16(int pcfg, const ConvArgs& a, int ncu, hipStream_t st) {
     if (pcfg == PIPE_FUSED2) return stem2_fused_launch<f16>(a, ncu, st);
     if (pcfg == PIPE_FUSED_PW) return pw_s2_fused_launch<f16>(a, ncu, st);
diff --git a/yolo-lp_amd/csrc/lp_engine.hip b/yolo-lp_amd/csrc/lp_engine.hip
--- a/yolo-lp_amd/csrc/lp_engine.hip
+++ b/yolo-lp_amd/csrc/lp_engine.hip
@@ -34,6 +34,7 @@
     int fused = 0;
     int fused_pw = 0;
     int fused_bf = 0;
+    int co_pipe = 0, co_tile = 0;
     Choice& choice() { return *this; }
 };
 
@@ -57,6 +58,9 @@
     int mode = MODE_ACT, nct = 1, nchunks = 0, nphase = 1;
     size_t det_scratch = (size_t)-1;
     int box_sparse = 1;
+    int reg_box = -1;
+    int reg_tower = -1;
+    int reg_sparse = 0;
     int bf_up = -1, bf_cv1 = -1;
     int bf_carrier = -1;
     int chunk_begin[LP_MAX_SRC + 1] = {0, 0, 0, 0, 0};
@@ -78,6 +82,7 @@
 static bool bifusion_fused_possible(const lp_engine* e, size_t i, int* up, int* cv1);
 static bool op_fam16(const lp_engine* e, const lp::Op& op);
 static int fam16_default_pipe(const lp_engine* e, const lp::Op& op);
+static int reg_sparse_possible(const lp_engine* e, size_t i);
 
 #ifndef LP_MAX_LANES
 #define LP_MAX_LANES 5
@@ -114,6 +119,7 @@
         float conf = 0.f;
         int x_dtype = -1;
         unsigned long long epoch = 0, last_use = 0;
+        unsigned long long reg_mask = 0;
         hipStream_t stream = nullptr;
     };
     std::vector<CachedGraph> graphs;
@@ -127,6 +133,9 @@
     Launch stem2_fused;
     std::map<int, Launch> pw_fused;
     std::map<int, Launch> bf_fused;
+    std::map<int, Launch> cls_only;
+    int* reg_counts = nullptr;
+    std::vector<char> reg_gate;
     std::map<std::vector<int>, std::vector<Choice>> tuned;
 };
 
@@ -160,6 +169,7 @@
         if (g.exec) (void)hipGraphExecDestroy(g.exec);
     }
     if (e->cap_stream) (void)hipStreamDestroy(e->cap_stream);
+    if (e->reg_counts) (void)hipHostFree(e->reg_counts);
     for (hipEvent_t ev : e->op_event) if (ev) (void)hipEventDestroy(ev);
     if (e->fork_ev) (void)hipEventDestroy(e->fork_ev);
     for (int l = 1; l < LP_MAX_LANES; ++l) { if (e->join_ev[l]) (void)hipEventDestroy(e->join_ev[l]); if (e->lane_stream[l]) (void)hipStreamDestroy(e->lane_stream[l]); }
@@ -521,6 +531,15 @@
         }
         e->box_sparse_ok = ok && nbox >= 1 && nbox <= 4 && cls_seen == 0;
     }
+    {
+        for (size_t i = 0; i < e->ops.size(); ++i) {
+            const int box = reg_sparse_possible(e, i);
+            if (box < 0) continue;
+            e->ops[i].reg_box = box;
+            e->ops[(size_t)box].reg_tower = e->ops[(size_t)box - 1].reg_tower = (int)i;
+            e->ops[i].reg_sparse = 2;
+        }
+    }
     e->finalized = true;
     return LP_OK;
 }
@@ -709,6 +728,27 @@
     return conv_pipe_fits(e->dtype, PIPE16_D, conv_shape(e->dtype, op.cfg, 1, 1).CB, 3, 1, op.mode, op.nct, op.nphase, op.nchunks);
 }
 static int fam16_default_pipe(const lp_engine*, const Op& op) { return (op.stride == 2 ? PIPE16_S2A : PIPE16_D) + 1; }
+
+static int reg_sparse_possible(const lp_engine* e, size_t i) {
+    if (e->dtype == LP_F32 || i + 2 >= e->ops.size() || !e->box_sparse_ok) return -1;
+    const Op& t = e->ops[i];
+    if (t.kind != OP_CONV || t.dst2 < 0 || t.res >= 0 || t.nphase != 1 || t.mode != MODE_ACT || !op_fam16(e, t)) return -1;
+    if (!head_regtower_fits(e->dtype, conv_shape(e->dtype, t.cfg, 3, 1).CB, t.ksize, t.stride, t.nsrc, t.nchunks, e->tensors[t.dst].cs,
+                            e->tensors[t.dst2].cs)) return -1;
+    const Op& c = e->ops[i + 1];
+    const Op& b = e->ops[i + 2];
+    if (c.kind != OP_HEAD_CLS || b.kind != OP_HEAD_BOX || c.level != b.level || c.src[0] != t.dst || b.src[0] != t.dst2 || b.reg_bins != 1 ||
+        b.cout != 12 || b.nchunks > 4) return -1;
+    for (size_t k = 0; k < e->ops.size(); ++k) {
+        const Op& o = e->ops[k];
+        if (k != i + 2) {
+            for (int q = 0; q < o.nsrc; ++q) if (o.src[q] == t.dst2) return -1;
+            if (o.res == t.dst2) return -1;
+        }
+        if (k != i && (o.dst == t.dst2 || o.dst2 == t.dst2 || o.dst3 == t.dst2)) return -1;
+    }
+    return (int)i + 2;
+}
 
 static int prepare_op(lp_engine* e, size_t idx) {
     ++e->epoch;
@@ -856,6 +896,32 @@
         fa.fz_c1 = e->tensors[pw.dst].cs;
         F.pipe = PIPE_FUSED_PW + 1;
     }
+    if (op.reg_box >= 0) {
+        Launch& C = e->cls_only[(int)idx];
+        C = L;
+        ConvArgs& ca = C.a;
+        ca.nct = a.out_split / cb_pack;
+        ca.out_c = a.out_split;
+        ca.out2 = nullptr;
+        ca.out_split = 0;
+        int pc = (op.co_pipe ? op.co_pipe : op.pipe) - 1;
+        if (pc < 0 || !pipe_is_16(pc) || pipe_is_16s2(pc) ||
+            !conv_pipe_fits(dt, pc, cb_pack, ks, stv, op.mode, ca.nct, op.nphase, op.nchunks))
+            pc = fam16_default_pipe(e, op) - 1;
+        const ConvShape ps = conv_pipe_shape(pc);
+        if (pipe_is_16v(pc)) {
+            conv_pick_tile16v(ps, ca.Ho, ca.Wo, e->B, ca.nct, op.co_tile, &ca.TH, &ca.TW);
+            ca.hpitch = ca.TW + 2;
+        } else {
+            conv_pick_tile(ps, ks, stv, ca.Ho, ca.Wo, op.co_tile, &ca.TH, &ca.TW);
+            ca.hpitch = conv_pick_pitch16(ps, ca.TH, ca.TW);
+        }
+        ca.tw_magic = (unsigned)(((1u << 22) + ca.TW - 1) / ca.TW);
+        ca.hp_magic = (unsigned)(((1u << 22) + ca.hpitch - 1) / ca.hpitch);
+        ca.tiles_x = ceil_div(ca.Wo, ca.TW);
+        ca.tiles_y = ceil_div(ca.Ho, ca.TH);
+        C.pipe = pc + 1;
+    }
     return LP_OK;
 }
 
@@ -938,41 +1004,85 @@
     float conf;
 };
 
+struct BoxForm { bool streams, snap, sparse; };
+static BoxForm box_form(const lp_engine* e, size_t idx) {
+    static const bool no_box_stream = getenv("LP_NO_BOX_STREAM") != nullptr;
+    static const bool no_box_sparse = getenv("LP_NO_BOX_SPARSE") != nullptr;
+    const bool snap_ok = !no_box_sparse && e->box_sparse_ok && (e->n_lanes <= 1 || e->single_lane) && e->box_ord[idx] >= 0 && e->n_anchors >= 8;
+    auto streams = [&](size_t j) { const Launch& Lj = e->launches[j]; return !no_box_stream && head_box_det_fits(Lj.a, Lj.cb_pack, Lj.ks, Lj.st); };
+    BoxForm f = {streams(idx), false, false};
+    if (!f.streams || !snap_ok) return f;
+    f.snap = true;
+    const int k = e->box_ord[idx];
+    bool prev_snap = k == 0;
+    for (size_t j = 0; j < idx && !prev_snap; ++j) prev_snap = e->box_ord[j] == k - 1 && streams(j);
+    f.sparse = e->ops[idx].box_sparse && prev_snap;
+    return f;
+}
+
+static bool reg_sparse_lanes_ok(const lp_engine* e) { return e->n_lanes <= 1 || e->single_lane; }
+constexpr int REG_GATE_DIV = 32;
+static unsigned long long update_reg_gate(lp_engine* e) {
+    unsigned long long mask = 0;
+    e->reg_gate.assign(e->ops.size(), 0);
+    if (!e->reg_counts || !e->arena) return 0;
+    for (size_t i = 0; i < e->ops.size() && i < 64; ++i) {
+        const Op& op = e->ops[i];
+        if (op.reg_box < 0 || op.reg_sparse != 2) continue;
+        const int k = e->box_ord[(size_t)op.reg_box];
+        const int cnt = ((volatile const int*)e->reg_counts)[k];
+        const Tensor& t = e->tensors[op.dst];
+        if (cnt >= 0 && (long long)cnt * REG_GATE_DIV <= (long long)e->B * t.h * t.w) { e->reg_gate[i] = 1; mask |= 1ull << i; }
+    }
+    return mask;
+}
+static bool reg_sparse_now(const lp_engine* e, size_t i) {
+    static const bool off = getenv("LP_NO_REG_SPARSE") != nullptr;
+    const Op& op = e->ops[i];
+    if (off || op.reg_box < 0 || !op.reg_sparse || !reg_sparse_lanes_ok(e) || !e->arena || i >= e->launches.size()) return false;
+    if (op.reg_sparse == 2 && !(i < e->reg_gate.size() && e->reg_gate[i])) return false;
+    const Launch& L = e->launches[i];
+    if (!L.pipe || !pipe_is_16(L.pipe - 1) || pipe_is_16s2(L.pipe - 1)) return false;
+    return box_form(e, (size_t)op.reg_box).sparse;
+}
+
 static int run_head_det(lp_engine* e, size_t idx, const DetCtx& dc, hipStream_t st) {
     const Op& op = e->ops[idx];
     const Launch& L = e->launches[idx];
     const int dt = e->dtype;
     ConvArgs a = L.a;
     const int anchor0 = e->level_off[op.level], N = e->n_anchors;
+    const bool reg_sparse = op.reg_tower >= 0 && reg_sparse_now(e, (size_t)op.reg_tower);
+    int* const snaps = dc.w.kept;
     if (L.mode == MODE_DECODE) {
         a.det_mode = 1;
         a.out = dc.w.rows + (long long)anchor0 * LP_DET_COLS;
         a.out_pix_stride = LP_DET_COLS;
         a.out_img_stride = (long long)N * LP_DET_COLS;
-        static const bool no_box_stream = getenv("LP_NO_BOX_STREAM") != nullptr;
-        static const bool no_box_sparse = getenv("LP_NO_BOX_SPARSE") != nullptr;
-        const bool snap_ok = !no_box_sparse && e->box_sparse_ok && (e->n_lanes <= 1 || e->single_lane) && e->box_ord[idx] >= 0 && N >= 8;
-        auto streams = [&](size_t j) { const Launch& Lj = e->launches[j]; return !no_box_stream && head_box_det_fits(Lj.a, Lj.cb_pack, Lj.ks, Lj.st); };
-        if (streams(idx)) {
-            if (snap_ok) {
+        const BoxForm f = box_form(e, idx);
+        if (f.streams) {
+            if (f.snap) {
                 const int k = e->box_ord[idx];
-                int* const snaps = dc.w.kept;
                 a.det_cnt = dc.w.cnt;
                 a.det_np = dc.w.NP;
                 a.det_snap = snaps + (size_t)k * e->B;
-                bool prev_snap = k == 0;
-                for (size_t j = 0; j < idx && !prev_snap; ++j) prev_snap = e->box_ord[j] == k - 1 && streams(j);
-                if (op.box_sparse && prev_snap) {
+                bool last = e->reg_counts != nullptr;
+                for (size_t j = 0; j < e->ops.size() && last; ++j)
+                    if (e->box_ord[j] >= 0) last = j <= idx ? box_form(e, j).snap : false;
+                if (last) { a.det_lvl_counts = e->reg_counts; a.det_snaps = snaps; a.det_nlev = k + 1; }
+                if (f.sparse) {
                     a.det_keys = dc.w.keys;
                     a.det_n = N;
                     a.det_anchor0 = anchor0;
                     a.det_prev = k > 0 ? snaps + (size_t)(k - 1) * e->B : nullptr;
+                    a.det_compact = reg_sparse ? 1 : 0;
                 }
             }
             return head_box_det_launch(dt, a, L.cb_pack, st);
         }
         return conv_launch(dt, L.cfg, L.mode, L.ks, L.st, L.nbuf, a, st);
     }
+    int rc;
     if (op.det_scratch == (size_t)-1) {
         a.det_mode = 1;
         a.out = dc.w.rows;
@@ -982,15 +1092,26 @@
         a.det_n = N;
         a.det_anchor0 = anchor0;
         a.det_conf = dc.conf;
-        return head_rows_launch(dt, a, L.cb_pack, st);
-    }
-    float* const scratch = (float*)(e->arena + op.det_scratch);
-    const int rpi = a.Ho * a.Wo;
-    a.out = scratch + 13;
-    a.out_img_stride = (long long)rpi * LP_PRED_COLS;
-    int rc = conv_launch(dt, L.cfg, L.mode, L.ks, L.st, L.nbuf, a, st);
-    if (rc) return rc;
-    return nms_score_launch(scratch, e->B, rpi, anchor0, N, dc.conf, dc.w, false, st);
+        rc = head_rows_launch(dt, a, L.cb_pack, st);
+    } else {
+        float* const scratch = (float*)(e->arena + op.det_scratch);
+        const int rpi = a.Ho * a.Wo;
+        a.out = scratch + 13;
+        a.out_img_stride = (long long)rpi * LP_PRED_COLS;
+        rc = conv_launch(dt, L.cfg, L.mode, L.ks, L.st, L.nbuf, a, st);
+        if (rc) return rc;
+        rc = nms_score_launch(scratch, e->B, rpi, anchor0, N, dc.conf, dc.w, false, st);
+    }
+    if (rc || !reg_sparse) return rc;
+    ConvArgs t = e->launches[(size_t)op.reg_tower].a;
+    const int k = e->box_ord[(size_t)e->ops[(size_t)op.reg_tower].reg_box];
+    t.det_keys = dc.w.keys;
+    t.det_cnt = dc.w.cnt;
+    t.det_np = dc.w.NP;
+    t.det_n = N;
+    t.det_anchor0 = anchor0;
+    t.det_prev = k > 0 ? snaps + (size_t)(k - 1) * e->B : nullptr;
+    return head_regtower_launch(dt, t, st);
 }
 
 static int run_op(lp_engine* e, size_t idx, const void* x, int x_dtype, float* pred, hipStream_t st, const DetCtx* det = nullptr) {
@@ -1021,6 +1142,10 @@
         ConvArgs a = e->stem_planar.a;
         a.src[0].ptr = x;
         return conv_pipe_launch(dt, PIPE_P, a, st);
+    }
+    if (det && op.reg_box >= 0 && reg_sparse_now(e, idx)) {
+        const Launch& C = e->cls_only[(int)idx];
+        return conv_pipe_launch(dt, C.pipe - 1, C.a, st);
     }
     if (L.mode == MODE_ACT && L.pipe) return conv_pipe_launch(dt, L.pipe - 1, L.a, st);
     if (L.mode == MODE_ACT && L.stream_wc) return conv_stream_launch(dt, L.stream_wc, L.a, L.cb_pack, st);
@@ -1112,6 +1237,18 @@
 
 static int run_forward(lp_engine* e, const void* x, int x_dtype, float* pred, const DetCtx* det, void* ws, hipStream_t main_st) {
     int rc;
+    unsigned long long reg_mask = 0;
+    if (det) {
+        if (!e->reg_counts) {
+            bool any = false;
+            for (const Op& op : e->ops) any = any || op.reg_box >= 0;
+            if (any) {
+                LP_HIP_CHECK(hipHostMalloc((void**)&e->reg_counts, 64, hipHostMallocMapped | hipHostMallocCoherent));
+                for (int k = 0; k < 16; ++k) e->reg_counts[k] = -1;
+            }
+        }
+        reg_mask = update_reg_gate(e);
+    }
     auto issue = [&](hipStream_t st) -> int {
         if (det) { if (int zr = zero_counts_launch(det->w.cnt, e->B, st)) return zr; }
         return issue_forward(e, x, x_dtype, pred, st, det);
@@ -1124,7 +1261,7 @@
     const float conf = det ? det->conf : 0.f;
     lp_engine::CachedGraph* hit = nullptr;
     for (auto& g : e->graphs)
-        if (g.exec && g.x == x && g.pred == pred && g.ws == ws && g.conf == conf && g.x_dtype == x_dtype && g.epoch == e->epoch) hit = &g;
+        if (g.exec && g.x == x && g.pred == pred && g.ws == ws && g.conf == conf && g.x_dtype == x_dtype && g.epoch == e->epoch && g.reg_mask == reg_mask) hit = &g;
     if (!hit) {
         for (size_t i = 0; i < e->graphs.size();) {
             auto& g = e->graphs[i];
@@ -1157,6 +1294,7 @@
         cg.conf = conf;
         cg.x_dtype = x_dtype;
         cg.epoch = e->epoch;
+        cg.reg_mask = reg_mask;
         e->graphs.push_back(cg);
         hit = &e->graphs.back();
     }
@@ -1248,17 +1386,19 @@
     LP_HIP_CHECK(hipEventCreate(&evp.b));
     const hipEvent_t e0 = evp.a, e1 = evp.b;
     int trc = LP_OK;
-    auto time_best = [&](std::initializer_list<size_t> seq) -> float {
+    auto time_calls = [&](auto&& issue) -> float {
         float ms_min = -1.f;
         for (int round = 0; round < 3 && trc == LP_OK; ++round) {
             float ms = 0.f;
             if (hipEventRecord(e0, st) != hipSuccess) { trc = LP_ERR_HIP; break; }
-            for (int r = 0; r < reps; ++r)
-                for (size_t k : seq) run_op(e, k, x, x_dtype, pred, st);
+            for (int r = 0; r < reps; ++r) issue();
             if (hipEventRecord(e1, st) != hipSuccess || hipEventSynchronize(e1) != hipSuccess || hipEventElapsedTime(&ms, e0, e1) != hipSuccess) { trc = LP_ERR_HIP; break; }
             if (ms_min < 0.f || ms < ms_min) ms_min = ms;
         }
         return trc ? -1.f : ms_min;
+    };
+    auto time_best = [&](std::initializer_list<size_t> seq) -> float {
+        return time_calls([&]() { for (size_t k : seq) run_op(e, k, x, x_dtype, pred, st); });
     };
     auto time_current = [&](size_t i) -> float { return run_op(e, i, x, x_dtype, pred, st) == LP_OK ? time_best({i}) : -1.f; };
     auto walk_tiles = [&](size_t i, float* best) -> int {
@@ -1376,6 +1516,32 @@
             rc = try_form(i, op.fused_bf, time_best({(size_t)op.bf_up, (size_t)op.bf_cv1, i}), false);
             if (rc) return rc;
         }
+        if (op.reg_box >= 0 && op.pipe && pipe_is_16(op.pipe - 1)) {
+            const int nct_cls = e->tensors[op.dst].cs / cb;
+            float t_best = -1.f;
+            int w_pipe = 0, w_tile = 0;
+            for (int pc = PIPE16_D; pc < PIPE_END && trc == LP_OK; ++pc) {
+                if (!pipe_is_16(pc) || !conv_pipe_fits(e->dtype, pc, cb, op.ksize, op.stride, op.mode, nct_cls, op.nphase, op.nchunks)) continue;
+                int last_th = -1, last_tw = -1;
+                for (int tile = 0; tile < 3 && trc == LP_OK; ++tile) {
+                    op.co_pipe = pc + 1;
+                    op.co_tile = tile;
+                    if (prepare_op(e, i) != LP_OK) continue;
+                    const Launch& C = e->cls_only[(int)i];
+                    if (C.a.TH == last_th && C.a.TW == last_tw) break;
+                    last_th = C.a.TH;
+                    last_tw = C.a.TW;
+                    if (conv_pipe_launch(e->dtype, C.pipe - 1, C.a, st) != LP_OK) continue;
+                    const float ms = time_calls([&]() { conv_pipe_launch(e->dtype, C.pipe - 1, C.a, st); });
+                    if (ms >= 0.f && (t_best < 0.f || ms < t_best)) { t_best = ms; w_pipe = pc + 1; w_tile = tile; }
+                }
+            }
+            if (trc) return fail(trc, "autotune: event timing failed");
+            op.co_pipe = w_pipe;
+            op.co_tile = w_tile;
+            rc = prepare_op(e, i);
+            if (rc) return rc;
+        }
     }
     e->tuned[{e->B, e->H, e->W}].assign(e->ops.begin(), e->ops.end());
     return LP_OK;
@@ -1407,6 +1573,16 @@
         op.rows = cfg == LP_VARIANT_ROWS;
         e->tuned.erase({e->B, e->H, e->W});
         if (e->arena && op_idx < (int)e->launches.size()) return prepare_op(e, (size_t)op_idx);
+        return LP_OK;
+    }
+    if (cfg == LP_VARIANT_REG_SPARSE || cfg == LP_VARIANT_REG_DENSE || cfg == LP_VARIANT_REG_AUTO) {
+        if (cfg != LP_VARIANT_REG_DENSE && (op.reg_box < 0 || !reg_sparse_lanes_ok(e)))
+            return fail(LP_ERR_UNSUPPORTED, "lp_engine_set_op_variant: not a head tower whose regression half can run for candidates only "
+                                            "(two-destination 16x16x32 3x3 layer split on a cout tile, <= 16 K-chunks, class and box predictors "
+                                            "right behind it, reg_feat read by the box predictors alone, 16-bit, no DFL, one lane)");
+        if (op.reg_box < 0) return LP_OK;
+        op.reg_sparse = cfg == LP_VARIANT_REG_SPARSE ? 1 : cfg == LP_VARIANT_REG_AUTO ? 2 : 0;
+        ++e->epoch;
         return LP_OK;
     }
     if (op.kind == OP_HEAD_BOX && (cfg == LP_VARIANT_BOX_SPARSE || cfg == LP_VARIANT_BOX_DENSE)) {
@@ -1580,3 +1756,46 @@
     if (nbuf) *nbuf = stream ? e->ops[op].stream_rd : e->ops[op].nbuf;
     return LP_OK;
 }
+
+extern "C" int lp_engine_op_reg_tower(const lp_engine* e, int op, int* sparse, int* now, int* cls_variant, int* cls_tile) {
+    if (!e || !e->finalized || op < 0 || op >= (int)e->ops.size()) return fail(LP_ERR_ARG, "lp_engine_op_reg_tower: engine not finalized, or op index");
+    const Op& o = e->ops[(size_t)op];
+    if (o.reg_box < 0) return fail(LP_ERR_UNSUPPORTED, "lp_engine_op_reg_tower: not a head tower whose regression half can run for candidates only");
+    if (sparse) *sparse = o.reg_sparse;
+    if (e->arena) update_reg_gate(const_cast<lp_engine*>(e));
+    if (now) *now = e->arena ? reg_sparse_now(e, (size_t)op) : (o.reg_sparse == 1 && reg_sparse_lanes_ok(e) && getenv("LP_NO_REG_SPARSE") == nullptr);
+    if (cls_variant) *cls_variant = o.co_pipe ? LP_VARIANT_PIPE_D + o.co_pipe - 1 : 0;
+    if (cls_tile) *cls_tile = o.co_tile;
+    return LP_OK;
+}
+
+extern "C" int lp_engine_set_op_cls_only(lp_engine* e, int op_idx, int variant, int tile) {
+    if (!e || !e->finalized || op_idx < 0 || op_idx >= (int)e->ops.size() || tile < 0) return fail(LP_ERR_ARG, "lp_engine_set_op_cls_only: op index or tile");
+    Op& op = e->ops[(size_t)op_idx];
+    const int pc = variant - LP_VARIANT_PIPE_D;
+    if (op.reg_box < 0) return fail(LP_ERR_UNSUPPORTED, "lp_engine_set_op_cls_only: not a head tower with a class-only launch");
+    if (variant != 0 && (!pipe_is_16(pc) || pipe_is_16s2(pc) ||
+                         !conv_pipe_fits(e->dtype, pc, 128, op.ksize, op.stride, op.mode, e->tensors[op.dst].cs / 128, op.nphase, op.nchunks)))
+        return fail(LP_ERR_UNSUPPORTED, "lp_engine_set_op_cls_only: not a 16x16x32 variant that fits the class half");
+    op.co_pipe = variant ? pc + 1 : 0;
+    op.co_tile = tile;
+    e->tuned.erase({e->B, e->H, e->W});
+    if (e->arena && op_idx < (int)e->launches.size()) return prepare_op(e, (size_t)op_idx);
+    return LP_OK;
+}
+
+extern "C" int lp_engine_remember_tuning(lp_engine* e, int B, int H, int W) {
+    if (!e || !e->finalized || B < 1 || H < 1 || W < 1) return fail(LP_ERR_ARG, "lp_engine_remember_tuning: engine not finalized, or shape");
+    e->tuned[{B, H, W}].assign(e->ops.begin(), e->ops.end());
+    return LP_OK;
+}
+
+extern "C" int lp_engine_tuned_cls_only(const lp_engine* e, int B, int H, int W, int op, int* cls_variant, int* cls_tile) {
+    if (!e || op < 0 || op >= (int)e->ops.size()) return fail(LP_ERR_ARG, "lp_engine_tuned_cls_only: op index");
+    const auto it = e->tuned.find({B, H, W});
+    if (it == e->tuned.end()) return fail(LP_ERR_STATE, "lp_engine_tuned_cls_only: no tuning remembered for this shape");
+    const Choice& c = it->second[(size_t)op];
+    if (cls_variant) *cls_variant = c.co_pipe ? LP_VARIANT_PIPE_D + c.co_pipe - 1 : 0;
+    if (cls_tile) *cls_tile = c.co_tile;
+    return LP_OK;
+}
diff --git a/yolo-lp_amd/csrc/lp_head_box.inc b/yolo-lp_amd/csrc/lp_head_box.inc
--- a/yolo-lp_amd/csrc/lp_head_box.inc
+++ b/yolo-lp_amd/csrc/lp_head_box.inc
@@ -30,6 +30,21 @@
         const int b = blockIdx.x * 256 + threadIdx.x;
         if (b < a.B) { const int c = a.det_cnt[b]; a.det_snap[b] = c > a.det_np ? a.det_np : c; }
     }
+    if (a.det_lvl_counts && blockIdx.x == 0 && wave == 0) {
+        for (int k = 0; k < a.det_nlev; ++k) {
+            int tot = 0;
+            for (int b = lane; b < a.B; b += 64) {
+                int c = a.det_cnt[b];
+                c = c > a.det_np ? a.det_np : c;
+                const int hi_ = k + 1 < a.det_nlev ? a.det_snaps[k * a.B + b] : c;
+                const int lo_ = k ? a.det_snaps[(k - 1) * a.B + b] : 0;
+                tot += hi_ > lo_ ? hi_ - lo_ : 0;
+            }
+#pragma unroll
+            for (int o = 32; o; o >>= 1) tot += __shfl_xor(tot, o);
+            if (lane == 0) a.det_lvl_counts[k] = tot;
+        }
+    }
     if (t0 >= ntiles) return;
 
     V wa[NK];
@@ -49,14 +64,16 @@
     for (long long t = t0; t < ntiles; t += tstride) {
         long long m = t * 32 + r;
         bool live = m < M;
+        [[maybe_unused]] long long mc = -1;
         if constexpr (SPARSE) {
-            live = m < sn;
+            live = m < sn && (!a.det_compact || m < HW);
+            if (a.det_compact) mc = (long long)sb * HW + (live ? m : 0);
             const unsigned long long key = a.det_keys[(long long)sb * a.det_np + slo + (live ? m : 0)];
             const int n_ = (int)(unsigned)key - a.det_anchor0;
             live = live && n_ >= 0 && n_ < HW;
             m = (long long)sb * HW + (live ? n_ : 0);
         }
-        const char* const row = src + (live ? m : M - 1) * (long long)cs * SZ + h * 16;
+        const char* const row = src + (live ? (mc >= 0 ? mc : m) : M - 1) * (long long)cs * SZ + h * 16;
         V vb[NK];
 #pragma unroll
         for (int k = 0; k < NK; ++k) vb[k] = *(const V*)(2 * k + h < ngran ? row + k * 32 : (const char*)a.zero);
diff --git a/yolo-lp_amd/csrc/lp_head_regtower.inc b/yolo-lp_amd/csrc/lp_head_regtower.inc
--- /dev/null
+++ b/yolo-lp_amd/csrc/lp_head_regtower.inc
@@ -0,0 +1,101 @@
+#pragma once
+#include "lp_conv3x3_pipe16.inc"
+
+namespace lp {
+
+constexpr int REGTOWER_MAXCHUNKS = 16;
+
+template <typename T, int NBW>
+__global__ __launch_bounds__(256) void head_regtower_kernel(const ConvArgs a, const int gpi) {
+    typedef typename Mma<T>::V V;
+    static_assert(sizeof(T) == 2, "16-bit activations only");
+    constexpr int CB = 128, NB = CB / 16, ROWB = 32, KC = 16, NG = NB / NBW;
+    static_assert(NB % NBW == 0, "whole groups of cout blocks");
+    const int lane = threadIdx.x & 63, wave = threadIdx.x >> 6;
+    const int li = lane & 15, g = lane >> 4, h = g >> 1;
+    const int HW = a.H * a.W;
+    const int nchunks = a.chunk_begin[a.nsrc];
+    const int ct0 = a.out_split / CB, nrt = a.nct - ct0;
+    const int cs = a.src[0].cs, cs2 = a.out2_pix_stride;
+    const int sb = blockIdx.x / gpi, gi = blockIdx.x - sb * gpi;
+    int hi = a.det_cnt[sb];
+    hi = hi > a.det_np ? a.det_np : hi;
+    int slo = a.det_prev ? a.det_prev[sb] : 0;
+    slo = slo < 0 ? 0 : (slo > hi ? hi : slo);
+    int sn = hi - slo;
+    sn = sn > HW ? HW : sn;
+    const int nitems = ((sn + 15) / 16) * nrt * NG;
+    const int arow = quad_order(li);
+    const int aoff = arow * ROWB + swz(arow, g & 1, 2) * 16;
+    const T* const zero = (const T*)a.zero;
+
+    for (int it = gi * 4 + wave; it < nitems; it += gpi * 4) {
+        const int tile = it / (nrt * NG), rem = it - tile * (nrt * NG);
+        const int ct = ct0 + rem / NG, b0 = (rem % NG) * NBW;
+        const int m = tile * 16 + li;
+        bool live = m < sn;
+        const unsigned long long key = a.det_keys[(long long)sb * a.det_np + slo + (live ? m : 0)];
+        int n_ = (int)(unsigned)key - a.det_anchor0;
+        live = live && n_ >= 0 && n_ < HW;
+        n_ = live ? n_ : 0;
+        const int oy = n_ / a.W, ox = n_ - oy * a.W;
+        const T* const px = (const T*)a.src[0].ptr + ((long long)sb * HW + n_) * cs;
+        const char* const wt = (const char*)a.w + (long long)ct * nchunks * (9 * CB * ROWB) + b0 * 16 * ROWB + aoff;
+
+        f32x4v acc[NBW];
+#pragma unroll
+        for (int c = 0; c < NBW; ++c) acc[c] = *(const f32x4v*)(a.bias + ct * CB + (b0 + c) * 16 + quad_order(4 * g));
+        for (int e = 0; e < nchunks; e += 2) {
+            V fa[9][NBW], fb[9];
+#pragma unroll
+            for (int s = 0; s < 9; ++s) {
+                const int ta = s < 4 ? 2 * s : (s == 4 ? 8 : 2 * s - 9), tb = s == 4 ? 0 : ta + 1;
+                const int t = h ? tb : ta;
+                const int q = e + (h ? (s >= 4 ? 1 : 0) : (s >= 5 ? 1 : 0));
+                const int dy = t / 3 - 1, dx = t - (t / 3) * 3 - 1;
+                const int yy = oy + dy, xx = ox + dx;
+                const int c = q * KC + (g & 1) * 8;
+                const bool ok = live && yy >= 0 && yy < a.H && xx >= 0 && xx < a.W && c < cs;
+                fb[s] = *(const V*)(ok ? px + (long long)(dy * a.W + dx) * cs + c : zero);
+                const char* const wp = wt + (long long)(q * 9 + t) * (CB * ROWB);
+#pragma unroll
+                for (int k = 0; k < NBW; ++k) fa[s][k] = *(const V*)(wp + k * 16 * ROWB);
+            }
+            __builtin_amdgcn_sched_barrier(0);
+#pragma unroll
+            for (int s = 0; s < 9; ++s)
+#pragma unroll
+                for (int k = 0; k < NBW; ++k) acc[k] = Mma16<T>::mma(fa[s][k], fb[s], acc[k]);
+        }
+        if (!live) continue;
+        T* const orow = (T*)a.out2 + ((long long)sb * HW + m) * cs2;
+        act_dispatch(a.act, [&](auto tag) {
+            constexpr int ACT = decltype(tag)::value;
+#pragma unroll
+            for (int k = 0; k < NBW; ++k) {
+                typedef T T4 __attribute__((ext_vector_type(4)));
+                T4 o;
+#pragma unroll
+                for (int j = 0; j < 4; ++j) o[j] = from_f32<T>(act_c<ACT>(acc[k][j]));
+                const int cc = (ct - ct0) * CB + (b0 + k) * 16 + quad_order(4 * g);
+                if (cc < cs2) *(T4*)(orow + cc) = o;
+            }
+        });
+    }
+}
+
+template <typename T>
+static inline int head_regtower_launch_dtype(const ConvArgs& a, hipStream_t st) {
+    constexpr int NBW = 2;
+    const int HW = a.H * a.W, nrt = a.nct - a.out_split / 128;
+    long long gpi = ((long long)((HW + 15) / 16) * nrt * (8 / NBW) + 3) / 4;
+    const long long cap = 2048 / a.B;
+    if (gpi > cap) gpi = cap;
+    if (gpi < 1) gpi = 1;
+    hipLaunchKernelGGL((head_regtower_kernel<T, NBW>), dim3((unsigned)(gpi * a.B)), dim3(256), 0, st, a, (int)gpi);
+    hipError_t e = hipGetLastError();
+    if (e != hipSuccess) return fail(LP_ERR_HIP, std::string("head regtower launch: ") + hipGetErrorString(e));
+    return LP_OK;
+}
+
+}
diff --git a/yolo-lp_amd/csrc/lp_internal.h b/yolo-lp_amd/csrc/lp_internal.h
--- a/yolo-lp_amd/csrc/lp_internal.h
+++ b/yolo-lp_amd/csrc/lp_internal.h
@@ -115,6 +115,10 @@
     float det_conf;
     const int* det_prev;
     int* det_snap;
+    int* det_lvl_counts;
+    const int* det_snaps;
+    int det_nlev;
+    int det_compact;
     const void* fz_w1;
     const float* fz_b1;
     int fz_act1, fz_c1;
@@ -151,6 +155,8 @@
 bool head_box_det_fits(const ConvArgs& a, int cb_pack, int ksize, int stride);
 int head_box_det_launch(int dtype, const ConvArgs& a, int cb_pack, hipStream_t st);
 int head_rows_launch(int dtype, const ConvArgs& a, int cb_pack, hipStream_t st);
+bool head_regtower_fits(int dtype, int cb_pack, int ksize, int stride, int nsrc, int nchunks, int out_split, int out2_c);
+int head_regtower_launch(int dtype, const ConvArgs& a, hipStream_t st);
 
 struct NmsWs {
     int32_t* cnt;
diff --git a/yolo-lp_amd/yolov6/hip/abi.py b/yolo-lp_amd/yolov6/hip/abi.py
--- a/yolo-lp_amd/yolov6/hip/abi.py
+++ b/yolo-lp_amd/yolov6/hip/abi.py
@@ -12,6 +12,7 @@
 LP_VARIANT_PIPE16_S2A, LP_VARIANT_PIPE16_S2B = 48, 49
 LP_VARIANT_FUSED_BIFUSION = 45
 LP_VARIANT_BOX_SPARSE, LP_VARIANT_BOX_DENSE = 46, 47
+LP_VARIANT_REG_SPARSE, LP_VARIANT_REG_DENSE, LP_VARIANT_REG_AUTO = 50, 51, 52
 LP_VARIANT_FUSED_PW_S2 = 38
 LP_VARIANT_FUSED_STEM2 = 37
 LP_VARIANT_PIPE_P = 36
@@ -159,6 +160,10 @@
     'lp_engine_set_op_tile': (c_int, [c_void_p, c_int, c_int]),
     'lp_engine_op_tile': (c_int, [c_void_p, c_int, POINTER(c_int), POINTER(c_int), POINTER(c_int)]),
     'lp_engine_copy_tuning': (c_int, [c_void_p, c_void_p]),
+    'lp_engine_op_reg_tower': (c_int, [c_void_p, c_int, POINTER(c_int), POINTER(c_int), POINTER(c_int), POINTER(c_int)]),
+    'lp_engine_set_op_cls_only': (c_int, [c_void_p, c_int, c_int, c_int]),
+    'lp_engine_remember_tuning': (c_int, [c_void_p, c_int, c_int, c_int]),
+    'lp_engine_tuned_cls_only': (c_int, [c_void_p, c_int, c_int, c_int, c_int, POINTER(c_int), POINTER(c_int)]),
     'lp_nms_workspace_bytes': (c_size_t, [c_int, c_int]),
     'lp_nms_candidate_counts': (c_void_p, [c_void_p, c_int, c_int]),
     'lp_preprocess_letterbox': (c_int, [c_void_p, c_int, c_int, c_void_p, c_int, c_int, c_int, c_int, c_int, c_int, c_int,
diff --git a/yolo-lp_amd/yolov6/hip/runtime.py b/yolo-lp_amd/yolov6/hip/runtime.py
--- a/yolo-lp_amd/yolov6/hip/runtime.py
+++ b/yolo-lp_amd/yolov6/hip/runtime.py
@@ -389,6 +389,16 @@
         cfg, nb = ctypes.c_int(), ctypes.c_int()
         abi.check(self.lib.lp_engine_op_variant(self.h, op, ctypes.byref(cfg), ctypes.byref(nb)), 'lp_engine_op_variant')
         return cfg.value, nb.value
+
+    def reg_tower(self, op):
+        v = [ctypes.c_int() for _ in range(4)]
+        if self.lib.lp_engine_op_reg_tower(self.h, op, *[ctypes.byref(t) for t in v]) != 0:
+            return None
+        return v[0].value, bool(v[1].value), v[2].value, v[3].value
+
+    def set_cls_only(self, op, variant, tile=0):
+        self.autotune = False
+        abi.check(self.lib.lp_engine_set_op_cls_only(self.h, op, variant, tile), 'lp_engine_set_op_cls_only')
 
     def op_io(self, op):
         src, dst = (ctypes.c_int * abi.LP_MAX_SRC)(), (ctypes.c_int * 3)()
```

Result: slower. 18060 images/s (-1.8%).
